# kotaro-kinoshita/yomitoku

Hardware: AMD Instinct MI355X
Metric: pages/sec (DocumentAnalyzer @1600x1200, lite model set) (higher is better)
Workload: dtype f32 held as two scaled fp16 planes per operand on the MFMA pipe: 3 x v_mfma_f32_32x32x16_f16 per product tile (products to 2^-21, below the fp32 accumulation's own rounding), fp32 accumulate, fp32 activations in HBM; attention, LayerNorm, the fused greedy step and every grid-starved launch exact fp3

## Files before the change

### include/ymk.h

```cpp
#ifndef YMK_H
#define YMK_H
#include <stddef.h>
#include <stdint.h>

#ifdef __cplusplus
extern "C" {
#endif

typedef struct ymk_model ymk_model;

int ymk_version(void);
const char* ymk_last_error(void);
int ymk_device_count(void);

ymk_model* ymk_model_create(const char* kind, int device);
void ymk_model_destroy(ymk_model* m);
int ymk_model_set_param(ymk_model* m, const char* key, double value);
int ymk_model_set_tensor(ymk_model* m, const char* name, const float* host_data, int ndim, const int64_t* dims);
int ymk_model_finalize(ymk_model* m);
int ymk_model_reserve(ymk_model* m, int n, int h, int w, void* stream);
int ymk_op_plan_workspace(int64_t n, const int64_t* sizes, const int64_t* release_pos, int64_t* offsets_out, int64_t* peak_out,
                          int64_t* live_bound_out);
int64_t ymk_model_weight_bytes(const ymk_model* m);
int64_t ymk_model_workspace_bytes(const ymk_model* m);
// ... 26 lines not shown
int ymk_crop_desc_size(void);

int ymk_db_postprocess(const float* prob_host, int h, int w, float thresh, float box_thresh, int min_size,
                       int max_candidates, float unclip_ratio, int dest_w, int dest_h, int16_t* quads_out,
                       double* scores_out, int capacity, int* count);

int ymk_table_hole_rects(int h, int w, const int* cell_boxes, int n, int pad, int close_ksize, int min_area, int* rects_out,
                         int capacity, int* count);

int ymk_prof_begin(void);
int ymk_debug_option(const char* key, int value);
int ymk_stat(const char* key, int64_t* value);
int ymk_amax_check_counters(int64_t* out4);
int ymk_prof_end(double* conv_ms, double* conv_flop, int64_t* conv_launches);
int ymk_prof_bytes(double* conv_bytes);
int ymk_prof_launch_table(double* ms, double* flop, double* bytes, double* mfma_products, int64_t capacity, int64_t* count);

int ymk_op_conv2d(const float* x_dev, int n, int h, int w, int c,
                  const float* w_host_oihw, int cout, int cin, int kh, int kw, const float* scale_host,
                  const float* bias_host, const float* res_dev, int stride, int pad, int dil, int act, int tap4,
                  float* y_dev, void* stream);
int ymk_op_conv1x1_astat(const float* x_dev, int m, int c, const float* w_host_oc, int cout, const float* scale_host,
                         const float* bias_host, const float* res_dev, int act, const float* ln_g_host, const float* ln_b_host,
                         float ln_eps, float* y_dev, int reps, float* kernel_ms, void* stream);

int ymk_op_vit_mlp(const float* x_dev, int m, int d, int f, const float* ln_g_host, const float* ln_b_host, float ln_eps,
                   const float* w1_host_fd, const float* b1_host, const float* w2_host_df, const float* b2_host, float* y_dev, int reps,
                   float* kernel_ms, void* stream);

int ymk_op_layernorm(const float* x_dev, int rows, int d, const float* g_dev, const float* b_dev, float eps,
                     float* y_dev, void* stream);
int ymk_op_attention(const float* q_dev, const float* k_dev, const float* v_dev, float* o_dev, int b, int heads, int lq,
                     int lk, int hd, float scale, const unsigned char* mask_qk_dev, const unsigned char* kpm_dev,
                     int use_small, void* stream);
int ymk_op_nar_cross_attention(const float* q_dev, const float* k_dev, const float* v_dev, float* o_dev, int b, int heads, int lq,
                               int lk, int hd, float scale, const int* koff_dev, const int* klen_dev, void* stream);
int ymk_op_maxpool3x3s2(const float* x_dev, int n, int h, int w, int c, float* y_dev, void* stream);
int ymk_op_upsample_bilinear(const float* x_dev, int n, int h, int w, int c, int oh, int ow, const float* add_dev,
                             float* y_dev, void* stream);

int ymk_op_topk_tokens(const float* logits_dev, int b, const int* level_hw, int nc, int k, int* idx_dev, void* stream);
int ymk_op_gather_queries(const float* om_dev, const float* bbox_dev, const float* anchors_dev, const int* idx_dev, int b,
                          const int* level_hw, int k, int d, float* content_dev, float* ref_dev, void* stream);
int ymk_op_refine_boxes(const float* delta_dev, const float* ref_dev, float* out_dev, int64_t n, void* stream);
int ymk_op_mask_rows(const float* in_dev, const float* valid_dev, int b, const int* level_hw, int d, float* out_dev, void* stream);
int ymk_op_deform_sample(const float* offs_dev, const float* attw_dev, const float* ref_dev, const float* value_dev, int ldv, int b,
                         const int* level_hw, int k, float* out_dev, void* stream);
int ymk_op_avgpool2x2_ceil(const float* x_dev, int n, int h, int w, int c, float* y_dev, void* stream);
int ymk_op_upsample_nearest2x(const float* x_dev, int n, int h, int w, int c, float* y_dev, void* stream);

int ymk_op_deconv2x2(const float* x_dev, int n, int h, int w, int cin, const float* w_host, int cout, const float* scale_host,
                     const float* bias_host, int act, float* y_dev, void* stream);
int ymk_op_deconv2x2_to1_sigmoid(const float* x_dev, int n, int h, int w, const float* w_host, float bias, float* y_dev, void* stream);
int ymk_op_dbnet_asf(const float* ax_dev, const float* fuse_dev, int n, int h, int w, const float* w1_host, const float* w2_host,
                     int cmid, const float* sp33_host, float sp11, const float* watt_host, float* out_dev, void* stream);

int ymk_op_parseq_dec_step(int d, int heads, int f, const float* sa_in_w_host, const float* sa_in_b_host, const float* sa_out_w_host,
                           const float* sa_out_b_host, const float* ca_in_w_host, const float* ca_in_b_host,
                           const float* ca_out_w_host, const float* ca_out_b_host, const float* lin1_w_host, const float* lin1_b_host,
                           const float* lin2_w_host, const float* lin2_b_host, const float* const* ln_host, const float* emb_host,
                           int ntok, const float* posq_host, const float* qsa_host, const int* tok_dev, float* skv_dev,
                           const float* memkv_dev, const int* mem_off_dev, const int* mem_len_dev, const int* prev_not_done_dev,
                           const int* gid_dev, const int* gopen_dev, int ng, int step, int b, int l, int ns, float* out_dev,
                           void* stream);
int ymk_op_greedy_step(const float* logits_dev, int64_t ld_b, int c, int step, int num_steps, int* tok_dev, int* raw_dev, int ld_tok,
                       int* state_dev, int eos_id, int rep_on, int period_max, int min_run_p1, int min_repeats, int* not_done_dev,
                       const int* prev_not_done_dev, const int* gid_dev, int* gopen_dev, int ng, int partials, int b, void* stream);
int ymk_op_refine_prep(const int* raw_dev, int ld_tok, int s_len, int bos_id, int eos_id, int* tok2_dev, unsigned char* kpm_dev, int b,
                       const int* gid_dev, const int* gsteps_dev, void* stream);
int ymk_op_rep_cut(float* logits_dev, int64_t ld_b, int c, int s_len, const int* state_dev, int eos_id, int b, void* stream);
int ymk_op_row_argmax(const float* logits_dev, int rows, int c, int* out_dev, void* stream);
int ymk_op_ctx_embed_ln(const int* tok_dev, int ld_tok, int pos0, int npos, const float* emb_dev, const float* posq_dev,
                        const float* g_dev, const float* b_dev, float eps, float* out_dev, int out_rows, int d, int b, void* stream);
int ymk_op_init_decode(int* tok_dev, int ld_tok, int* state_dev, int bos_id, int pad_id, int b, void* stream);
int ymk_op_tile_rows(const float* src_dev, int rows, int d, float* dst_dev, int b, void* stream);
int ymk_op_add_pos_embed(float* x_dev, const float* pos_dev, int b, int gh, int gw, int full_gw, int d, void* stream);

#ifdef __cplusplus
}
#endif
#endif
```

### yomitoku_amd/_lib.py

```python

from __future__ import annotations

import ctypes
import os
from ctypes import POINTER, c_char_p, c_double, c_float, c_int, c_int64, c_void_p

_HERE = os.path.dirname(os.path.abspath(__file__))
LIB_PATH = os.path.join(_HERE, "lib", "libymk_hip.so")

SIGNATURES = {
    "ymk_version": (c_int, []),
    "ymk_last_error": (c_char_p, []),
    "ymk_device_count": (c_int, []),
    "ymk_model_create": (c_void_p, [c_char_p, c_int]),
    "ymk_model_destroy": (None, [c_void_p]),
    "ymk_model_set_param": (c_int, [c_void_p, c_char_p, c_double]),
    "ymk_model_set_tensor": (c_int, [c_void_p, c_char_p, c_void_p, c_int, POINTER(c_int64)]),
    "ymk_model_finalize": (c_int, [c_void_p]),
    "ymk_model_reserve": (c_int, [c_void_p, c_int, c_int, c_int, c_void_p]),
    "ymk_op_plan_workspace": (c_int, [c_int64, POINTER(c_int64), POINTER(c_int64), POINTER(c_int64), POINTER(c_int64), POINTER(c_int64)]),
    "ymk_model_weight_bytes": (c_int64, [c_void_p]),
    "ymk_model_workspace_bytes": (c_int64, [c_void_p]),
    "ymk_dbnet_forward": (c_int, [c_void_p, c_void_p, c_int, c_int, c_int, c_void_p, c_void_p]),
    "ymk_parseq_dims": (c_int, [c_void_p, POINTER(c_int), POINTER(c_int)]),
# ... 31 lines not shown
    "ymk_stat": (c_int, [c_char_p, POINTER(c_int64)]),
    "ymk_op_vit_mlp": (
        c_int,
        [c_void_p, c_int, c_int, c_int, c_void_p, c_void_p, c_float, c_void_p, c_void_p, c_void_p, c_void_p, c_void_p, c_int, POINTER(c_float), c_void_p],
    ),
    "ymk_amax_check_counters": (c_int, [POINTER(c_int64)]),
    "ymk_prof_begin": (c_int, []),
    "ymk_prof_end": (c_int, [POINTER(c_double), POINTER(c_double), POINTER(c_int64)]),
    "ymk_prof_bytes": (c_int, [POINTER(c_double)]),
    "ymk_prof_launch_table": (c_int, [POINTER(c_double), POINTER(c_double), POINTER(c_double), POINTER(c_double), c_int64, POINTER(c_int64)]),
    "ymk_op_conv2d": (
        c_int,
        [c_void_p, c_int, c_int, c_int, c_int, c_void_p, c_int, c_int, c_int, c_int, c_void_p, c_void_p, c_void_p,
         c_int, c_int, c_int, c_int, c_int, c_void_p, c_void_p],
    ),
    "ymk_op_conv1x1_astat": (
        c_int,
        [c_void_p, c_int, c_int, c_void_p, c_int, c_void_p, c_void_p, c_void_p, c_int, c_void_p, c_void_p, c_float, c_void_p, c_int,
         POINTER(c_float), c_void_p],
    ),
    "ymk_op_layernorm": (c_int, [c_void_p, c_int, c_int, c_void_p, c_void_p, c_float, c_void_p, c_void_p]),
    "ymk_op_attention": (
        c_int,
        [c_void_p, c_void_p, c_void_p, c_void_p, c_int, c_int, c_int, c_int, c_int, c_float, c_void_p, c_void_p, c_int,
         c_void_p],
    ),
    "ymk_op_nar_cross_attention": (
        c_int,
        [c_void_p, c_void_p, c_void_p, c_void_p, c_int, c_int, c_int, c_int, c_int, c_float, c_void_p, c_void_p, c_void_p],
    ),
    "ymk_op_maxpool3x3s2": (c_int, [c_void_p, c_int, c_int, c_int, c_int, c_void_p, c_void_p]),
    "ymk_op_upsample_bilinear": (
        c_int,
        [c_void_p, c_int, c_int, c_int, c_int, c_int, c_int, c_void_p, c_void_p, c_void_p],
    ),
    "ymk_op_topk_tokens": (c_int, [c_void_p, c_int, POINTER(c_int), c_int, c_int, c_void_p, c_void_p]),
    "ymk_op_gather_queries": (
        c_int,
        [c_void_p, c_void_p, c_void_p, c_void_p, c_int, POINTER(c_int), c_int, c_int, c_void_p, c_void_p, c_void_p],
    ),
    "ymk_op_refine_boxes": (c_int, [c_void_p, c_void_p, c_void_p, c_int64, c_void_p]),
    "ymk_op_mask_rows": (c_int, [c_void_p, c_void_p, c_int, POINTER(c_int), c_int, c_void_p, c_void_p]),
    "ymk_op_deform_sample": (
        c_int,
        [c_void_p, c_void_p, c_void_p, c_void_p, c_int, c_int, POINTER(c_int), c_int, c_void_p, c_void_p],
    ),
    "ymk_op_avgpool2x2_ceil": (c_int, [c_void_p, c_int, c_int, c_int, c_int, c_void_p, c_void_p]),
    "ymk_op_upsample_nearest2x": (c_int, [c_void_p, c_int, c_int, c_int, c_int, c_void_p, c_void_p]),
    "ymk_op_deconv2x2": (
        c_int,
        [c_void_p, c_int, c_int, c_int, c_int, c_void_p, c_int, c_void_p, c_void_p, c_int, c_void_p, c_void_p],
    ),
    "ymk_op_deconv2x2_to1_sigmoid": (c_int, [c_void_p, c_int, c_int, c_int, c_void_p, c_float, c_void_p, c_void_p]),
    "ymk_op_dbnet_asf": (
        c_int,
        [c_void_p, c_void_p, c_int, c_int, c_int, c_void_p, c_void_p, c_int, c_void_p, c_float, c_void_p, c_void_p, c_void_p],
    ),
    "ymk_op_parseq_dec_step": (
        c_int,
        [c_int, c_int, c_int] + [c_void_p] * 12 + [POINTER(c_void_p), c_void_p, c_int, c_void_p, c_void_p]
        + [c_void_p] * 8 + [c_int, c_int, c_int, c_int, c_int, c_void_p, c_void_p],
    ),
    "ymk_op_greedy_step": (
        c_int,
        [c_void_p, c_int64, c_int, c_int, c_int, c_void_p, c_void_p, c_int, c_void_p, c_int, c_int, c_int, c_int, c_int, c_void_p,
         c_void_p, c_void_p, c_void_p, c_int, c_int, c_int, c_void_p],
    ),
    "ymk_op_refine_prep": (c_int, [c_void_p, c_int, c_int, c_int, c_int, c_void_p, c_void_p, c_int, c_void_p, c_void_p, c_void_p]),
    "ymk_op_rep_cut": (c_int, [c_void_p, c_int64, c_int, c_int, c_void_p, c_int, c_int, c_void_p]),
    "ymk_op_row_argmax": (c_int, [c_void_p, c_int, c_int, c_void_p, c_void_p]),
    "ymk_op_ctx_embed_ln": (
        c_int,
        [c_void_p, c_int, c_int, c_int, c_void_p, c_void_p, c_void_p, c_void_p, c_float, c_void_p, c_int, c_int, c_int, c_void_p],
    ),
    "ymk_op_init_decode": (c_int, [c_void_p, c_int, c_void_p, c_int, c_int, c_int, c_void_p]),
    "ymk_op_tile_rows": (c_int, [c_void_p, c_int, c_int, c_void_p, c_int, c_void_p]),
    "ymk_op_add_pos_embed": (c_int, [c_void_p, c_void_p, c_int, c_int, c_int, c_int, c_int, c_void_p]),
}

_lib = None


class YmkError(RuntimeError):
    pass


def load():
    global _lib
    if _lib is not None:
        return _lib
    if not os.path.exists(LIB_PATH):
        raise YmkError(
            f"{LIB_PATH} not found - build it with `python -c 'import __graft_entry__ as g; g.build()'` "
            "or `make -C yomitoku_amd/csrc` (there is no CPU fallback)"
        )
    lib = ctypes.CDLL(LIB_PATH)
    for name, (res, args) in SIGNATURES.items():
        fn = getattr(lib, name)
        fn.restype = res
        fn.argtypes = args
    _lib = lib
    spec = os.environ.get("YMK_DEBUG_OPTIONS", "")
    if os.environ.get("YMK_CONV_SPLIT"):
        spec += ",conv_split=" + os.environ["YMK_CONV_SPLIT"]
    if os.environ.get("YMK_WORKSPACE_REUSE"):
        spec += ",workspace_reuse=" + os.environ["YMK_WORKSPACE_REUSE"]
# ... 71 lines not shown
```

### yomitoku_amd/csrc/ymk_api.cpp

```cpp
#include "../../include/ymk.h"
#include "ymk_common.h"
#include "ymk_decstep.h"
#include "ymk_det.h"
#include "ymk_seq.h"

namespace ymk {
const std::string& last_error();
void dbnet_forward(Model* m, const float* x, int n, int h, int w, float* prob, hipStream_t s);
void parseq_forward(Model* m, const float* x, int B, int W, float* logits, int* out_len, int* ar_steps, hipStream_t s);
void parseq_forward_groups(Model* m, const float* const* x, const int* b, const int* w, int ng, float* logits, int* out_len,
                           int* ar_steps, hipStream_t s);
void parseq_dims(Model* m, int* num_steps, int* num_classes);
Model* create_parseq();
Model* create_rtdetr();
void rtdetr_forward(Model* m, const float* x, int B, int H, int W, float* logits, float* boxes, hipStream_t s);
void row_maxprob(hipStream_t s, const float* logits, int rows, int C, int* ids, float* probs);
void prof_begin();
void prof_end(double* ms, double* flop, int64_t* launches);
double prof_bytes();
int64_t prof_launch_table(double* ms, double* flop, double* bytes, double* products, int64_t capacity);
bool gemm_takes_astat(int M, int K, const ConvW& w, bool with_res, int ld);
bool conv_debug_option(const std::string& key, int value);
bool parseq_debug_option(const std::string& key, int value);
bool decstep_debug_option(const std::string& key, int value);
bool conv_split_debug_option(const std::string& key, int value);
bool conv_split_stat(const std::string& key, long long* value);
bool parseq_stat(const std::string& key, long long* value);
void amax_check_counters(long long* out4);
}

struct ymk_model {
  ymk::Model* impl = nullptr;
  int device = 0;
};

#include <dlfcn.h>
namespace {
struct Roctx {
  int (*push)(const char*) = nullptr;
  int (*pop)() = nullptr;
  Roctx() {
    const char* on = std::getenv("YMK_ROCTX");
    if (on == nullptr || on[0] == '\0' || on[0] == '0') return;
    for (const char* name : {"librocprofiler-sdk-roctx.so", "libroctx64.so"}) {
      if (void* h = dlopen(name, RTLD_NOW | RTLD_GLOBAL)) {
        push = reinterpret_cast<int (*)(const char*)>(dlsym(h, "roctxRangePushA"));
        pop = reinterpret_cast<int (*)()>(dlsym(h, "roctxRangePop"));
        if (push && pop) return;
        push = nullptr;
        pop = nullptr;
      }
    }
  }
};
struct RoctxRange {
  explicit RoctxRange(const char* name) {
    static Roctx r;
    pop_ = r.pop;
    if (r.push) (void)r.push(name);
    else pop_ = nullptr;
  }
  ~RoctxRange() {
    if (pop_) (void)pop_();
  }
  int (*pop_)() = nullptr;
};
}

#define YMK_API_BEGIN try {
#define YMK_API_END                                 \
  return 0;                                         \
  }                                                 \
  catch (const std::exception& e) {                 \
    ymk::set_error(e.what());                       \
    return 1;                                       \
  }                                                 \
  catch (...) {                                     \
    ymk::set_error("unknown C++ exception");        \
    return 2;                                       \
// ... 104 lines not shown
int ymk_parseq_forward(ymk_model* m, const float* x_dev, int b, int w, float* logits_dev, int* out_len, int* ar_steps,
                       void* stream) {
  YMK_API_BEGIN
  RoctxRange roctx_range("ymk_parseq_forward");
  YMK_CHECK(m && x_dev && logits_dev && out_len && ar_steps, "null argument");
  YMK_HIP(hipSetDevice(m->device));
  ymk::parseq_forward(m->impl, x_dev, b, w, logits_dev, out_len, ar_steps, (hipStream_t)stream);
  YMK_API_END
}

int ymk_parseq_forward_groups(ymk_model* m, const float* const* x_dev, const int* b, const int* w, int n_groups,
                              float* logits_dev, int* out_len, int* ar_steps, void* stream) {
  YMK_API_BEGIN
  RoctxRange roctx_range("ymk_parseq_forward_groups");
  YMK_CHECK(m && x_dev && b && w && logits_dev && out_len && ar_steps, "null argument");
  YMK_HIP(hipSetDevice(m->device));
  ymk::parseq_forward_groups(m->impl, x_dev, b, w, n_groups, logits_dev, out_len, ar_steps, (hipStream_t)stream);
  YMK_API_END
}

int ymk_parseq_token_stats(const float* logits_dev, int rows, int num_classes, int* ids_dev, float* probs_dev,
                           void* stream) {
  YMK_API_BEGIN
  RoctxRange roctx_range("ymk_parseq_token_stats");
  YMK_CHECK(logits_dev && ids_dev && probs_dev, "null argument");
  ymk::row_maxprob((hipStream_t)stream, logits_dev, rows, num_classes, ids_dev, probs_dev);
  YMK_API_END
}

int ymk_rtdetr_forward(ymk_model* m, const float* x_dev, int b, int h, int w, float* logits_dev, float* boxes_dev,
                       void* stream) {
  YMK_API_BEGIN
  RoctxRange roctx_range("ymk_rtdetr_forward");
  YMK_CHECK(m && x_dev && logits_dev && boxes_dev, "null argument");
  YMK_HIP(hipSetDevice(m->device));
  ymk::rtdetr_forward(m->impl, x_dev, b, h, w, logits_dev, boxes_dev, (hipStream_t)stream);
  YMK_API_END
}

int ymk_debug_option(const char* key, int value) {
  YMK_API_BEGIN
  YMK_CHECK(key != nullptr, "null key");
  const std::string k(key);
  YMK_CHECK(ymk::conv_debug_option(k, value) || ymk::parseq_debug_option(k, value) || ymk::decstep_debug_option(k, value) ||
                ymk::conv_split_debug_option(k, value) || ymk::runtime_debug_option(k, value),
            "unknown debug option: " + k);
  YMK_API_END
}

int ymk_stat(const char* key, int64_t* value) {
  YMK_API_BEGIN
  YMK_CHECK(key != nullptr && value != nullptr, "null argument");
  long long v = 0;
  YMK_CHECK(ymk::conv_split_stat(std::string(key), &v) || ymk::runtime_stat(std::string(key), &v) || ymk::parseq_stat(std::string(key), &v), std::string("unknown counter: ") + key);
  *value = v;
  YMK_API_END
}

int ymk_amax_check_counters(int64_t* out4) {
  YMK_API_BEGIN
  YMK_CHECK(out4 != nullptr, "null argument");
  long long v[4];
  ymk::amax_check_counters(v);
  for (int i = 0; i < 4; ++i) out4[i] = v[i];
  YMK_API_END
}

int ymk_prof_begin(void) {
  YMK_API_BEGIN
  ymk::prof_begin();
  YMK_API_END
}

int ymk_prof_end(double* conv_ms, double* conv_flop, int64_t* conv_launches) {
  YMK_API_BEGIN
  YMK_CHECK(conv_ms && conv_flop && conv_launches, "null argument");
  ymk::prof_end(conv_ms, conv_flop, conv_launches);
  YMK_API_END
}

int ymk_prof_bytes(double* conv_bytes) {
  YMK_API_BEGIN
  YMK_CHECK(conv_bytes, "null argument");
  *conv_bytes = ymk::prof_bytes();
  YMK_API_END
}

int ymk_prof_launch_table(double* ms, double* flop, double* bytes, double* mfma_products, int64_t capacity, int64_t* count) {
  YMK_API_BEGIN
  YMK_CHECK(count != nullptr && capacity >= 0 && (capacity == 0 || (ms && flop && bytes && mfma_products)), "null argument");
  *count = ymk::prof_launch_table(ms, flop, bytes, mfma_products, capacity);
  YMK_API_END
}

int ymk_op_plan_workspace(int64_t n, const int64_t* sizes, const int64_t* release_pos, int64_t* offsets_out, int64_t* peak_out,
                          int64_t* live_bound_out) {
  YMK_API_BEGIN
  YMK_CHECK(n >= 0 && (n == 0 || (sizes && offsets_out)), "plan_workspace: bad argument");
  std::vector<size_t> sz((size_t)n), off((size_t)n);
  for (int64_t k = 0; k < n; ++k) {
    YMK_CHECK(sizes[k] >= 0, "plan_workspace: negative size");
    sz[(size_t)k] = (size_t)sizes[k];
  }
  size_t peak = 0, live = 0;
  ymk::plan_workspace((size_t)n, sz.data(), release_pos, off.data(), &peak, &live);
  for (int64_t k = 0; k < n; ++k) offsets_out[k] = (int64_t)off[(size_t)k];
  if (peak_out) *peak_out = (int64_t)peak;
// ... 260 lines not shown

int ymk_op_deform_sample(const float* offs_dev, const float* attw_dev, const float* ref_dev, const float* value_dev, int ldv, int b,
                         const int* level_hw, int k, float* out_dev, void* stream) {
  YMK_API_BEGIN
  using namespace ymk;
  const DetGeom g = det_geom_arg(b, level_hw);
  YMK_CHECK(offs_dev && attw_dev && ref_dev && value_dev && out_dev && k >= 1, "deform_sample: bad argument");
  YMK_CHECK(ldv >= 256 && ldv % 4 == 0, "deform_sample: ldv >= 256, a multiple of 4");
  YMK_CHECK(aligned16(value_dev) && aligned16(ref_dev) && aligned16(out_dev), "deform_sample: value / ref / out must be 16 B aligned");
  deform_sample((hipStream_t)stream, offs_dev, attw_dev, ref_dev, value_dev, ldv, g, k, out_dev);
  YMK_API_END
}

int ymk_op_avgpool2x2_ceil(const float* x_dev, int n, int h, int w, int c, float* y_dev, void* stream) {
  YMK_API_BEGIN
  using namespace ymk;
  YMK_CHECK(x_dev && y_dev && n >= 1 && h >= 1 && w >= 1 && c >= 4 && c % 4 == 0, "avgpool: c must be a positive multiple of 4");
  Tensor in{const_cast<float*>(x_dev), n, h, w, c, c};
  Tensor out{y_dev, n, (h + 1) / 2, (w + 1) / 2, c, c};
  avgpool2x2_ceil((hipStream_t)stream, in, out);
  YMK_API_END
}

int ymk_op_upsample_nearest2x(const float* x_dev, int n, int h, int w, int c, float* y_dev, void* stream) {
  YMK_API_BEGIN
  using namespace ymk;
  YMK_CHECK(x_dev && y_dev && n >= 1 && h >= 1 && w >= 1 && c >= 4 && c % 4 == 0, "nearest2x: c must be a positive multiple of 4");
  Tensor in{const_cast<float*>(x_dev), n, h, w, c, c};
  Tensor out{y_dev, n, 2 * h, 2 * w, c, c};
  upsample_nearest2x((hipStream_t)stream, in, out);
  YMK_API_END
}

int ymk_op_deconv2x2(const float* x_dev, int n, int h, int w, int cin, const float* w_host, int cout, const float* scale_host,
                     const float* bias_host, int act, float* y_dev, void* stream) {
  YMK_API_BEGIN
  using namespace ymk;
  YMK_CHECK(x_dev && w_host && y_dev && n >= 1 && h >= 1 && w >= 1, "deconv2x2: bad argument");
  YMK_CHECK(cin >= 4 && cin % 4 == 0 && cout >= 4 && cout % 4 == 0, "deconv2x2: cin and cout must be positive multiples of 4");
  DevicePool pool;
  const ConvW cw = make_deconv2x2_panel(pool, w_host, cin, cout, scale_host, bias_host);
  Tensor in{const_cast<float*>(x_dev), n, h, w, cin, cin};
  Tensor out{y_dev, n, 2 * h, 2 * w, cout, cout};
  ConvArgs a;
  a.act = act;
  a.epi = EPI_DECONV2X2;
  SplitCtxOwner split_ctx;
  ConvSplitScope scope(-1, split_ctx.get(), 0);
  conv2d((hipStream_t)stream, in, cw, a, out);
  YMK_HIP(hipStreamSynchronize((hipStream_t)stream));
  YMK_API_END
}

int ymk_op_deconv2x2_to1_sigmoid(const float* x_dev, int n, int h, int w, const float* w_host, float bias, float* y_dev,
                                 void* stream) {
  YMK_API_BEGIN
  using namespace ymk;
  YMK_CHECK(x_dev && w_host && y_dev && n >= 1 && h >= 1 && w >= 1, "deconv_to1: bad argument");
  YMK_CHECK(aligned16(x_dev), "deconv_to1: input must be 16 B aligned");
  DevicePool pool;
  const float* wd = pool.upload(w_host, 64 * 4);
  Tensor in{const_cast<float*>(x_dev), n, h, w, 64, 64};
  deconv2x2_to1_sigmoid((hipStream_t)stream, in, wd, bias, y_dev);
  YMK_HIP(hipStreamSynchronize((hipStream_t)stream));
  YMK_API_END
}

int ymk_op_dbnet_asf(const float* ax_dev, const float* fuse_dev, int n, int h, int w, const float* w1_host, const float* w2_host,
                     int cmid, const float* sp33_host, float sp11, const float* watt_host, float* out_dev, void* stream) {
  YMK_API_BEGIN
  using namespace ymk;
  YMK_CHECK(ax_dev && fuse_dev && out_dev && w1_host && w2_host && sp33_host && watt_host && n >= 1 && h >= 1 && w >= 1,
            "asf: bad argument");
  YMK_CHECK(cmid >= 1 && cmid <= 64, "asf: 1 <= cmid <= 64");
  YMK_CHECK(aligned16(ax_dev) && aligned16(fuse_dev) && aligned16(out_dev), "asf: tensors must be 16 B aligned");
  hipStream_t s = (hipStream_t)stream;
  DevicePool pool;
  const float* w1 = pool.upload(w1_host, (size_t)cmid * 64);
  const float* w2 = pool.upload(w2_host, (size_t)64 * cmid);
  const float* sp33 = pool.upload(sp33_host, 9);
  const float* watt = pool.upload(watt_host, 4 * 64);
  float* gap_scr = pool.alloc((size_t)GAP_CHUNKS * n * 64);
  float* gap = pool.alloc((size_t)n * 64);
  float* gate = pool.alloc((size_t)n * 64);
  float* cmean = pool.alloc((size_t)n * h * w);
  Tensor x{const_cast<float*>(ax_dev), n, h, w, 64, 64};
  Tensor fuse{const_cast<float*>(fuse_dev), n, h, w, 256, 256};
  Tensor out{out_dev, n, h, w, 256, 256};
  asf_block(s, x, w1, w2, cmid, sp33, sp11, watt, fuse, gap_scr, gap, gate, cmean, out);
  YMK_HIP(hipStreamSynchronize(s));
  YMK_API_END
}

int ymk_op_parseq_dec_step(int d, int heads, int f, const float* sa_in_w_host, const float* sa_in_b_host, const float* sa_out_w_host,
                           const float* sa_out_b_host, const float* ca_in_w_host, const float* ca_in_b_host,
                           const float* ca_out_w_host, const float* ca_out_b_host, const float* lin1_w_host, const float* lin1_b_host,
                           const float* lin2_w_host, const float* lin2_b_host, const float* const* ln_host, const float* emb_host,
                           int ntok, const float* posq_host, const float* qsa_host, const int* tok_dev, float* skv_dev,
                           const float* memkv_dev, const int* mem_off_dev, const int* mem_len_dev, const int* prev_not_done_dev,
                           const int* gid_dev, const int* gopen_dev, int ng, int step, int b, int l, int ns, float* out_dev,
                           void* stream) {
  YMK_API_BEGIN
  using namespace ymk;
  YMK_CHECK(d >= 4 && heads >= 1 && f >= 4 && l >= 1 && ns >= 1 && parseq_dec_step_supported(d, heads, f, l, ns),
            "fused decoder step: unsupported geometry");
  YMK_CHECK(sa_in_w_host && sa_in_b_host && sa_out_w_host && sa_out_b_host && ca_in_w_host && ca_in_b_host && ca_out_w_host &&
// ... 99 lines not shown
```

### yomitoku_amd/csrc/ymk_common.h

```cpp
#pragma once
#include <hip/hip_runtime.h>
#include <cstdint>
#include <cstdio>
#include <cstring>
#include <map>
#include <string>
#include <vector>
#include <stdexcept>
#include <cmath>

namespace ymk {

void set_error(const std::string& msg);

struct Error : public std::runtime_error {
  explicit Error(const std::string& m) : std::runtime_error(m) {}
};

#define YMK_HIP(expr)                                                                 \
  do {                                                                                \
    hipError_t e__ = (expr);                                                          \
    if (e__ != hipSuccess) {                                                          \
      throw ::ymk::Error(std::string(#expr) + " failed: " + hipGetErrorString(e__) +  \
                         " at " + __FILE__ + ":" + std::to_string(__LINE__));         \
// ... 57 lines not shown
  size_t high_water() const { return high_; }
  size_t capacity() const { return cap_; }
  bool dry_run = false;
  void amax_begin(hipStream_t s, int records);
  unsigned* amax_next();
  bool planned() const { return planned_; }
  bool set_planned(bool on);
  bool resize_pending() const { return resize_pending_; }
  size_t plan_commit(uint64_t key, bool bound = false);
  bool plan_select(uint64_t key, size_t* need);
  void forward_begin();
 private:
  struct Plan {
    std::vector<size_t> size, off;
    std::vector<int64_t> rel;
    std::vector<uint32_t> rel_order;
    size_t peak = 0, bump = 0, live = 0;
  };
  void publish(const Plan& p) const;
  char* base_ = nullptr;
  size_t cap_ = 0, off_ = 0, high_ = 0;
  unsigned* amax_pool_ = nullptr;
  int amax_n_ = 0, amax_used_ = 0;
  hipStream_t stream_ = nullptr;
  bool planned_ = false, resize_pending_ = false;
  std::map<uint64_t, Plan> plans_;
  std::vector<Plan> bounds_;
  const Plan* cur_ = nullptr;
  size_t k_ = 0, r_ = 0;
  std::vector<size_t> t_size_, t_at_;
  std::vector<int64_t> t_rel_;
  std::vector<uint32_t> t_rel_order_;
};
bool runtime_debug_option(const std::string& key, int value);
bool workspace_reuse_default();

__device__ __forceinline__ void amax_fold(unsigned& am, float v) { am = max(am, __float_as_uint(fabsf(v))); }
__device__ __forceinline__ void amax_fold4(unsigned& am, const float4 v) {
  am = max(max(am, __float_as_uint(fabsf(v.x))), max(__float_as_uint(fabsf(v.y)), max(__float_as_uint(fabsf(v.z)), __float_as_uint(fabsf(v.w)))));
}
__device__ __forceinline__ void amax_commit(unsigned* rec, unsigned am, int t) {
#pragma unroll
  for (int o = 32; o > 0; o >>= 1) am = max(am, (unsigned)__shfl_xor((int)am, o));
  if ((t & 63) == 0 && am != 0u)
    atomicMax(rec + ((blockIdx.x * (blockDim.x >> 6) + (t >> 6)) & (AMAX_LINES - 1)) * AMAX_LINE_WORDS, am);
}
__device__ __forceinline__ unsigned amax_read(const unsigned* rec, int lane) {
  unsigned m = rec[(lane & (AMAX_LINES - 1)) * AMAX_LINE_WORDS];
#pragma unroll
  for (int o = 16; o > 0; o >>= 1) m = max(m, (unsigned)__shfl_xor((int)m, o));
  return m;
}

enum Act : int { ACT_NONE = 0, ACT_RELU = 1, ACT_SILU = 2, ACT_SIGMOID = 3, ACT_GELU = 4 };

__device__ __forceinline__ float gelu_f32(float v) {
  const float z = fabsf(v) * 0.70710678118654752440f;
  const float t = __builtin_amdgcn_rcpf(fmaf(0.39032074649205456f, z, 1.f));
  float q = -0.22690855651422961f;
  q = fmaf(q, t, 0.8816638035254636f);
  q = fmaf(q, t, -0.6277749224408846f);
  q = fmaf(q, t, 0.6443424378640197f);
  q = fmaf(q, t, 0.09342759526711675f);
  q = fmaf(q, t, 0.23524963446014596f);
  const float e = __builtin_amdgcn_exp2f(z * z * -1.4426950408889634f);
  const float r = fmaf(-(t * q), e, 1.f);
  const float hv = 0.5f * v;
  return fmaf(hv, copysignf(r, v), hv);
}

struct ConvW {
  float* w = nullptr;
  float* scale = nullptr;
  float* bias = nullptr;
  int cout = 0, cin = 0, kh = 1, kw = 1;
  int kpad = 0, ctiles = 0, mode = 0;
  float pl_a = 0.f, pl_b = 0.f;
};

enum Epi : int { EPI_STORE = 0, EPI_DECONV2X2 = 1, EPI_ROWMAX = 2 };
constexpr int ROWMAX_TILE_N = 64;

struct ConvArgs {
  int stride = 1, pad = 0, dil = 1;
  int stride_w = 0;
  int act = ACT_NONE;
  int epi = EPI_STORE;
  const Tensor* res = nullptr;
  bool res_post = false;
  const int* row_group = nullptr;
  const int* group_open = nullptr;
  const unsigned* amax_in = nullptr;
  unsigned* amax_out = nullptr;
  const float* ln_g = nullptr;
  const float* ln_b = nullptr;
  float ln_eps = 0.f;
  bool out_planes = false;
};

constexpr int SPLIT_F16X2 = 16;
class SplitCtx;
struct SplitCtxOwner {
  SplitCtx* get();
  ~SplitCtxOwner();
 private:
  SplitCtx* p_ = nullptr;
};
constexpr int SPLIT_MODEL_DEFAULT = SPLIT_F16X2;
class ConvSplitScope {
 public:
  explicit ConvSplitScope(int split, SplitCtx* ctx = nullptr, int dflt = -1);
  ~ConvSplitScope();
 private:
  int prev_, prev_dflt_;
  SplitCtx* prev_ctx_;
};

class ConvSplitTileScope {
 public:
  explicit ConvSplitTileScope(int tile);
  ~ConvSplitTileScope();
 private:
  int prev_;
};

int conv_effective_split();
void absmax_record(hipStream_t s, const float* x, size_t n, unsigned* rec);

void conv2d(hipStream_t s, const Tensor& in, const ConvW& w, const ConvArgs& a, const Tensor& out);

bool conv_planes_pair_ok(const Tensor& in, const ConvW& w1, const ConvArgs& a1, const ConvW& w2, const ConvArgs& a2);

void gemm(hipStream_t s, const float* A, int M, int K, int lda, const ConvW& w, int act, const float* res, int res_ld,
          float* out, int out_ld, const int* row_group = nullptr, const int* group_open = nullptr, int epi = EPI_STORE,
          const unsigned* amax_in = nullptr, unsigned* amax_out = nullptr);

bool gemm_ln_fused(hipStream_t s, const float* X, int M, int K, int ldx, const float* ln_g, const float* ln_b, float ln_eps, const ConvW& w,
                   int act, const float* res, int res_ld, float* out, int out_ld, const unsigned* amax_in, unsigned* amax_out = nullptr);

bool vit_mlp_fused(hipStream_t s, float* x, int M, int ld, const float* ln_g, const float* ln_b, float ln_eps, float ln_bound, const ConvW& fc1,
                   const ConvW& fc2);
float layernorm_output_bound(const std::vector<float>& gamma, const std::vector<float>& beta);

void pack_conv_weight(const float* oihw, int cout, int cin, int kh, int kw, bool tap4,
                      std::vector<float>& panel, int& kpad, int& ctiles);

inline int conv_out_dim(int in, int k, int stride, int pad, int dil) {
  return (in + 2 * pad - dil * (k - 1) - 1) / stride + 1;
}

void nchw3_to_nhwc4(hipStream_t s, const float* in, int n, int h, int w, const Tensor& out);
void maxpool3x3s2(hipStream_t s, const Tensor& in, const Tensor& out);
void upsample_bilinear(hipStream_t s, const Tensor& in, const Tensor& out, const Tensor* add);
void upsample_nearest2x(hipStream_t s, const Tensor& in, const Tensor& out);
void avgpool2x2_ceil(hipStream_t s, const Tensor& in, const Tensor& out);
constexpr int GAP_CHUNKS = 256;
void global_avgpool(hipStream_t s, const Tensor& in, float* scratch, float* out_nc);
void add_act(hipStream_t s, const Tensor& a, const Tensor& b, int act, const Tensor& out);
void amax_merge(hipStream_t s, unsigned* dst, const unsigned* src);

void asf_channel_gate(hipStream_t s, const float* gap_nc, const float* w1, const float* w2, int n,
                      int c, int cmid, float* gate_nc);
void asf_channel_mean(hipStream_t s, const Tensor& x, const float* gate_nc, float* mean_nhw);
void asf_apply(hipStream_t s, const Tensor& x, const float* gate_nc, const float* mean_nhw,
               const float* w_sp3x3, float w_sp1x1, const float* w_att ,
               const Tensor& fuse , const Tensor& out);
void asf_block(hipStream_t s, const Tensor& x, const float* w1 , const float* w2 , int cmid,
               const float* w_sp3x3, float w_sp1x1, const float* w_att , const Tensor& fuse, float* gap_scr,
               float* gap, float* gate, float* cmean, const Tensor& out);
void deconv2x2_to1_sigmoid(hipStream_t s, const Tensor& in, const float* w_c4 , float bias,
                           float* out);

struct HostTensor {
  std::vector<int64_t> dims;
  std::vector<float> data;
  size_t numel() const { return data.size(); }
};

class WeightStore {
 public:
  void put(const std::string& name, const float* data, int ndim, const int64_t* dims);
  const HostTensor& get(const std::string& name) const;
  bool has(const std::string& name) const { return t_.count(name) != 0; }
  void clear() { t_.clear(); }
// ... 56 lines not shown
```

### yomitoku_amd/csrc/ymk_conv.hip

```cpp
#include <atomic>
#include <deque>
#include <mutex>

#include "ymk_conv_kernel.h"

namespace ymk {

template <int BM, int BN, int WM, int WN, int MODE, int PF = 1, int OPT = 0>
__global__ __launch_bounds__(64 * WM * WN, ((OPT & 2) ? blocks_per_cu(BM, BN, OPT) : 2 * (BM + BN) * LDK * 4 <= 80 * 1024 ? 2 : 1) * WM * WN / 4) void conv_igemm(ConvK p) {
  static_assert(PF == 1 || PF == 2, "prefetch distance 1 or 2");
  constexpr int LDR = lds_row(OPT);
  static_assert(!(OPT & 2) || (64 * WM * WN / 8) % 16 == 0, "swizzle: staging passes must keep (row >> 1) & 7");
  constexpr int NT = 64 * WM * WN;
  static_assert(NT == 256 || NT == 512 || NT == 1024, "4, 8 or 16 waves per block");
  constexpr int WTM = BM / WM, WTN = BN / WN;
  constexpr int TM = WTM / 32, TN = WTN / 32;
  constexpr int RPP = NT / 8;
  constexpr int APASS = BM / RPP, BPASS = BN / RPP;
  static_assert(BM % RPP == 0 && BN % RPP == 0, "tile rows must divide by the staging pass");
  constexpr int STAGE = (BM + BN) * LDR;
  constexpr int LDC = BN + 4;
  constexpr int EROWS = (2 * STAGE / LDC) / 32 * 32 < BM ? (2 * STAGE / LDC) / 32 * 32 : BM;
  static_assert(EROWS >= WTM && EROWS % WTM == 0, "an epilogue pass must hold whole wave tiles");
  __shared__ __attribute__((aligned(16))) float lds[2 * STAGE];

  const int t = threadIdx.x;
  int tile;
  {
    const int nblk = gridDim.x, bid = blockIdx.x;
    const int xcd = bid & 7, idx = bid >> 3, q = nblk >> 3, r = nblk & 7;
    tile = (xcd < r ? xcd * (q + 1) : r * (q + 1) + (xcd - r) * q) + idx;
  }
  const int tile_m = tile / p.ntiles_n, tile_n = tile - tile_m * p.ntiles_n;
  const int m0 = tile_m * BM, n0 = tile_n * BN;
  if (!tile_needed<BM, NT>(p, m0, t)) return;

  const int colq = t & 7, rowb = t >> 3;
  int pixb[APASS], ih0[APASS], iw0[APASS];
  const bool pointwise = (p.fast & 1) && p.KH == 1 && p.KW == 1 && p.stride == 1 && p.stride_w == 1 && p.pad == 0;
#pragma unroll
  for (int i = 0; i < APASS; ++i) {
    const int m = m0 + rowb + RPP * i;
    if (m < p.M && pointwise) {
      pixb[i] = m;
      ih0[i] = 0;
      iw0[i] = 0;
    } else if (m < p.M) {
      const int ohw = p.OH * p.OW;
      const int n = m / ohw, rem = m - n * ohw;
      const int oh = rem / p.OW, ow = rem - oh * p.OW;
      pixb[i] = n * p.H * p.W;
      ih0[i] = oh * p.stride - p.pad;
      iw0[i] = ow * p.stride_w - p.pad;
    } else {
      pixb[i] = 0;
      ih0[i] = -(1 << 20);
      iw0[i] = 0;
    }
  }
  const float* wrow = p.w + (size_t)(n0 + rowb) * p.Kpad + colq * 4;

// ... 62 lines not shown
      *reinterpret_cast<f32x4*>(Bs + RPP * j * LDR) = rb[set][j];
  };

  const int wv = t >> 6, lane = t & 63;
  const int wm = wv / WN, wn = wv - wm * WN;
  const int li = lane & 31, lh = lane >> 5;

  f32x16 acc[TM][TN];
#pragma unroll
  for (int a = 0; a < TM; ++a)
#pragma unroll
    for (int b = 0; b < TN; ++b)
#pragma unroll
      for (int r = 0; r < 16; ++r) acc[a][b][r] = 0.f;

  const int ktiles = p.Kpad >> 5;

  int a_off[4], b_off[4];
#pragma unroll
  for (int kc = 0; kc < 4; ++kc) {
    a_off[kc] = lds_slot<OPT>(wm * WTM + li, 2 * kc + lh);
    b_off[kc] = BM * LDR + lds_slot<OPT>(wn * WTN + li, 2 * kc + lh);
  }
  auto compute = [&](int buf) {
    const float* Ts = lds + buf * STAGE;
#pragma unroll
    for (int kc = 0; kc < 4; ++kc) {
      f32x4 fa[TM], fb[TN];
#pragma unroll
      for (int a = 0; a < TM; ++a)
        fa[a] = *reinterpret_cast<const f32x4*>(Ts + a_off[kc] + a * 32 * LDR);
#pragma unroll
      for (int b = 0; b < TN; ++b)
        fb[b] = *reinterpret_cast<const f32x4*>(Ts + b_off[kc] + b * 32 * LDR);
#pragma unroll
      for (int a = 0; a < TM; ++a)
#pragma unroll
        for (int b = 0; b < TN; ++b) {
          acc[a][b] = __builtin_amdgcn_mfma_f32_32x32x2f32(fa[a].x, fb[b].x, acc[a][b], 0, 0, 0);
          acc[a][b] = __builtin_amdgcn_mfma_f32_32x32x2f32(fa[a].y, fb[b].y, acc[a][b], 0, 0, 0);
          acc[a][b] = __builtin_amdgcn_mfma_f32_32x32x2f32(fa[a].z, fb[b].z, acc[a][b], 0, 0, 0);
          acc[a][b] = __builtin_amdgcn_mfma_f32_32x32x2f32(fa[a].w, fb[b].w, acc[a][b], 0, 0, 0);
        }
    }
  };

  load_tile(0, 0);
  store_tile(0, 0);
  if (PF == 2 && ktiles > 1) load_tile(1, 1);
  __syncthreads();

  using Epi = EpiRows<EROWS, BN, NT>;
  constexpr bool CAN_PRE = PF == 1 && EROWS == BM && Epi::NR <= 8 && NT <= 512;
  const bool pre_res = CAN_PRE && (p.fast & 2) && p.res != nullptr && p.vec && p.epi == EPI_STORE;
  float4 rpre[CAN_PRE ? Epi::NR : 1];
  if (PF == 1) {
    for (int kt = 0; kt < ktiles; ++kt) {
      const int buf = kt & 1;
      if (kt + 1 < ktiles) load_tile(kt + 1, 0);
      if (CAN_PRE && kt + 1 == ktiles && pre_res) prefetch_residual<EROWS, BN, NT>(p, m0, n0, t, rpre);
      compute(buf);
      if (kt + 1 < ktiles) store_tile(buf ^ 1, 0);
      if (!(OPT & 1) || kt + 1 < ktiles) __syncthreads();
    }
  } else {
    for (int kt = 0; kt < ktiles; kt += 2) {
      if (kt + 2 < ktiles) load_tile(kt + 2, 0);
      compute(0);
      if (kt + 1 < ktiles) store_tile(1, PF - 1);
      __syncthreads();
      if (kt + 1 >= ktiles) break;
      if (kt + 3 < ktiles) load_tile(kt + 3, PF - 1);
      compute(1);
      if (kt + 2 < ktiles) store_tile(0, 0);
      __syncthreads();
    }
  }

  if (OPT & 1) {
    epilogue_direct<TM, TN>(p, acc, m0 + wm * WTM, n0 + wn * WTN, li, lh);
    return;
  }
  float* Cs = lds;
#pragma unroll
  for (int e0 = 0; e0 < BM; e0 += EROWS) {
    if (e0 > 0) __syncthreads();
    if (wm * WTM >= e0 && wm * WTM < e0 + EROWS) {
#pragma unroll
      for (int a = 0; a < TM; ++a)
#pragma unroll
        for (int b = 0; b < TN; ++b)
#pragma unroll
          for (int r = 0; r < 16; ++r) {
            const int row = wm * WTM - e0 + a * 32 + (r & 3) + 8 * (r >> 2) + 4 * lh;
            Cs[row * LDC + wn * WTN + b * 32 + li] = acc[a][b][r];
          }
    }
    __syncthreads();
    if (CAN_PRE && pre_res) epilogue_tile<EROWS, BN, NT, true>(p, Cs, m0 + e0, n0, t, rpre);
    else epilogue_tile<EROWS, BN, NT>(p, Cs, m0 + e0, n0, t);
  }
}

template <int TM, int TN, int NW, int PF>
__global__ __launch_bounds__(64 * NW) void conv_splitk(ConvK p) {
  constexpr int BM = 32 * TM, BN = 32 * TN, NT = 64 * NW;
  constexpr int LDC = BN + 4;
  constexpr int PART = TM * TN * 16 * 64;
  constexpr int RED = (NW / 2) * PART > BM * LDC ? (NW / 2) * PART : BM * LDC;
  __shared__ __attribute__((aligned(16))) float red[RED];

  const int t = threadIdx.x;
  const int lane = t & 63, li = lane & 31, lh = lane >> 5;
  const int wv = __builtin_amdgcn_readfirstlane(t >> 6);
  int tile;
  {
    const int nblk = gridDim.x, bid = blockIdx.x;
    const int xcd = bid & 7, idx = bid >> 3, q = nblk >> 3, r = nblk & 7;
    tile = (xcd < r ? xcd * (q + 1) : r * (q + 1) + (xcd - r) * q) + idx;
  }
  const int tile_m = tile / p.ntiles_n, tile_n = tile - tile_m * p.ntiles_n;
  const int m0 = tile_m * BM, n0 = tile_n * BN;
  if (!tile_needed<BM, NT>(p, m0, t)) return;

  int pixb[TM], ih0[TM], iw0[TM];
  const bool pointwise = (p.fast & 1) && p.KH == 1 && p.KW == 1 && p.stride == 1 && p.stride_w == 1 && p.pad == 0;
#pragma unroll
  for (int a = 0; a < TM; ++a) {
    const int m = m0 + 32 * a + li;
    if (m < p.M && pointwise) {
      pixb[a] = m;
      ih0[a] = 0;
      iw0[a] = 0;
    } else if (m < p.M) {
      const int ohw = p.OH * p.OW;
      const int n = m / ohw, rem = m - n * ohw;
      const int oh = rem / p.OW, ow = rem - oh * p.OW;
      pixb[a] = n * p.H * p.W;
      ih0[a] = oh * p.stride - p.pad;
      iw0[a] = ow * p.stride_w - p.pad;
    } else {
      pixb[a] = 0;
      ih0[a] = -(1 << 20);
      iw0[a] = 0;
    }
  }
  const float* wrow = p.w + (size_t)(n0 + li) * p.Kpad + lh * 4;
  const __amdgpu_buffer_rsrc_t rsrc = __builtin_amdgcn_make_buffer_rsrc(const_cast<float*>(p.in), 0, p.in_bytes, 0x00020000);

  const int ktiles = p.Kpad >> 5;
  const int nt = wv < ktiles ? (ktiles - wv + NW - 1) / NW : 0;
  f32x4 sa[PF][TM][4], sb[PF][TN][4];

  auto load = [&](int s, int j) {
    int kt = wv + NW * j;
    kt = kt < ktiles ? kt : ktiles - 1;
    const int tap = kt / p.ctiles, cc = kt - tap * p.ctiles;
// ... 43 lines not shown

#pragma unroll
  for (int s = 0; s < PF; ++s) load(s, s);
  int j0 = 0;
  for (; j0 + PF <= nt; j0 += PF) {
#pragma unroll
    for (int s = 0; s < PF; ++s) {
      compute(s);
      load(s, j0 + s + PF);
    }
  }
  {
    const int rem = nt - j0;
#pragma unroll
    for (int s = 0; s < PF - 1; ++s)
      if (s < rem) compute(s);
  }

#pragma unroll
  for (int half = NW / 2; half >= 1; half >>= 1) {
    if (wv >= half && wv < 2 * half) {
      float* dst = red + (wv - half) * PART + lane;
#pragma unroll
      for (int a = 0; a < TM; ++a)
#pragma unroll
        for (int b = 0; b < TN; ++b)
#pragma unroll
          for (int r = 0; r < 16; ++r) dst[((a * TN + b) * 16 + r) * 64] = acc[a][b][r];
    }
    __syncthreads();
    if (wv < half) {
      const float* src = red + wv * PART + lane;
#pragma unroll
      for (int a = 0; a < TM; ++a)
#pragma unroll
        for (int b = 0; b < TN; ++b)
#pragma unroll
          for (int r = 0; r < 16; ++r) acc[a][b][r] += src[((a * TN + b) * 16 + r) * 64];
    }
    __syncthreads();
  }
  if (wv == 0) {
#pragma unroll
    for (int a = 0; a < TM; ++a)
#pragma unroll
      for (int b = 0; b < TN; ++b)
#pragma unroll
        for (int r = 0; r < 16; ++r) {
          const int row = a * 32 + (r & 3) + 8 * (r >> 2) + 4 * lh;
          red[row * LDC + b * 32 + li] = acc[a][b][r];
        }
  }
  __syncthreads();
  epilogue_tile<BM, BN, NT>(p, red, m0, n0, t);
}

struct ProfState {
  std::mutex mu;
  bool on = false;
  std::deque<std::pair<hipEvent_t, hipEvent_t>> ev;
  size_t used = 0;
  double flop = 0.0;
  double bytes = 0.0;
  std::vector<std::string> desc;
  std::vector<double> lflop, lbytes, lms, lprod;
};
static ProfState g_prof;

constexpr int SPLITK_MAX_GRID = 384;
static std::atomic<int> g_splitk_force{-1};
static std::atomic<int> g_no_splitk{0};
static std::atomic<int> g_conv_fast{27};
static std::atomic<int> g_conv_variant{0};
static std::atomic<int> g_prof_dump{0};
static std::atomic<int> g_conv_split{-1};
static std::atomic<int> g_gemm_row_limit{0};
static int gemm_row_limit() { return g_gemm_row_limit.load(std::memory_order_relaxed); }
static int splitk_forced() { return g_splitk_force.load(std::memory_order_relaxed); }
static bool no_splitk() { return g_no_splitk.load(std::memory_order_relaxed) != 0; }
static thread_local int t_conv_split = -1;
static thread_local SplitCtx* t_split_ctx = nullptr;
static thread_local int t_split_default = 0;
ConvSplitScope::ConvSplitScope(int split, SplitCtx* ctx, int dflt) : prev_(t_conv_split), prev_dflt_(t_split_default), prev_ctx_(t_split_ctx) {
  t_conv_split = split;
  if (ctx) t_split_ctx = ctx;
  if (dflt >= 0) t_split_default = dflt;
}
ConvSplitScope::~ConvSplitScope() {
  t_conv_split = prev_;
  t_split_default = prev_dflt_;
  t_split_ctx = prev_ctx_;
}

int conv_effective_split() {
  int split = t_conv_split;
  if (split < 0) split = g_conv_split.load(std::memory_order_relaxed);
  if (split < 0) split = t_split_default;
  return split;
}

bool conv_debug_option(const std::string& key, int value) {
  if (key == "splitk_force") g_splitk_force = value;
  else if (key == "no_splitk") g_no_splitk = value;
  else if (key == "conv_variant") g_conv_variant = value;
  else if (key == "conv_fast") g_conv_fast = value;
  else if (key == "prof_dump") g_prof_dump = value;
  else if (key == "conv_split") g_conv_split = value;
  else if (key == "gemm_row_limit") g_gemm_row_limit = value;
  else return false;
  return true;
}

void prof_begin() {
  std::lock_guard<std::mutex> lock(g_prof.mu);
  g_prof.on = true;
  g_prof.used = 0;
  g_prof.flop = 0.0;
  g_prof.bytes = 0.0;
}
double prof_bytes() {
  std::lock_guard<std::mutex> lock(g_prof.mu);
  return g_prof.bytes;
}
void prof_end(double* ms, double* flop, int64_t* launches) {
  std::lock_guard<std::mutex> lock(g_prof.mu);
  double total = 0.0;
  for (size_t i = 0; i < g_prof.used; ++i) {
    YMK_HIP(hipEventSynchronize(g_prof.ev[i].second));
    float t = 0.f;
    YMK_HIP(hipEventElapsedTime(&t, g_prof.ev[i].first, g_prof.ev[i].second));
    total += t;
    g_prof.lms[i] = t;
    if (g_prof_dump.load(std::memory_order_relaxed))
      fprintf(stderr, "[ymk-prof] %3zu %s  %8.1f us  %6.1f TFLOP/s  %7.1f MB\n", i, g_prof.desc[i].c_str(), t * 1e3,
              g_prof.lflop[i] / (t * 1e-3) / 1e12, g_prof.lbytes[i] / 1e6);
  }
  *ms = total;
  *flop = g_prof.flop;
  *launches = (int64_t)g_prof.used;
  g_prof.on = false;
}
int64_t prof_launch_table(double* ms, double* flop, double* bytes, double* products, int64_t capacity) {
  std::lock_guard<std::mutex> lock(g_prof.mu);
  const int64_t n = g_prof.on ? 0 : (int64_t)g_prof.used;
  for (int64_t i = 0; i < n && i < capacity; ++i) {
    ms[i] = g_prof.lms[i];
    flop[i] = g_prof.lflop[i];
    bytes[i] = g_prof.lbytes[i];
    products[i] = g_prof.lprod[i];
  }
  return n;
}

std::pair<hipEvent_t, hipEvent_t>* conv_prof_open(hipStream_t s, const ConvK& k, int BM, int BN, int grid, int ksplit) {
  std::pair<hipEvent_t, hipEvent_t>* e = nullptr;
  if (g_prof.on) {
    std::lock_guard<std::mutex> lock(g_prof.mu);
    if (g_prof.used == g_prof.ev.size()) {
      std::pair<hipEvent_t, hipEvent_t> n;
      YMK_HIP(hipEventCreate(&n.first));
      YMK_HIP(hipEventCreate(&n.second));
      g_prof.ev.push_back(n);
    }
    e = &g_prof.ev[g_prof.used++];
    const int creal = k.mode == 0 ? k.C : 3;
    const double fl = 2.0 * (double)k.M * (double)k.Cout * (double)(k.KH * k.KW * creal);
    g_prof.flop += fl;
    const double images = (double)k.M / ((double)k.OH * k.OW);
    const double outs = (double)k.M * k.Cout;
    const double by = 4.0 * (images * k.H * k.W * creal + (double)k.Cout * k.KH * k.KW * creal + outs * (k.res ? 2.0 : 1.0));
    g_prof.bytes += by;
    char buf[176];
    snprintf(buf, sizeof buf, "M=%7d Cin=%4d Cout=%4d k=%dx%d s=%d d=%d res=%d tile=%dx%d ksplit=%d grid=%d", k.M, k.C, k.Cout,
             k.KH, k.KW, k.stride, k.dil, k.res ? 1 : 0, BM, BN, ksplit, grid);
    if (g_prof.desc.size() < g_prof.used) {
      g_prof.desc.resize(g_prof.used);
      g_prof.lflop.resize(g_prof.used);
      g_prof.lbytes.resize(g_prof.used);
      g_prof.lms.resize(g_prof.used);
      g_prof.lprod.resize(g_prof.used);
    }
    g_prof.desc[g_prof.used - 1] = buf;
    g_prof.lflop[g_prof.used - 1] = fl;
    g_prof.lbytes[g_prof.used - 1] = by;
    g_prof.lms[g_prof.used - 1] = 0.0;
    g_prof.lprod[g_prof.used - 1] = ksplit >= 160 ? 3.0 : (ksplit == 30 ? 6.0 : (ksplit == 20 ? 3.0 : 0.0));
    YMK_HIP(hipEventRecord(e->first, s));
  }
  return e;
}

std::pair<hipEvent_t, hipEvent_t>* conv_prof_open_raw(hipStream_t s, const char* desc, double flops, double bytes, double products) {
  if (!g_prof.on) return nullptr;
  std::lock_guard<std::mutex> lock(g_prof.mu);
  if (g_prof.used == g_prof.ev.size()) {
    std::pair<hipEvent_t, hipEvent_t> n;
    YMK_HIP(hipEventCreate(&n.first));
    YMK_HIP(hipEventCreate(&n.second));
    g_prof.ev.push_back(n);
  }
  auto* e = &g_prof.ev[g_prof.used++];
  g_prof.flop += flops;
  g_prof.bytes += bytes;
  if (g_prof.desc.size() < g_prof.used) {
    g_prof.desc.resize(g_prof.used);
    g_prof.lflop.resize(g_prof.used);
    g_prof.lbytes.resize(g_prof.used);
    g_prof.lms.resize(g_prof.used);
    g_prof.lprod.resize(g_prof.used);
  }
  g_prof.desc[g_prof.used - 1] = desc;
  g_prof.lflop[g_prof.used - 1] = flops;
  g_prof.lbytes[g_prof.used - 1] = bytes;
  g_prof.lms[g_prof.used - 1] = 0.0;
  g_prof.lprod[g_prof.used - 1] = products;
  YMK_HIP(hipEventRecord(e->first, s));
  return e;
}

template <int TM, int TN, int NW, int PF>
static void launch_splitk(hipStream_t s, ConvK& k) {
  const int mt = (k.M + 32 * TM - 1) / (32 * TM), nt = (k.Cout + 32 * TN - 1) / (32 * TN);
  k.ntiles_n = nt;
  auto* e = conv_prof_open(s, k, 32 * TM, 32 * TN, mt * nt, NW);
  hipLaunchKernelGGL((conv_splitk<TM, TN, NW, PF>), dim3(mt * nt), dim3(64 * NW), 0, s, k);
  if (e) YMK_HIP(hipEventRecord(e->second, s));
}

static bool try_splitk(hipStream_t s, ConvK& k) {
  struct Cand {
    int tm, tn, nw;
    void (*fn)(hipStream_t, ConvK&);
  };
  static const Cand cands[] = {
      {2, 2, 4, launch_splitk<2, 2, 4, 2>}, {2, 1, 4, launch_splitk<2, 1, 4, 3>}, {2, 1, 8, launch_splitk<2, 1, 8, 3>},
      {1, 1, 4, launch_splitk<1, 1, 4, 4>}, {1, 1, 8, launch_splitk<1, 1, 8, 4>},
  };
  if (k.in_bytes >= SPLITK_OOB_ROW) return false;
  const int ktiles = k.Kpad >> 5;
  const Cand* best = nullptr;
  double best_cost = 0.0;
  for (const Cand& c : cands) {
    const long blocks = (long)((k.M + 32 * c.tm - 1) / (32 * c.tm)) * ((k.Cout + 32 * c.tn - 1) / (32 * c.tn));
    const long waves = blocks * c.nw;
    const double per_wave = (double)((ktiles + c.nw - 1) / c.nw) * c.tm * c.tn * 1024.0 + 3000.0 + (c.nw == 8 ? 1800.0 : 1200.0);
    const double cost = (double)((waves + 1023) / 1024) * per_wave;
    if (!best || cost < best_cost * 0.97) {
      best = &c;
      best_cost = cost;
    }
  }
  const int forced = splitk_forced();
  if (forced >= 0) best = &cands[forced % (int)(sizeof(cands) / sizeof(cands[0]))];
  best->fn(s, k);
  return true;
}

template <int BM, int BN, int WM, int WN, int MODE = 0, int PF = 1>
static void launch(hipStream_t s, ConvK& k) {
  const int mt = (k.M + BM - 1) / BM, nt = (k.Cout + BN - 1) / BN;
  k.ntiles_n = nt;
  if (MODE == 0 && (mt * nt < SPLITK_MAX_GRID || splitk_forced() >= 0) && !no_splitk() && try_splitk(s, k)) return;
  constexpr bool HAS_OPT = MODE == 0 && PF == 1;
  constexpr bool HAS_SWZ = HAS_OPT && BM == 128 && BN == 64 && WM * WN == 8;
  const bool direct = HAS_OPT && k.epi == EPI_STORE && ((k.fast & 4) || ((k.fast & 16) && !k.vec));
  const bool swz = HAS_SWZ && (k.fast & 8);
  auto* e = conv_prof_open(s, k, BM, BN, mt * nt, 1);
  const dim3 grid(mt * nt), block(64 * WM * WN);
  if constexpr (HAS_SWZ) {
    if (swz && direct) hipLaunchKernelGGL((conv_igemm<BM, BN, WM, WN, MODE, PF, 3>), grid, block, 0, s, k);
    else if (swz) hipLaunchKernelGGL((conv_igemm<BM, BN, WM, WN, MODE, PF, 2>), grid, block, 0, s, k);
  }
  if constexpr (HAS_OPT) {
    if (direct && !swz) hipLaunchKernelGGL((conv_igemm<BM, BN, WM, WN, MODE, PF, 1>), grid, block, 0, s, k);
  }
  if (!direct && !swz) hipLaunchKernelGGL((conv_igemm<BM, BN, WM, WN, MODE, PF>), grid, block, 0, s, k);
  if (e) YMK_HIP(hipEventRecord(e->second, s));
}

static void launch_wide(hipStream_t s, ConvK& k) {
  switch (g_conv_variant.load(std::memory_order_relaxed)) {
    case 1: launch<128, 128, 2, 2>(s, k); break;
    case 2: launch<128, 128, 4, 4>(s, k); break;
    case 4: launch<128, 128, 4, 2>(s, k); break;
    case 5: launch<128, 128, 4, 2, 0, 2>(s, k); break;
    case 8: launch<128, 64, 4, 2>(s, k); break;
    default:
      if (k.Kpad <= 512) launch<128, 128, 4, 4>(s, k);
      else launch<128, 128, 4, 2>(s, k);
      break;
  }
}
static void launch_n64(hipStream_t s, ConvK& k) {
  switch (g_conv_variant.load(std::memory_order_relaxed)) {
    case 3: launch<128, 64, 2, 2>(s, k); break;
    case 6: launch<128, 64, 4, 2, 0, 2>(s, k); break;
    default: launch<128, 64, 4, 2>(s, k); break;
  }
}

static bool conv2d_impl(hipStream_t s, const Tensor& in, const ConvW& w, const ConvArgs& a, const Tensor& out) {
  ConvK k{};
  k.ln_g = a.ln_g;
  k.ln_b = a.ln_b;
  k.ln_eps = a.ln_eps;
  k.in_planes = in.planes ? 1 : 0;
  k.out_planes = a.out_planes ? 1 : 0;
  k.pl_a = w.pl_a;
  k.pl_b = w.pl_b;
  if (a.out_planes)
    YMK_CHECK(a.epi == EPI_STORE && a.res == nullptr && out.ld == w.cout && w.cout % 32 == 0 && out.amax != nullptr,
              "conv: fp16 planes are written by plain stores into a whole tensor of 32-channel slices that has a record");
  if (in.planes) YMK_CHECK(in.ld == in.c && in.c % 32 == 0 && in.amax != nullptr, "conv: malformed tensor of fp16 planes");
  k.in = in.p;
  k.w = w.w;
  k.scale = w.scale;
  k.bias = w.bias;
  k.res = a.res ? a.res->p : nullptr;
  k.res_ld = a.res ? a.res->ld : 0;
  k.res_post = a.res_post ? 1 : 0;
  k.out = out.p;
  k.H = in.h;
  k.W = in.w;
  k.C = in.c;
  k.in_ld = in.ld;
  k.KH = w.kh;
  k.KW = w.kw;
  k.stride = a.stride;
  k.stride_w = a.stride_w > 0 ? a.stride_w : a.stride;
  k.pad = a.pad;
  k.dil = a.dil;
  k.OH = conv_out_dim(in.h, w.kh, a.stride, a.pad, a.dil);
  k.OW = conv_out_dim(in.w, w.kw, k.stride_w, a.pad, a.dil);
  k.Cout = w.cout;
  k.out_ld = out.ld;
  k.Kpad = w.kpad;
  k.ctiles = w.ctiles;
  k.mode = w.mode;
  k.M = in.n * k.OH * k.OW;
  k.act = a.act;
  k.epi = a.epi;
  k.row_group = a.row_group;
  k.group_open = a.group_open;
  k.amax = in.amax ? in.amax : a.amax_in;
  k.amax_out = a.epi == EPI_ROWMAX ? nullptr : (out.amax ? out.amax : a.amax_out);
  YMK_CHECK((a.row_group == nullptr) == (a.group_open == nullptr), "conv: row_group and group_open come together");
  YMK_CHECK(w.w != nullptr, "conv weight not packed");
  if (w.mode == 0) {
    YMK_CHECK(in.c == w.cin, "conv: input channels " + std::to_string(in.c) + " != weight cin " + std::to_string(w.cin));
    YMK_CHECK(in.c % 4 == 0 && in.ld % 4 == 0, "conv: channels/ld must be multiples of 4");
  } else {
    YMK_CHECK(in.c == 4 && in.ld == 4, "conv tap4 mode wants a 4-channel packed input");
  }
  YMK_CHECK(((uintptr_t)in.p & 15) == 0, "conv: input not 16B aligned");
  if (a.epi == EPI_ROWMAX) {
    YMK_CHECK(a.res == nullptr && a.act == ACT_NONE && w.mode == 0, "row-max epilogue: plain linear layers only");
    YMK_CHECK(out.ld == 2 * ((w.cout + ROWMAX_TILE_N - 1) / ROWMAX_TILE_N), "row-max epilogue: out must be [M][2 * ceil(Cout / 64)]");
  } else if (a.epi == EPI_STORE) {
    YMK_CHECK(out.n == in.n && out.h == k.OH && out.w == k.OW && out.c == w.cout, "conv: bad output shape");
    if (a.res && a.res->ld != 0)
      YMK_CHECK(a.res->n == out.n && a.res->h == out.h && a.res->w == out.w && a.res->c == out.c, "conv: bad residual shape");
  } else {
    YMK_CHECK(w.kh == 1 && w.kw == 1 && a.stride == 1 && a.pad == 0, "deconv epilogue wants a 1x1 panel");
    YMK_CHECK(out.n == in.n && out.h == 2 * in.h && out.w == 2 * in.w && out.c * 4 == w.cout, "deconv: bad output shape");
  }
  if (k.M == 0) return true;
  {
    const size_t ib = ((in.pixels() - 1) * (size_t)in.ld + in.c) * sizeof(float);
    if (a.ln_g != nullptr && ib >= (size_t)OOB_OFFSET) return false;
    YMK_CHECK(ib < (size_t)OOB_OFFSET, "conv input view must stay below 4 GiB (split the batch)");
    k.in_bytes = (unsigned)ib;
  }
  {
    auto al16 = [](const void* q) { return ((uintptr_t)q & 15) == 0; };
    const int cq = a.epi == EPI_DECONV2X2 ? w.cout / 4 : w.cout;
    k.vec = (cq % 4 == 0) && (out.ld % 4 == 0) && al16(out.p) && (!w.scale || al16(w.scale)) &&
            (!w.bias || al16(w.bias)) && (!a.res || (a.res->ld % 4 == 0 && al16(a.res->p)));
    if (a.epi == EPI_DECONV2X2) YMK_CHECK(k.vec, "deconv epilogue needs 16 B aligned channels");
  }
  k.fast = g_conv_fast.load(std::memory_order_relaxed);

  {
    int split = t_conv_split;
    if (split < 0) split = g_conv_split.load(std::memory_order_relaxed);
    if (split < 0) split = t_split_default;
    if (split != 0 && t_split_ctx != nullptr && conv2d_split(s, k, w, split, t_split_ctx)) return true;
    if (a.ln_g != nullptr) return false;
    YMK_CHECK(!in.planes && !a.out_planes, "conv: fp16 planes outside the fp16-split path (conv_planes_pair_ok decides before the launch)");
  }
  if (a.epi == EPI_ROWMAX) {
    k.vec = 0;
    const int mt = (k.M + 63) / 64, nt = (k.Cout + ROWMAX_TILE_N - 1) / ROWMAX_TILE_N;
    k.ntiles_n = nt;
    auto* e = conv_prof_open(s, k, 64, 64, mt * nt, 1);
    hipLaunchKernelGGL((conv_igemm<64, 64, 2, 2, 0, 1>), dim3(mt * nt), dim3(256), 0, s, k);
    if (e) YMK_HIP(hipEventRecord(e->second, s));
    YMK_HIP(hipGetLastError());
    return true;
  }
  const long blocks128 = (long)((k.M + 127) / 128) * ((w.cout + 127) / 128);
  if (w.mode == 0 && g_conv_variant.load(std::memory_order_relaxed) == 7) {
    launch<64, 64, 2, 2>(s, k);
  } else if (w.mode == 1) {
    if (w.cout <= 32) launch<128, 32, 4, 1, 1>(s, k);
    else launch<128, 64, 2, 2, 1>(s, k);
  } else if (w.cout <= 32) {
    launch<128, 32, 4, 1>(s, k);
  } else if (w.cout <= 64) {
    if ((k.M + 127) / 128 >= 256) launch_n64(s, k);
    else launch<64, 64, 2, 2>(s, k);
  } else if (blocks128 >= 384) {
    const int waste = (128 - w.cout % 128) % 128;
    const bool short_k = (k.fast & 8) && k.Kpad <= 512 && g_conv_variant.load(std::memory_order_relaxed) == 0;
    if ((waste >= 48 && waste * 5 >= w.cout) || short_k) launch_n64(s, k);
    else launch_wide(s, k);
  } else {
    const long blocks64 = (long)((k.M + 127) / 128) * ((w.cout + 63) / 64);
    const int pad_rows = (k.M + 127) / 128 * 128 - k.M;
    if (blocks64 >= 256 && !(k.M <= 1024 && pad_rows * 8 >= k.M)) launch_n64(s, k);
    else launch<64, 64, 2, 2>(s, k);
  }
  YMK_HIP(hipGetLastError());
  return true;
}

int conv_split_route_with_planes(long M, int cout, int kpad, int taps, bool* auto_tile);

bool conv_planes_pair_ok(const Tensor& in, const ConvW& w1, const ConvArgs& a1, const ConvW& w2, const ConvArgs& a2) {
  if (conv_effective_split() != SPLIT_F16X2 || t_split_ctx == nullptr) return false;
  if (w1.mode != 0 || w2.mode != 0 || a1.epi != EPI_STORE || a2.epi != EPI_STORE || a1.res != nullptr) return false;
  if (a1.row_group != nullptr || a2.row_group != nullptr || a1.ln_g != nullptr) return false;
  if (a1.act != ACT_NONE && a1.act != ACT_RELU && a1.act != ACT_SILU && a1.act != ACT_GELU) return false;
  if (w1.cout % 32 != 0 || w2.cin != w1.cout || w2.kh * w2.kw <= 1 || in.planes) return false;
  const int sw1 = a1.stride_w > 0 ? a1.stride_w : a1.stride, sw2 = a2.stride_w > 0 ? a2.stride_w : a2.stride;
  const int h1 = conv_out_dim(in.h, w1.kh, a1.stride, a1.pad, a1.dil), v1 = conv_out_dim(in.w, w1.kw, sw1, a1.pad, a1.dil);
  const int h2 = conv_out_dim(h1, w2.kh, a2.stride, a2.pad, a2.dil), v2 = conv_out_dim(v1, w2.kw, sw2, a2.pad, a2.dil);
  if (h1 <= 0 || v1 <= 0 || h2 <= 0 || v2 <= 0) return false;
  if ((size_t)in.n * h1 * v1 * w1.cout * sizeof(float) >= (size_t)OOB_OFFSET) return false;
  bool auto1 = false, auto2 = false;
  const int r1 = conv_split_route_with_planes((long)in.n * h1 * v1, w1.cout, w1.kpad, w1.kh * w1.kw, &auto1);
  const int r2 = conv_split_route_with_planes((long)in.n * h2 * v2, w2.cout, w2.kpad, w2.kh * w2.kw, &auto2);
  return auto1 && auto2 && (r1 == 2 || r1 == 3) && r2 == 2;
}

void conv2d(hipStream_t s, const Tensor& in, const ConvW& w, const ConvArgs& a, const Tensor& out) {
  YMK_CHECK(a.ln_g == nullptr, "conv2d: a fused LayerNorm goes through gemm_ln_fused");
  (void)conv2d_impl(s, in, w, a, out);
}

bool gemm_ln_fused(hipStream_t s, const float* X, int M, int K, int ldx, const float* ln_g, const float* ln_b, float ln_eps, const ConvW& w,
                   int act, const float* res, int res_ld, float* out, int out_ld, const unsigned* amax_in, unsigned* amax_out) {
  YMK_CHECK(K == w.cin && ln_g != nullptr && ln_b != nullptr, "gemm_ln_fused: K must equal the weight's in-features; gamma and beta are required");
  if (w.kh != 1 || w.kw != 1 || w.mode != 0 || amax_in == nullptr) return false;
  Tensor in{const_cast<float*>(X), 1, 1, M, K, ldx};
  Tensor o{out, 1, 1, M, w.cout, out_ld};
  Tensor r{const_cast<float*>(res), 1, 1, M, w.cout, res_ld};
  ConvArgs a;
  a.act = act;
  a.res = res ? &r : nullptr;
  a.amax_in = amax_in;
  a.amax_out = amax_out;
  a.ln_g = ln_g;
  a.ln_b = ln_b;
  a.ln_eps = ln_eps;
  return conv2d_impl(s, in, w, a, o);
}

bool vit_mlp_split_launch(hipStream_t s, SplitCtx* ctx, float* x, int M, int ld, const float* ln_g, const float* ln_b, float ln_eps,
                          float ln_bound, const ConvW& fc1, const ConvW& fc2);

bool vit_mlp_fused(hipStream_t s, float* x, int M, int ld, const float* ln_g, const float* ln_b, float ln_eps, float ln_bound, const ConvW& fc1,
                   const ConvW& fc2) {
  if (conv_effective_split() != SPLIT_F16X2 || t_split_ctx == nullptr) return false;
  return vit_mlp_split_launch(s, t_split_ctx, x, M, ld, ln_g, ln_b, ln_eps, ln_bound, fc1, fc2);
}

void gemm(hipStream_t s, const float* A, int M, int K, int lda, const ConvW& w, int act, const float* res, int res_ld,
          float* out, int out_ld, const int* row_group, const int* group_open, int epi, const unsigned* amax_in, unsigned* amax_out) {
  YMK_CHECK(K == w.cin, "gemm: K " + std::to_string(K) + " != weight in-features " + std::to_string(w.cin));
// ... 46 lines not shown
```

### yomitoku_amd/csrc/ymk_conv_astat.hip

```cpp
#include <atomic>
#include <string>

#include "ymk_conv_kernel.h"

namespace ymk {

typedef _Float16 as_hf16x2_t __attribute__((ext_vector_type(2)));
typedef _Float16 as_hf16x8_t __attribute__((ext_vector_type(8)));
typedef float as_hf32x2_t __attribute__((ext_vector_type(2)));
typedef __attribute__((address_space(3))) void as_lds_void;

__device__ __forceinline__ float2 astat_scales(unsigned amax_bits) {
  int e = (int)(amax_bits >> 23);
  e = e < 27 ? 27 : (e > 227 ? 227 : e);
  float2 r;
  r.x = __uint_as_float((unsigned)(268 - e) << 23);
  r.y = __uint_as_float((unsigned)(e - 14) << 23);
  return r;
}

__device__ __forceinline__ void astat_split8(const f32x4 u, const f32x4 v, float sa, as_hf16x8_t& hi, as_hf16x8_t& lo) {
  as_hf32x2_t x[4] = {{u.x, u.y}, {u.z, u.w}, {v.x, v.y}, {v.z, v.w}};
  as_hf16x2_t h[4], l[4];
#pragma unroll
// ... 252 lines not shown
        }
#pragma unroll
        for (int b = 0; b < TN; ++b) acc[b] = __builtin_amdgcn_mfma_f32_32x32x16_f16(al[kt][s], bh[b], acc[b], 0, 0, 0);
#pragma unroll
        for (int b = 0; b < TN; ++b) acc[b] = __builtin_amdgcn_mfma_f32_32x32x16_f16(ah[kt][s], bl[b], acc[b], 0, 0, 0);
#pragma unroll
        for (int b = 0; b < TN; ++b) acc[b] = __builtin_amdgcn_mfma_f32_32x32x16_f16(ah[kt][s], bh[b], acc[b], 0, 0, 0);
        if (s == 0 && issued < total) {
          issue(inb, ikt, stp);
          advance();
          ++issued;
        }
      }
      st = st == NST - 1 ? 0 : st + 1;
      stp = stp == NST - 1 ? 0 : stp + 1;
    }
    if constexpr (RM) {
      static_assert(!RM || TN == 4, "row-max epilogue: 128-column blocks");
      astat_rowmax(p, acc, inv_sa, m0 + 32 * wv, nb * BN, li, lh);
    } else {
      switch (p.act) {
        case ACT_RELU: astat_store<ACT_RELU, TN, RG>(p, acc, inv_sa, m0 + 32 * wv, nb * BN, li, lh, rsrc_o, rsrc_r, am); break;
        case ACT_GELU: astat_store<ACT_GELU, TN, RG>(p, acc, inv_sa, m0 + 32 * wv, nb * BN, li, lh, rsrc_o, rsrc_r, am); break;
        case ACT_SILU: astat_store<ACT_SILU, TN, RG>(p, acc, inv_sa, m0 + 32 * wv, nb * BN, li, lh, rsrc_o, rsrc_r, am); break;
        case ACT_SIGMOID: astat_store<ACT_SIGMOID, TN, RG>(p, acc, inv_sa, m0 + 32 * wv, nb * BN, li, lh, rsrc_o, rsrc_r, am); break;
        default: astat_store<ACT_NONE, TN, RG>(p, acc, inv_sa, m0 + 32 * wv, nb * BN, li, lh, rsrc_o, rsrc_r, am); break;
      }
    }
#pragma unroll
    for (int b = 0; b < TN; ++b)
#pragma unroll
      for (int r = 0; r < 16; ++r) acc[b][r] = 0.f;
  }
  if (p.amax_out) amax_commit(p.amax_out, am, t);
}


static std::atomic<int> g_astat_rowmax_dealt{0};
void astat_rowmax_dealt(int on) { g_astat_rowmax_dealt = on; }

template <int BN, int KT, bool LN, bool RM = false>
static void launch_astat(hipStream_t s, ConvK& k, const void* planes, size_t w_bytes, int groups) {
  hipLaunchKernelGGL((conv_f16_astat<BN, KT, LN, RM>), dim3((k.M + 127) / 128, groups), dim3(256), 0, s, k, reinterpret_cast<const uint4*>(planes), (unsigned)w_bytes);
}

static bool astat_narrow(const ConvK& k) { return k.epi == EPI_ROWMAX ? false : k.Kpad > 192 || k.Cout <= 64 || (k.res != nullptr && k.Kpad > 128) || k.ln_g != nullptr; }

int conv2d_f16_astat_columns(const ConvK& k) { return astat_narrow(k) ? 64 : 128; }

bool conv2d_f16_astat_can(const ConvK& k, size_t w_bytes) {
  if (k.KH != 1 || k.KW != 1 || k.stride != 1 || k.stride_w != 1 || k.pad != 0) return false;
  if (k.epi == EPI_ROWMAX) {
    if (k.Kpad > 192 || k.res != nullptr || k.ln_g != nullptr || k.act != ACT_NONE || k.Cout <= 64) return false;
  } else if (k.epi != EPI_STORE || k.row_group != nullptr) {
    return false;
  }
  if (k.Kpad % 32 != 0 || k.Kpad < 32 || k.Kpad > 256 || k.C % 4 != 0 || k.M <= 0) return false;
  if ((size_t)k.M * (size_t)k.out_ld * 4 >= (size_t)OOB_OFFSET || (size_t)k.M * (size_t)k.res_ld * 4 >= (size_t)OOB_OFFSET) return false;
  if (w_bytes >= (size_t)OOB_OFFSET) return false;
  if (k.ln_g != nullptr && (k.C != k.Kpad || k.ln_b == nullptr || (k.Kpad != 128 && k.Kpad != 192))) return false;
  return true;
}

bool gemm_takes_astat(int M, int K, const ConvW& w, bool with_res, int ld) {
  ConvK k{};
  k.KH = k.KW = k.stride = k.stride_w = 1;
  k.epi = EPI_STORE;
  k.Kpad = w.kpad;
  k.C = K;
  k.M = M;
  k.out_ld = ld;
  k.res_ld = with_res ? ld : 0;
  return w.kh == 1 && w.kw == 1 && w.mode == 0 && conv2d_f16_astat_can(k, (size_t)((w.cout + 255) / 256 * 256) * w.kpad * 4);
}

bool conv2d_f16_astat(hipStream_t s, ConvK& k, const void* planes, size_t w_bytes) {
  if (!conv2d_f16_astat_can(k, w_bytes)) return false;
  const bool narrow = astat_narrow(k);
  const int bn = narrow ? 64 : 128;
  k.ntiles_n = (k.Cout + bn - 1) / bn;
  const int mblocks = (k.M + 127) / 128;
  int groups = 1;
  while (mblocks * groups < 512 && groups * 2 <= k.ntiles_n) groups *= 2;
  if (k.epi == EPI_ROWMAX && !g_astat_rowmax_dealt.load(std::memory_order_relaxed)) groups = k.ntiles_n;
  const int kt = k.Kpad / 32;
  if (k.epi == EPI_ROWMAX) {
    switch (kt) {
      case 1: launch_astat<128, 1, false, true>(s, k, planes, w_bytes, groups); break;
      case 2: launch_astat<128, 2, false, true>(s, k, planes, w_bytes, groups); break;
      case 3: launch_astat<128, 3, false, true>(s, k, planes, w_bytes, groups); break;
      case 4: launch_astat<128, 4, false, true>(s, k, planes, w_bytes, groups); break;
      case 5: launch_astat<128, 5, false, true>(s, k, planes, w_bytes, groups); break;
      default: launch_astat<128, 6, false, true>(s, k, planes, w_bytes, groups); break;
    }
  } else if (k.ln_g != nullptr) {
    switch (kt) {
      case 4: launch_astat<64, 4, true>(s, k, planes, w_bytes, groups); break;
      case 6: launch_astat<64, 6, true>(s, k, planes, w_bytes, groups); break;
      default: return false;
    }
  } else if (narrow) {
    switch (kt) {
      case 1: launch_astat<64, 1, false>(s, k, planes, w_bytes, groups); break;
      case 2: launch_astat<64, 2, false>(s, k, planes, w_bytes, groups); break;
      case 3: launch_astat<64, 3, false>(s, k, planes, w_bytes, groups); break;
      case 4: launch_astat<64, 4, false>(s, k, planes, w_bytes, groups); break;
      case 5: launch_astat<64, 5, false>(s, k, planes, w_bytes, groups); break;
// ... 19 lines not shown
```

### yomitoku_amd/csrc/ymk_conv_kernel.h

```cpp
#pragma once
#include <utility>

#include "ymk_common.h"

namespace ymk {

typedef float f32x16 __attribute__((ext_vector_type(16)));

struct ConvK {
  const float* in;
  const float* w;
  const float* scale;
  const float* bias;
  const float* res;
  float* out;
  int H, W, C, in_ld;
  int OH, OW, Cout, out_ld, res_ld, res_post;
  int KH, KW, stride, stride_w, pad, dil;
  int Kpad, ctiles, mode;
  int M;
  int act, epi;
  int ntiles_n;
  unsigned in_bytes;
  int vec;
  const int* row_group;
  const int* group_open;
  int fast;
  const unsigned* amax;
  unsigned* amax_out;
  const float* ln_g;
  const float* ln_b;
  float ln_eps;
  int in_planes, out_planes;
  float pl_a, pl_b;
};

template <int BM, int NT>
__device__ __forceinline__ bool tile_needed(const ConvK& p, int m0, int t) {
  if (!p.row_group) return true;
  int live = 0;
  for (int r = t; r < BM; r += NT) {
    const int m = m0 + r;
    if (m < p.M && p.group_open[p.row_group[m]] != 0) live = 1;
  }
  return __syncthreads_or(live) != 0;
}

__device__ __forceinline__ float apply_act(float v, int act) {
  switch (act) {
    case ACT_RELU: return fmaxf(v, 0.f);
    case ACT_SILU: return v / (1.f + expf(-v));
    case ACT_SIGMOID: return 1.f / (1.f + expf(-v));
    case ACT_GELU: return gelu_f32(v);
    default: return v;
  }
}

__device__ __forceinline__ float2 f16_plane_scales(unsigned amax_bits) {
  int e = (int)(amax_bits >> 23);
  e = e < 27 ? 27 : (e > 227 ? 227 : e);
  float2 r;
  r.x = __uint_as_float((unsigned)(268 - e) << 23);
  r.y = __uint_as_float((unsigned)(e - 14) << 23);
  return r;
}

constexpr int LDK = 36;

constexpr int lds_row(int opt) { return (opt & 2) ? 32 : LDK; }
constexpr int blocks_per_cu(int bm, int bn, int opt) {
  const int bytes = 2 * (bm + bn) * lds_row(opt) * 4;
  return 3 * bytes <= 160 * 1024 ? 3 : 2 * bytes <= 160 * 1024 ? 2 : 1;
}
template <int OPT>
__device__ __forceinline__ int lds_slot(int row, int slot) {
  if (OPT & 2) return (row >> 1) * 64 + ((((row & 1) << 3) | slot) ^ ((row >> 1) & 7)) * 4;
  return row * LDK + slot * 4;
}

typedef unsigned int u32x4 __attribute__((ext_vector_type(4)));
typedef float f32x4 __attribute__((ext_vector_type(4)));
constexpr unsigned OOB_OFFSET = 0xFFFFFFF0u;
constexpr unsigned SPLITK_OOB_ROW = 0xC0000000u;

template <int BM, int BN, int NT>
struct EpiRows {
  static constexpr int TPR = BN / 4, RPP = NT / TPR, NR = (BM + RPP - 1) / RPP;
};

template <int BM, int BN, int NT>
__device__ __forceinline__ void prefetch_residual(const ConvK& p, int m0, int n0, int t, float4* rr) {
  using E = EpiRows<BM, BN, NT>;
  const int c4 = t % E::TPR, r0 = t / E::TPR;
  const int co = n0 + c4 * 4;
#pragma unroll
  for (int i = 0; i < E::NR; ++i) {
    const int m = m0 + r0 + E::RPP * i;
    rr[i] = (co < p.Cout && m < p.M && r0 + E::RPP * i < BM) ? *reinterpret_cast<const float4*>(p.res + (size_t)m * p.res_ld + co)
                                                         : make_float4(0.f, 0.f, 0.f, 0.f);
  }
}

template <int BM, int BN, int NT, bool PRE = false, int UNROLL = 4, bool PL = false>
__device__ __forceinline__ void epilogue_tile(const ConvK& p, const float* Cs, int m0, int n0, int t, const float4* pre = nullptr) {
  constexpr int LDC = BN + 4;
  if constexpr (PL) {
    typedef _Float16 ep_h2 __attribute__((ext_vector_type(2)));
    typedef float ep_f2 __attribute__((ext_vector_type(2)));
    constexpr int TPR = BN / 4, RPP = NT / TPR;
    const int c4 = t % TPR, r0 = t / TPR;
    const int co = n0 + c4 * 4;
    const unsigned bound_bits = __float_as_uint(fmaf(__uint_as_float(amax_read(p.amax, t)), p.pl_a, p.pl_b));
    const float so = f16_plane_scales(bound_bits).x;
    if (co < p.Cout) {
      const float4 sc = p.scale ? *reinterpret_cast<const float4*>(p.scale + co) : make_float4(1.f, 1.f, 1.f, 1.f);
      const float4 bi = p.bias ? *reinterpret_cast<const float4*>(p.bias + co) : make_float4(0.f, 0.f, 0.f, 0.f);
      char* const obase = reinterpret_cast<char*>(p.out) + (size_t)(co >> 5) * 128 + (size_t)(co & 31) * 2;
#pragma unroll 4
      for (int i = 0; i < EpiRows<BM, BN, NT>::NR; ++i) {
        const int row = r0 + RPP * i;
        const int m = m0 + row;
        if (row >= BM || m >= p.M) break;
        float4 v = *reinterpret_cast<const float4*>(Cs + row * LDC + c4 * 4);
        v.x = apply_act(v.x * sc.x + bi.x, p.act);
        v.y = apply_act(v.y * sc.y + bi.y, p.act);
        v.z = apply_act(v.z * sc.z + bi.z, p.act);
        v.w = apply_act(v.w * sc.w + bi.w, p.act);
        ep_f2 a = {v.x * so, v.y * so}, b = {v.z * so, v.w * so};
        const ep_h2 ha = __builtin_convertvector(a, ep_h2), hb = __builtin_convertvector(b, ep_h2);
        a -= __builtin_convertvector(ha, ep_f2);
        b -= __builtin_convertvector(hb, ep_f2);
        const ep_h2 la = __builtin_convertvector(a, ep_h2), lb = __builtin_convertvector(b, ep_h2);
        char* o = obase + (size_t)m * p.out_ld * 4;
        *reinterpret_cast<uint2*>(o) = make_uint2(__builtin_bit_cast(unsigned, ha), __builtin_bit_cast(unsigned, hb));
        *reinterpret_cast<uint2*>(o + 64) = make_uint2(__builtin_bit_cast(unsigned, la), __builtin_bit_cast(unsigned, lb));
      }
    }
    if (p.amax_out) amax_commit(p.amax_out, bound_bits, t);
    return;
  }
  const float4 zero4 = make_float4(0.f, 0.f, 0.f, 0.f);
  constexpr int TPR = BN / 4;
  constexpr int RPP = NT / TPR;
  const int c4 = t % TPR, r0 = t / TPR;
  const int co = n0 + c4 * 4;
  if (p.epi == EPI_ROWMAX) {
    constexpr int G = (BN < ROWMAX_TILE_N ? BN : ROWMAX_TILE_N) / 4;
    const int ntn = (p.Cout + ROWMAX_TILE_N - 1) / ROWMAX_TILE_N, tn = co / ROWMAX_TILE_N;
    for (int row = r0; row < BM; row += RPP) {
      float best = -INFINITY;
      int bi = 0x7fffffff;
#pragma unroll
      for (int e = 0; e < 4; ++e) {
        const int c = co + e;
        if (c < p.Cout) {
          const float v = Cs[row * LDC + c4 * 4 + e] * (p.scale ? p.scale[c] : 1.f) + (p.bias ? p.bias[c] : 0.f);
          if (v > best) {
            best = v;
            bi = c;
          }
        }
      }
#pragma unroll
      for (int o = G / 2; o > 0; o >>= 1) {
        const float ov = __shfl_xor(best, o);
        const int oi = __shfl_xor(bi, o);
        if (ov > best || (ov == best && oi < bi)) {
          best = ov;
          bi = oi;
        }
      }
      const int m = m0 + row;
      if ((c4 & (G - 1)) == 0 && m < p.M && co < p.Cout) {
        float2 pr;
        pr.x = best;
        pr.y = __int_as_float(bi);
        *reinterpret_cast<float2*>(p.out + ((size_t)m * ntn + tn) * 2) = pr;
      }
    }
    return;
  }
  unsigned am = 0u;
  const bool live = co < p.Cout;
  const int ohw = p.OH * p.OW;
  if (live && p.vec) {
    float4 sc = make_float4(1.f, 1.f, 1.f, 1.f), bi = zero4;
    if (p.scale) sc = *reinterpret_cast<const float4*>(p.scale + co);
    if (p.bias) bi = *reinterpret_cast<const float4*>(p.bias + co);
    int cq = co, ab = 0;
    if (p.epi == EPI_DECONV2X2) {
      const int cq_n = p.Cout >> 2;
      ab = co / cq_n;
      cq = co - ab * cq_n;
    }
#pragma unroll(PRE ? EpiRows<BM, BN, NT>::NR : UNROLL)
    for (int i = 0; i < EpiRows<BM, BN, NT>::NR; ++i) {
      const int row = r0 + RPP * i;
      const int m = m0 + row;
      if (row >= BM || m >= p.M) break;
      float4 v = *reinterpret_cast<const float4*>(Cs + row * LDC + c4 * 4);
      v.x = v.x * sc.x + bi.x;
      v.y = v.y * sc.y + bi.y;
      v.z = v.z * sc.z + bi.z;
      v.w = v.w * sc.w + bi.w;
      size_t o;
      float4 rr = zero4;
      if (p.epi == EPI_STORE) {
        if (p.res) {
          rr = PRE ? pre[i] : *reinterpret_cast<const float4*>(p.res + (size_t)m * p.res_ld + co);
          if (!p.res_post) {
            v.x += rr.x; v.y += rr.y; v.z += rr.z; v.w += rr.w;
          }
        }
        o = (size_t)m * p.out_ld + co;
      } else {
        const int n = m / ohw, rem = m - n * ohw;
        const int oh = rem / p.OW, ow = rem - oh * p.OW;
        const size_t opix = ((size_t)n * (2 * p.OH) + 2 * oh + (ab >> 1)) * (2 * p.OW) + 2 * ow + (ab & 1);
        o = opix * p.out_ld + cq;
      }
      v.x = apply_act(v.x, p.act);
      v.y = apply_act(v.y, p.act);
      v.z = apply_act(v.z, p.act);
      v.w = apply_act(v.w, p.act);
      if (p.res_post) {
        v.x += rr.x; v.y += rr.y; v.z += rr.z; v.w += rr.w;
      }
      *reinterpret_cast<float4*>(p.out + o) = v;
      amax_fold4(am, v);
      if (PRE) __builtin_amdgcn_sched_barrier(0);
    }
  } else if (live) {
    for (int row = r0; row < BM; row += RPP) {
      const int m = m0 + row;
      if (m >= p.M) break;
      for (int e = 0; e < 4 && co + e < p.Cout; ++e) {
        float v = Cs[row * LDC + c4 * 4 + e];
        v = v * (p.scale ? p.scale[co + e] : 1.f) + (p.bias ? p.bias[co + e] : 0.f);
        const float rr = p.res ? p.res[(size_t)m * p.res_ld + co + e] : 0.f;
        if (!p.res_post) v += rr;
        v = apply_act(v, p.act);
        if (p.res_post) v += rr;
        p.out[(size_t)m * p.out_ld + co + e] = v;
        amax_fold(am, v);
      }
    }
  }
  if (p.amax_out) amax_commit(p.amax_out, am, t);
}

template <int ACT, int TM, int TN>
__device__ __forceinline__ void epilogue_direct_act(const ConvK& p, const f32x16 (&acc)[TM][TN], int mw, int nw, int li, int lh) {
  unsigned am = 0u;
#pragma unroll
  for (int b = 0; b < TN; ++b) {
    const int co = nw + 32 * b + li;
    const bool cok = co < p.Cout;
    const float sc = (p.scale && cok) ? p.scale[co] : 1.f;
    const float bi = (p.bias && cok) ? p.bias[co] : 0.f;
#pragma unroll
    for (int a = 0; a < TM; ++a) {
      const int mb = mw + 32 * a + 4 * lh;
      const float* rp = p.res ? p.res + (size_t)mb * p.res_ld + co : nullptr;
      float* op = p.out + (size_t)mb * p.out_ld + co;
      float rr[16];
#pragma unroll
      for (int r = 0; r < 16; ++r) {
        const int dr = (r & 3) + 8 * (r >> 2);
        rr[r] = (rp && cok && mb + dr < p.M) ? rp[(size_t)dr * p.res_ld] : 0.f;
      }
#pragma unroll
      for (int r = 0; r < 16; ++r) {
        const int dr = (r & 3) + 8 * (r >> 2);
        float v = acc[a][b][r] * sc + bi;
        if (rp && !p.res_post) v += rr[r];
        v = apply_act(v, ACT);
        if (p.res_post) v += rr[r];
        if (cok && mb + dr < p.M) {
          op[(size_t)dr * p.out_ld] = v;
          amax_fold(am, v);
        }
      }
    }
  }
// ... 23 lines not shown
```

### yomitoku_amd/csrc/ymk_conv_split.hip

```cpp
#include <atomic>
#include <string>
#include <type_traits>
#include <unordered_map>

#include "ymk_conv_kernel.h"

namespace ymk {

typedef __bf16 bf16x2_t __attribute__((ext_vector_type(2)));
typedef __bf16 bf16x8_t __attribute__((ext_vector_type(8)));
typedef _Float16 f16x2_t __attribute__((ext_vector_type(2)));
typedef _Float16 f16x8_t __attribute__((ext_vector_type(8)));
typedef float f32x2_t __attribute__((ext_vector_type(2)));

template <int FMT> struct Half;
template <> struct Half<0> { typedef bf16x2_t v2; typedef bf16x8_t v8; };
template <> struct Half<1> { typedef f16x2_t v2; typedef f16x8_t v8; };

template <int FMT>
__device__ __forceinline__ f32x16 mfma16(const typename Half<FMT>::v8 a, const typename Half<FMT>::v8 b, const f32x16 c) {
  if constexpr (FMT == 0) return __builtin_amdgcn_mfma_f32_32x32x16_bf16(a, b, c, 0, 0, 0);
  else return __builtin_amdgcn_mfma_f32_32x32x16_f16(a, b, c, 0, 0, 0);
}

template <int FMT, int NS>
__device__ __forceinline__ void split4(const f32x4 v, float sa, uint2* planes) {
  typedef typename Half<FMT>::v2 h2;
  f32x2_t a = {v.x, v.y}, b = {v.z, v.w};
  if (FMT == 1) {
    a *= sa;
    b *= sa;
  }
#pragma unroll
  for (int pl = 0; pl < NS; ++pl) {
    const h2 pa = __builtin_convertvector(a, h2), pb = __builtin_convertvector(b, h2);
    planes[pl].x = __builtin_bit_cast(unsigned, pa);
    planes[pl].y = __builtin_bit_cast(unsigned, pb);
    if (pl + 1 < NS) {
      a -= __builtin_convertvector(pa, f32x2_t);
      b -= __builtin_convertvector(pb, f32x2_t);
    }
  }
}

__device__ __forceinline__ float2 f16_scales(unsigned amax_bits) { return f16_plane_scales(amax_bits); }

template <int BM, int BN, int WM, int WN, int NS, int KS>
constexpr int bf16_waves_per_simd() {
  constexpr int lds = 2 * (BM + BN) * (KS * NS * 64 + 16);
  constexpr int blocks = 2 * lds <= 160 * 1024 ? 2 : 1;
  return blocks * 64 * WM * WN / 256;
}

template <int BM, int BN, int WM, int WN, int NS, int KS, int PF, int FMT, bool OPL = false>
__global__ __launch_bounds__(64 * WM * WN, (bf16_waves_per_simd<BM, BN, WM, WN, NS, KS>())) void conv_igemm_split(ConvK p, const uint4* __restrict__ wsplit) {
  typedef typename Half<FMT>::v8 h8;
  static_assert(PF >= 1 && PF <= 3, "prefetch: 1 = one stage ahead, 2 = two ahead, 3 = two ahead with the LDS stores threaded through the MFMAs");
  constexpr int NSET = PF == 1 ? 1 : 2;
  constexpr int NT = 64 * WM * WN;
  constexpr int WTM = BM / WM, WTN = BN / WN;
  constexpr int TM = WTM / 32, TN = WTN / 32;
  constexpr int TILEB = NS * 64;
  constexpr int ROWB = KS * TILEB + 16;
  constexpr int STAGE_B = (BM + BN) * ROWB;
  constexpr int RPP = NT / 8;
  constexpr int APASS = BM / RPP;
  static_assert(BM % RPP == 0, "tile rows must divide by the staging pass");
  constexpr int PPR = NS * 4;
  constexpr int BPASS = (BN * PPR + NT - 1) / NT;
  constexpr int LDC = BN + 4;
  constexpr int ECAP = 2 * STAGE_B / 4 / LDC;
  constexpr int EROWS = ECAP >= BM ? BM : (ECAP >= BM / 2 ? BM / 2 : BM / 4);
  static_assert(EROWS >= WTM && EROWS % WTM == 0 && EROWS <= ECAP, "an epilogue pass must hold whole wave tiles");
  __shared__ __attribute__((aligned(16))) char lds[2 * STAGE_B];

  const int t = threadIdx.x;
  float sa = 1.f, inv_sa = 1.f;
  if (FMT == 1) {
    const float2 sc = f16_scales((unsigned)__builtin_amdgcn_readfirstlane((int)amax_read(p.amax, t)));
    sa = sc.x;
    inv_sa = sc.y;
  }
  int tile;
  {
    const int nblk = gridDim.x, bid = blockIdx.x;
    const int xcd = bid & 7, idx = bid >> 3, q = nblk >> 3, r = nblk & 7;
    tile = (xcd < r ? xcd * (q + 1) : r * (q + 1) + (xcd - r) * q) + idx;
  }
  const int tile_m = tile / p.ntiles_n, tile_n = tile - tile_m * p.ntiles_n;
  const int m0 = tile_m * BM, n0 = tile_n * BN;
  if (!tile_needed<BM, NT>(p, m0, t)) return;

  const int colq = t & 7, rowb = t >> 3;
  int pixb[APASS], ih0[APASS], iw0[APASS];
  const bool pointwise = (p.fast & 1) && p.KH == 1 && p.KW == 1 && p.stride == 1 && p.stride_w == 1 && p.pad == 0;
#pragma unroll
  for (int i = 0; i < APASS; ++i) {
    const int m = m0 + rowb + RPP * i;
    if (m < p.M && pointwise) {
      pixb[i] = m;
      ih0[i] = 0;
      iw0[i] = 0;
    } else if (m < p.M) {
      const int ohw = p.OH * p.OW;
      const int n = m / ohw, rem = m - n * ohw;
      const int oh = rem / p.OW, ow = rem - oh * p.OW;
      pixb[i] = n * p.H * p.W;
// ... 189 lines not shown
  store_stage(0, 0);
  if (PF >= 2 && nstages > 1) load_stage(1, 1);
  __syncthreads();
  if (PF == 3) {
    for (int st = 0; st < nstages; st += 2) {
      if (st + 2 < nstages) load_stage(st + 2, 0);
      if (st + 1 < nstages) compute_store(0, 1, NSET - 1, std::true_type{});
      else compute_store(0, 1, NSET - 1, std::false_type{});
      __syncthreads();
      if (st + 1 >= nstages) break;
      if (st + 3 < nstages) load_stage(st + 3, NSET - 1);
      if (st + 2 < nstages) compute_store(1, 0, 0, std::true_type{});
      else compute_store(1, 0, 0, std::false_type{});
      __syncthreads();
    }
  } else if (PF == 1) {
    for (int st = 0; st < nstages; ++st) {
      const int buf = st & 1;
      if (st + 1 < nstages) load_stage(st + 1, 0);
      compute(buf);
      if (st + 1 < nstages) store_stage(buf ^ 1, 0);
      __syncthreads();
    }
  } else {
    for (int st = 0; st < nstages; st += 2) {
      if (st + 2 < nstages) load_stage(st + 2, 0);
      compute(0);
      if (st + 1 < nstages) store_stage(1, NSET - 1);
      __syncthreads();
      if (st + 1 >= nstages) break;
      if (st + 3 < nstages) load_stage(st + 3, NSET - 1);
      compute(1);
      if (st + 2 < nstages) store_stage(0, 0);
      __syncthreads();
    }
  }

  float* Cs = reinterpret_cast<float*>(lds);
#pragma unroll
  for (int e0 = 0; e0 < BM; e0 += EROWS) {
    if (e0 > 0) __syncthreads();
    if (wm * WTM >= e0 && wm * WTM < e0 + EROWS) {
#pragma unroll
      for (int a = 0; a < TM; ++a)
#pragma unroll
        for (int b = 0; b < TN; ++b)
#pragma unroll
          for (int r = 0; r < 16; ++r) {
            const int row = wm * WTM - e0 + a * 32 + (r & 3) + 8 * (r >> 2) + 4 * lh;
            Cs[row * LDC + wn * WTN + b * 32 + li] = FMT == 1 ? acc[a][b][r] * inv_sa : acc[a][b][r];
          }
    }
    __syncthreads();
    epilogue_tile<EROWS, BN, NT, false, 4, OPL>(p, Cs, m0 + e0, n0, t);
  }
}

template <int NS>
__global__ void k_split_panel(const float* __restrict__ w, unsigned short* __restrict__ out, size_t n_elems, int kpad) {
  const size_t i = (size_t)blockIdx.x * blockDim.x + threadIdx.x;
  if (i >= n_elems) return;
  const size_t row = i / kpad;
  const int k = (int)(i - row * kpad), kt = k >> 5, kk = k & 31;
  float r = w[i];
#pragma unroll
  for (int pl = 0; pl < NS; ++pl) {
    const __bf16 h = (__bf16)r;
    out[((row * (kpad >> 5) + kt) * NS + pl) * 32 + kk] = __builtin_bit_cast(unsigned short, h);
    r -= (float)h;
  }
}

__global__ void k_split_panel_f16(const float* __restrict__ w, unsigned short* __restrict__ out, int kpad, const float* __restrict__ scale,
                                  int cout, float* __restrict__ scale_out, int taps, int ctiles, int perm) {
  __shared__ unsigned red[4];
  const int row = blockIdx.x, t = threadIdx.x;
  const float* wr = w + (size_t)row * kpad;
  unsigned m = 0;
  for (int k = t; k < kpad; k += 256) m = max(m, __float_as_uint(fabsf(wr[k])));
#pragma unroll
  for (int o = 32; o > 0; o >>= 1) m = max(m, (unsigned)__shfl_xor((int)m, o));
  if ((t & 63) == 0) red[t >> 6] = m;
  __syncthreads();
  m = max(max(red[0], red[1]), max(red[2], red[3]));
  const float2 sc = f16_scales(m);
  for (int k = t; k < kpad; k += 256) {
    const int kt_src = k >> 5;
    int kk = k & 31;
    const int tap = kt_src / ctiles, cc = kt_src - tap * ctiles;
    const int kt = cc * taps + tap;
    if (perm) {
      const int rem = kk & 15;
      kk = (kk & 16) | (((rem >> 2) & 1) << 3) | ((rem >> 3) << 2) | (rem & 3);
    }
    float r = wr[k] * sc.x;
    const _Float16 h = (_Float16)r;
    r -= (float)h;
    const _Float16 l = (_Float16)r;
    unsigned short* o = out + (((size_t)row * (kpad >> 5) + kt) * 2) * 32 + kk;
    o[0] = __builtin_bit_cast(unsigned short, h);
    o[32] = __builtin_bit_cast(unsigned short, l);
  }
  if (t == 0 && row < cout) scale_out[row] = (scale ? scale[row] : 1.f) * sc.y;
}

__global__ __launch_bounds__(256) void k_absmax(const float* __restrict__ in, size_t items, int c4, int ld, unsigned* __restrict__ slot,
                                                unsigned* __restrict__ next) {
// ... 165 lines not shown
  SplitCtx* ctx = split_ctx.get();
  int code;
  {
    ConvSplitScope scope(conv_split(), ctx, SPLIT_MODEL_DEFAULT);
    code = conv_effective_split();
  }
  ctx->prebuild(nullptr, pool.convs(), pool.perm_convs(), code);
  const int enc = (int)param("conv_split_encoder", -1);
  if (enc > 0 && enc != code) ctx->prebuild(nullptr, pool.convs(), pool.perm_convs(), enc);
  YMK_HIP(hipStreamSynchronize(nullptr));
}

static void amax_verify(hipStream_t s, const ConvK& k, SplitCtx* ctx) {
  if (!g_amax_counters) {
    YMK_HIP(hipMalloc((void**)&g_amax_counters, 4 * sizeof(unsigned long long)));
    YMK_HIP(hipMemset(g_amax_counters, 0, 4 * sizeof(unsigned long long)));
  }
  const unsigned* truth = ctx->absmax(s, k);
  hipLaunchKernelGGL(k_amax_verify, dim3(1), dim3(64), 0, s, k.amax, truth, g_amax_counters);
  if (g_amax_check.load(std::memory_order_relaxed) >= 2) {
    unsigned got[AMAX_REC_WORDS], want[AMAX_REC_WORDS];
    YMK_HIP(hipStreamSynchronize(s));
    YMK_HIP(hipMemcpy(got, k.amax, sizeof(got), hipMemcpyDeviceToHost));
    YMK_HIP(hipMemcpy(want, truth, sizeof(want), hipMemcpyDeviceToHost));
    unsigned g = 0, w = 0;
    for (int i = 0; i < AMAX_LINES; ++i) {
      g = std::max(g, got[i * AMAX_LINE_WORDS]);
      w = std::max(w, want[i * AMAX_LINE_WORDS]);
    }
    if (g < w) {
      float gf, wf;
      std::memcpy(&gf, &g, 4);
      std::memcpy(&wf, &w, 4);
      std::fprintf(stderr, "amax_check: record BELOW the truth: %g < %g  M=%d C=%d ld=%d Cout=%d k=%dx%d stride=%d H=%d W=%d act=%d res=%d rec=%p in=%p\n", gf, wf,
                   k.M, k.C, k.in_ld, k.Cout, k.KH, k.KW, k.stride, k.H, k.W, k.act, k.res ? 1 : 0, (const void*)k.amax, (const void*)k.in);
    }
  }
}

template <int FMT, int BM, int BN, int WM, int WN, int NS, int KS = 1, int PF = 1, bool OPL = false>
static void launch_split(hipStream_t s, ConvK& k, const void* wsplit, SplitCtx* ctx = nullptr) {
  if (KS > 1 && (k.Kpad >> 5) % KS != 0) {
    launch_split<FMT, BM, BN, WM, WN, NS, 1, PF, OPL>(s, k, wsplit, ctx);
    return;
  }
  const int mt = (k.M + BM - 1) / BM, nt = (k.Cout + BN - 1) / BN;
  k.ntiles_n = nt;
  auto* e = conv_prof_open(s, k, BM, BN, mt * nt, (FMT ? 160 : 10 * NS));
  if (FMT == 1 && k.amax == nullptr) {
    k.amax = ctx->absmax(s, k);
  } else if (FMT == 1 && g_amax_check.load(std::memory_order_relaxed)) {
    amax_verify(s, k, ctx);
  }
  hipLaunchKernelGGL((conv_igemm_split<BM, BN, WM, WN, NS, KS, PF, FMT, OPL>), dim3(mt * nt), dim3(64 * WM * WN), 0, s, k,
                     reinterpret_cast<const uint4*>(wsplit));
  if (e) YMK_HIP(hipEventRecord(e->second, s));
}

static std::atomic<int> g_split_tile{0};
static thread_local int t_split_tile = 0;
static int split_tile_now() { return t_split_tile != 0 ? t_split_tile : g_split_tile.load(std::memory_order_relaxed); }
ConvSplitTileScope::ConvSplitTileScope(int tile) : prev_(t_split_tile) { t_split_tile = tile; }
ConvSplitTileScope::~ConvSplitTileScope() { t_split_tile = prev_; }
static std::atomic<int> g_astat{1};
static std::atomic<int> g_act_planes{1};
static std::atomic<int> g_rowmax_tile{0};
static std::atomic<long long> g_n_astat{0}, g_n_ln_fused{0}, g_n_planes_read{0}, g_n_planes_written{0}, g_n_rowmax_wide{0};
long long vit_mlp_fused_launches();
bool conv_split_stat(const std::string& key, long long* value) {
  if (key == "astat_launches") *value = g_n_astat.load();
  else if (key == "ln_fused_launches") *value = g_n_ln_fused.load();
  else if (key == "planes_read_launches") *value = g_n_planes_read.load();
  else if (key == "planes_written_launches") *value = g_n_planes_written.load();
  else if (key == "rowmax_wide_launches") *value = g_n_rowmax_wide.load();
  else if (key == "mlp_fused_launches") *value = vit_mlp_fused_launches();
  else return false;
  return true;
}
void astat_rowmax_dealt(int on);
bool conv_split_debug_option(const std::string& key, int value) {
  if (key == "conv_split_tile") g_split_tile = value;
  else if (key == "amax_check") g_amax_check = value;
  else if (key == "astat") g_astat = value;
  else if (key == "act_planes") g_act_planes = value;
  else if (key == "rowmax_tile") {
    g_rowmax_tile = value;
    astat_rowmax_dealt(value == 4);
  }
  else return false;
  return true;
}

template <int NS>
static void dispatch_bf16(hipStream_t s, ConvK& k, const void* ws, int tile, bool narrow) {
  if (narrow) {
    launch_split<0, 128, 64, 4, 2, NS>(s, k, ws);
    return;
  }
  switch (tile) {
    case 2: launch_split<0, 256, 128, 4, 4, NS>(s, k, ws); break;
    case 4: launch_split<0, 128, 128, 4, 2, NS>(s, k, ws); break;
    case 5: launch_split<0, 128, 128, 4, 4, NS, NS == 2 ? 2 : 1, 1>(s, k, ws); break;
    case 6: launch_split<0, 128, 128, 4, 4, NS, NS == 2 ? 2 : 1, 2>(s, k, ws); break;
    case 7: launch_split<0, 128, 128, 4, 2, NS, NS == 2 ? 2 : 1, 2>(s, k, ws); break;
    case 8: launch_split<0, 256, 128, 4, 4, NS, 1, 2>(s, k, ws); break;
    case 9: launch_split<0, 128, 128, 4, 2, NS, 1, 2>(s, k, ws); break;
    case 10: launch_split<0, 128, 128, 4, 4, NS, 1, 2>(s, k, ws); break;
    case 12: launch_split<0, 128, 128, 4, 4, NS, 1, 3>(s, k, ws); break;
    case 13: launch_split<0, 256, 128, 4, 4, NS, 1, 3>(s, k, ws); break;
    case 14: launch_split<0, 128, 128, 4, 2, NS, 1, 3>(s, k, ws); break;
    case 11:
      if (NS == 2 && k.Cout >= 256) launch_split<0, 256, 256, 4, 4, 2>(s, k, ws);
      else launch_split<0, 128, 128, 4, 4, NS>(s, k, ws);
      break;
    default: launch_split<0, 128, 128, 4, 4, NS>(s, k, ws); break;
  }
}

static void dispatch_f16(hipStream_t s, ConvK& k, const void* ws, int tile, bool narrow, SplitCtx* ctx) {
  if (k.out_planes) {
    if (narrow) launch_split<1, 128, 64, 4, 2, 2, 1, 1, true>(s, k, ws, ctx);
    else launch_split<1, 128, 128, 4, 4, 2, 1, 1, true>(s, k, ws, ctx);
    return;
  }
  if (narrow) {
    launch_split<1, 128, 64, 4, 2, 2>(s, k, ws, ctx);
    return;
  }
  switch (tile) {
    case 2: launch_split<1, 256, 128, 4, 4, 2>(s, k, ws, ctx); break;
    case 4: launch_split<1, 128, 128, 4, 2, 2>(s, k, ws, ctx); break;
    case 11:
      if (k.Cout >= 256) launch_split<1, 256, 256, 4, 4, 2>(s, k, ws, ctx);
      else launch_split<1, 128, 128, 4, 4, 2>(s, k, ws, ctx);
      break;
    default: launch_split<1, 128, 128, 4, 4, 2>(s, k, ws, ctx); break;
  }
}

bool conv2d_f16_dma(hipStream_t s, ConvK& k, const void* wsplit, size_t w_bytes, bool narrow, int rows);

enum SplitRoute : int { ROUTE_NONE = 0, ROUTE_ASTAT = 1, ROUTE_DMA = 2, ROUTE_STAGED = 3 };
struct RouteQuery {
  long M;
  int cout, kpad, taps;
  bool rowmax, row_group, astat_can, ln, planes_io;
};
static SplitRoute route_f16(const RouteQuery& q, int& tile, bool& narrow) {
  const long mt128 = (q.M + 127) / 128;
  const long blocks128 = mt128 * ((q.cout + 127) / 128), blocks64 = mt128 * ((q.cout + 63) / 64);
  tile = split_tile_now();
  const bool auto_tile = tile == 0;
  const bool astat_forced = tile == 30;
  bool few = false;
  if (blocks128 < 256 && !astat_forced) {
    if (blocks64 < 256) return ROUTE_NONE;
    few = true;
  }
  if (tile == 0) tile = 3;
  const int rowmax_tile = q.rowmax && auto_tile && !few ? g_rowmax_tile.load(std::memory_order_relaxed) : 0;
  if (rowmax_tile == 2) tile = 4;
  if (rowmax_tile == 3) tile = 2;
  narrow = q.cout <= 64 || tile == 1 || (q.rowmax && (rowmax_tile < 1 || rowmax_tile > 3)) || few;
  if ((!q.rowmax || ((rowmax_tile == 0 || rowmax_tile == 4) && auto_tile)) && q.astat_can && !q.planes_io &&
      (astat_forced || q.ln || (auto_tile && g_astat.load(std::memory_order_relaxed) != 0 && q.cout > 64 && !few && q.kpad <= 192)))
    return ROUTE_ASTAT;
  if (q.ln) return ROUTE_NONE;
  if (tile == 30) {
    if (blocks128 < 256) return ROUTE_NONE;
    tile = 3;
  }
  const bool dma_shape = q.taps > 1 || (q.kpad >= 1024 && q.cout <= 512) || q.cout <= 64;
  const bool dma_fills = blocks128 >= 256 || (q.cout <= 64 && mt128 >= 256);
  if (!q.rowmax && !q.row_group && (tile == 20 || tile == 21 || (auto_tile && dma_shape && dma_fills))) return ROUTE_DMA;
  if (tile == 20 || tile == 21) tile = 3;
  return ROUTE_STAGED;
}

int conv_split_route_with_planes(long M, int cout, int kpad, int taps, bool* auto_tile) {
  int tile = 0;
  bool narrow = false;
  *auto_tile = split_tile_now() == 0 && g_act_planes.load(std::memory_order_relaxed) != 0;
  return (int)route_f16(RouteQuery{M, cout, kpad, taps, false, false, false, false, true}, tile, narrow);
}

bool conv2d_split(hipStream_t s, ConvK& k, const ConvW& w, int code, SplitCtx* ctx) {
  if (w.mode != 0 || ctx == nullptr || (code != 2 && code != 3 && code != SPLIT_F16X2)) return false;
  const bool planes_io = k.in_planes != 0 || k.out_planes != 0;
  if ((k.ln_g != nullptr || planes_io) && code != SPLIT_F16X2) return false;
  const bool rowmax = k.epi == EPI_ROWMAX;
  const size_t w_bytes_f16 = (size_t)((w.cout + 255) / 256 * 256) * w.kpad * 2 * 2;
  int tile = 0;
  bool narrow = false;
  SplitRoute route = ROUTE_STAGED;
  if (code == SPLIT_F16X2) {
    route = route_f16(RouteQuery{k.M, w.cout, k.Kpad, k.KH * k.KW, rowmax, k.row_group != nullptr, conv2d_f16_astat_can(k, w_bytes_f16),
                                 k.ln_g != nullptr, planes_io}, tile, narrow);
  } else {
    const long mt128 = (k.M + 127) / 128;
    const long blocks128 = mt128 * ((w.cout + 127) / 128), blocks64 = mt128 * ((w.cout + 63) / 64);
    tile = split_tile_now();
    if (tile == 0) tile = code == 3 ? 2 : 3;
    if (tile == 20 || tile == 21 || tile == 30) tile = 3;
    if (blocks128 < 256 && blocks64 < 256) return false;
    narrow = w.cout <= 64 || tile == 1 || rowmax || blocks128 < 256;
  }
  if (route == ROUTE_NONE) return false;
  YMK_CHECK(!k.in_planes || (route == ROUTE_DMA && tile != 20), "a tensor stored as fp16 planes reached a kernel that cannot read it");
  YMK_CHECK(!k.out_planes || (route == ROUTE_DMA && tile != 20) || (route == ROUTE_STAGED && (narrow || tile == 3)),
            "fp16 planes asked of a kernel that cannot write them");
  const SplitCtx::Panels& pn = ctx->panels(s, w, code);
  if (k.in_planes) ++g_n_planes_read;
  if (k.out_planes) ++g_n_planes_written;
  if (route == ROUTE_ASTAT) {
    k.scale = pn.scale;
    const int bn = conv2d_f16_astat_columns(k);
    auto* e = conv_prof_open(s, k, 128, bn, ((k.M + 127) / 128) * ((k.Cout + bn - 1) / bn), 162);
    if (k.amax == nullptr) k.amax = ctx->absmax(s, k);
    else if (g_amax_check.load(std::memory_order_relaxed) && k.ln_g == nullptr) amax_verify(s, k, ctx);
    const bool taken = conv2d_f16_astat(s, k, pn.planes, w_bytes_f16);
    if (e) YMK_HIP(hipEventRecord(e->second, s));
    YMK_HIP(hipGetLastError());
    YMK_CHECK(taken, "conv_f16_astat refused a launch it had accepted");
    ++g_n_astat;
    if (rowmax) ++g_n_rowmax_wide;
    if (k.ln_g != nullptr) ++g_n_ln_fused;
    return true;
  }
  if (route == ROUTE_DMA) {
    k.scale = pn.scale;
    const bool nar = w.cout <= 64;
    const int rows = tile == 20 ? 256 : 128;
    k.ntiles_n = (k.Cout + (nar ? 64 : 128) - 1) / (nar ? 64 : 128);
    auto* e = conv_prof_open(s, k, rows, nar ? 64 : 128, ((k.M + rows - 1) / rows) * k.ntiles_n, 161);
    YMK_CHECK(!k.in_planes || k.amax != nullptr, "a tensor of fp16 planes without the record that holds its scale");
    if (k.amax == nullptr) k.amax = ctx->absmax(s, k);
    else if (g_amax_check.load(std::memory_order_relaxed) && !k.in_planes) amax_verify(s, k, ctx);
    const bool taken = conv2d_f16_dma(s, k, pn.planes, w_bytes_f16, nar, rows);
    if (e) YMK_HIP(hipEventRecord(e->second, s));
    YMK_HIP(hipGetLastError());
    YMK_CHECK(taken, "conv_f16_dma refused a launch");
    return true;
  }
  if (code == SPLIT_F16X2) {
    k.scale = pn.scale;
    if (rowmax && !narrow) ++g_n_rowmax_wide;
    dispatch_f16(s, k, pn.planes, tile, narrow, ctx);
  } else if (code == 2) {
    dispatch_bf16<2>(s, k, pn.planes, tile, narrow);
  } else {
    dispatch_bf16<3>(s, k, pn.planes, tile, narrow);
  }
  YMK_HIP(hipGetLastError());
  return true;
}

struct MlpK {
  const float* x;
  float* out;
  int M, ld;
  const float *ln_g, *ln_b;
  float ln_eps, ln_bound;
  const uint4* w1;
  unsigned w1_bytes;
  const float *s1, *b1;
  const uint4* w2;
  unsigned w2_bytes;
  const float *s2, *b2;
  float g_bound;
};
bool vit_mlp_f16_launch(hipStream_t s, const MlpK& k, int D, int F);
std::pair<hipEvent_t, hipEvent_t>* conv_prof_open_raw(hipStream_t s, const char* desc, double flops, double bytes, double products);

static std::atomic<long long> g_n_mlp_fused{0};
long long vit_mlp_fused_launches() { return g_n_mlp_fused.load(); }

bool vit_mlp_split_launch(hipStream_t s, SplitCtx* ctx, float* x, int M, int ld, const float* ln_g, const float* ln_b, float ln_eps,
                          float ln_bound, const ConvW& fc1, const ConvW& fc2) {
  const int D = fc1.cin, F = fc1.cout;
  if (ctx == nullptr || fc1.mode != 0 || fc2.mode != 0 || fc1.kh * fc1.kw != 1 || fc2.kh * fc2.kw != 1) return false;
  if (fc2.cin != F || fc2.cout != D || fc1.kpad != D || fc2.kpad != F || fc1.scale != nullptr || fc2.scale != nullptr) return false;
  if (fc1.bias == nullptr || fc2.bias == nullptr || D != 192 || F != 768) return false;
  if ((M + 127) / 128 < 256) return false;
  const SplitCtx::Panels& p1 = ctx->panels(s, fc1, SPLIT_F16X2);
  const SplitCtx::Panels& p2 = ctx->panels(s, fc2, SPLIT_F16X2_PERM);
  MlpK k{};
  k.x = x;
  k.out = x;
  k.M = M;
  k.ld = ld;
  k.ln_g = ln_g;
  k.ln_b = ln_b;
  k.ln_eps = ln_eps;
  k.ln_bound = ln_bound;
  k.w1 = reinterpret_cast<const uint4*>(p1.planes);
  k.w1_bytes = (unsigned)((size_t)((F + 255) / 256 * 256) * fc1.kpad * 4);
  k.s1 = p1.scale;
  k.b1 = fc1.bias;
  k.w2 = reinterpret_cast<const uint4*>(p2.planes);
// ... 16 lines not shown
```

### yomitoku_amd/csrc/ymk_dbnet.cpp

```cpp
#include "ymk_common.h"

namespace ymk {

namespace {

struct Bottleneck {
  ConvW c1, c2, c3, down;
  bool has_down = false;
  int stride = 1, dil = 1;
};

class DBNetModel : public Model {
 public:
  const char* kind() const override { return "dbnet"; }

  void finalize() override {
    const std::string bb = "backbone.body.";
    stem_ = make_conv(pool, ws, bb + "conv1", bb + "bn1", true);
    const int nblocks[4] = {3, 4, 6, 3};
    for (int L = 0; L < 4; ++L) {
      layers_[L].clear();
      for (int i = 0; i < nblocks[L]; ++i) {
        const std::string p = bb + "layer" + std::to_string(L + 1) + "." + std::to_string(i) + ".";
        Bottleneck b;
// ... 11 lines not shown
    for (int L = 0; L < 4; ++L) {
      in_proj_[L] = make_conv(pool, ws, d + "input_proj.layer" + std::to_string(L + 1), "");
      out_proj_[L] = make_conv(pool, ws, d + "out_proj.layer" + std::to_string(L + 1) + (L == 0 ? "" : ".0"), "");
    }
    asf_conv_ = make_conv(pool, ws, d + "concat_attention.conv", "");
    const std::string ea = d + "concat_attention.enhanced_attention.";
    {
      const HostTensor& w1 = ws.get(ea + "channel_wise.1.weight");
      const HostTensor& w2 = ws.get(ea + "channel_wise.3.weight");
      asf_c_ = (int)w1.dims[1];
      asf_cmid_ = (int)w1.dims[0];
      YMK_CHECK(asf_c_ == 64 && (int)w2.dims[0] == 64, "ASF expects 64 inner channels");
      asf_w1_ = pool.upload(w1.data);
      asf_w2_ = pool.upload(w2.data);
      asf_sp33_ = pool.upload(ws.get(ea + "spatial_wise.0.weight").data);
      asf_sp11_ = ws.get(ea + "spatial_wise.2.weight").data[0];
      const HostTensor& wa = ws.get(ea + "attention_wise.0.weight");
      YMK_CHECK((int)wa.dims[0] == 4, "ASF expects 4 scales");
      asf_watt_ = pool.upload(wa.data);
    }
    bin_conv_ = make_conv(pool, ws, d + "binarize.0", d + "binarize.1");
    {
      const HostTensor& w = ws.get(d + "binarize.3.weight");
      const HostTensor& b = ws.get(d + "binarize.3.bias");
      const int ci = (int)w.dims[0], co = (int)w.dims[1];
      YMK_CHECK(w.dims[2] == 2 && w.dims[3] == 2, "binarize.3 must be a 2x2 transposed conv");
      const HostTensor& g = ws.get(d + "binarize.4.weight");
      const HostTensor& be = ws.get(d + "binarize.4.bias");
      const HostTensor& m = ws.get(d + "binarize.4.running_mean");
      const HostTensor& v = ws.get(d + "binarize.4.running_var");
      std::vector<float> sc(co), bi(co);
      for (int o = 0; o < co; ++o) {
        const float s = g.data[o] / std::sqrt(v.data[o] + 1e-5f);
        sc[o] = s;
        bi[o] = be.data[o] + (b.data[o] - m.data[o]) * s;
      }
      deconv1_ = make_deconv2x2_panel(pool, w.data.data(), ci, co, sc.data(), bi.data());
    }
    {
      const HostTensor& w = ws.get(d + "binarize.6.weight");
      YMK_CHECK(w.dims[0] == 64 && w.dims[1] == 1, "binarize.6 must be 64->1");
      deconv2_w_ = pool.upload(w.data);
      deconv2_b_ = ws.get(d + "binarize.6.bias").data[0];
    }
    ws.clear();
    finalized = true;
  }

  void forward(const float* x_nchw, int n, int h, int w, float* prob, hipStream_t s) {
    YMK_CHECK(finalized, "model not finalized");
    ForwardScope forward_scope;
    ConvSplitScope split_scope(conv_split(), split_ctx.get(), SPLIT_MODEL_DEFAULT);
    YMK_CHECK(n > 0 && h % 32 == 0 && w % 32 == 0 && h >= 32 && w >= 32, "dbnet input must be a multiple of 32");
    const uint64_t key = shape_key(n, h, w);
    if (sync_workspace_mode()) shape_key_ = 0;
    if (key != shape_key_) {
      size_t need = 0;
      if (!arena.plan_select(key, &need)) {
        arena.dry_run = true;
        arena.reset();
        run(x_nchw, n, h, w, prob, s);
        arena.dry_run = false;
        need = arena.plan_commit(key);
        arena.reset();
      }
      if (need > arena.capacity()) {
        forward_sync(s);
        arena.reserve(need);
      }
      shape_key_ = key;
    }
    arena.forward_begin();
    run(x_nchw, n, h, w, prob, s);
  }

  void reserve(int n, int h, int w, hipStream_t s) override {
    YMK_CHECK(finalized, "model not finalized");
    YMK_CHECK(n > 0 && h % 32 == 0 && w % 32 == 0 && h >= 32 && w >= 32, "dbnet reserve: sizes must be multiples of 32");
    sync_workspace_mode();
    size_t need = 0;
    for (int turn = 0; turn < 2; ++turn) {
      arena.dry_run = true;
      arena.reset();
      run(nullptr, n, turn ? w : h, turn ? h : w, nullptr, s);
      arena.dry_run = false;
      need = std::max(need, arena.plan_commit(shape_key(n, turn ? w : h, turn ? h : w), true));
      arena.reset();
    }
    if (need > arena.capacity() || arena.resize_pending()) {
      YMK_HIP(hipStreamSynchronize(s));
      arena.reserve(need);
    }
    shape_key_ = 0;
  }

 private:
  static uint64_t shape_key(int n, int h, int w) { return ((uint64_t)n << 40) | ((uint64_t)h << 20) | (uint64_t)w; }

  Tensor conv(hipStream_t s, const Tensor& in, const ConvW& w, int stride, int pad, int dil, int act,
              const Tensor* res = nullptr, const Tensor* into = nullptr, unsigned* rec = nullptr, bool out_planes = false) {
    Tensor out;
    if (into) {
      out = *into;
    } else {
      out = arena.tensor(in.n, conv_out_dim(in.h, w.kh, stride, pad, dil), conv_out_dim(in.w, w.kw, stride, pad, dil),
                         w.cout);
      out.amax = arena.amax_next();
    }
    if (rec) out.amax = rec;
    out.planes = out_planes && out.amax != nullptr;
    if (arena.dry_run) return out;
    ConvArgs a;
    a.stride = stride;
    a.pad = pad;
    a.dil = dil;
    a.act = act;
    a.res = res;
    a.out_planes = out.planes;
    conv2d(s, in, w, a, out);
    return out;
  }

  Tensor bottleneck(hipStream_t s, const Tensor& x, const Bottleneck& b) {
    ConvArgs a1, a2;
    a1.act = a2.act = ACT_RELU;
    a2.stride = b.stride;
    a2.pad = a2.dil = b.dil;
    const bool planes = conv_planes_pair_ok(x, b.c1, a1, b.c2, a2);
    Tensor t1 = conv(s, x, b.c1, 1, 0, 1, ACT_RELU, nullptr, nullptr, nullptr, planes);
    Tensor t2 = conv(s, t1, b.c2, b.stride, b.dil, b.dil, ACT_RELU);
    arena.release(t1);
    Tensor idn = x;
    if (b.has_down) idn = conv(s, x, b.down, b.stride, 0, 1, ACT_NONE);
    Tensor out = conv(s, t2, b.c3, 1, 0, 1, ACT_RELU, &idn);
    arena.release(t2);
    if (b.has_down) arena.release(idn);
    return out;
  }

  void run(const float* x_nchw, int n, int h, int w, float* prob, hipStream_t s) {
    const bool dry = arena.dry_run;
    arena.amax_begin(s, 96);
    Tensor x4 = arena.tensor(n, h, w, 4);
    if (!dry) nchw3_to_nhwc4(s, x_nchw, n, h, w, x4);
    Tensor c1 = conv(s, x4, stem_, 2, 3, 1, ACT_RELU);
    arena.release(x4);
    Tensor p = arena.tensor(n, (c1.h + 2 - 3) / 2 + 1, (c1.w + 2 - 3) / 2 + 1, c1.c);
    p.amax = c1.amax;
    if (!dry) maxpool3x3s2(s, c1, p);
    arena.release(c1);
    Tensor feat[4];
    Tensor cur = p;
    for (int L = 0; L < 4; ++L) {
      for (const Bottleneck& b : layers_[L]) {
        Tensor next = bottleneck(s, cur, b);
        if (L == 0 || cur.p != feat[L - 1].p) arena.release(cur);
        cur = next;
      }
      feat[L] = cur;
    }
    Tensor p4 = conv(s, feat[3], in_proj_[3], 1, 0, 1, ACT_NONE);
    arena.release(feat[3]);
    Tensor p3;
    if (feat[2].h == p4.h && feat[2].w == p4.w) {
      p3 = conv(s, feat[2], in_proj_[2], 1, 0, 1, ACT_NONE, &p4);
    } else {
      Tensor up = arena.tensor(n, feat[2].h, feat[2].w, p4.c);
      if (!dry) upsample_bilinear(s, p4, up, nullptr);
      p3 = conv(s, feat[2], in_proj_[2], 1, 0, 1, ACT_NONE, &up);
      arena.release(up);
    }
    arena.release(feat[2]);
    Tensor up3 = arena.tensor(n, feat[1].h, feat[1].w, p3.c);
    if (!dry) upsample_bilinear(s, p3, up3, nullptr);
    Tensor p2 = conv(s, feat[1], in_proj_[1], 1, 0, 1, ACT_NONE, &up3);
    arena.release(up3);
    arena.release(feat[1]);
    Tensor up2 = arena.tensor(n, feat[0].h, feat[0].w, p2.c);
    if (!dry) upsample_bilinear(s, p2, up2, nullptr);
    Tensor p1 = conv(s, feat[0], in_proj_[0], 1, 0, 1, ACT_NONE, &up2);
    arena.release(up2);
    arena.release(feat[0]);

    const int fh = p1.h, fw = p1.w;
    Tensor fuse = arena.tensor(n, fh, fw, 256);
    fuse.amax = arena.amax_next();
    {
      Tensor o4 = conv(s, p4, out_proj_[3], 1, 1, 1, ACT_NONE, nullptr, nullptr, fuse.amax);
      Tensor o3 = conv(s, p3, out_proj_[2], 1, 1, 1, ACT_NONE, nullptr, nullptr, fuse.amax);
      Tensor o2 = conv(s, p2, out_proj_[1], 1, 1, 1, ACT_NONE, nullptr, nullptr, fuse.amax);
      arena.release(p4);
      arena.release(p3);
      arena.release(p2);
      Tensor s0 = fuse.slice_c(0, 64), s1 = fuse.slice_c(64, 64), s2 = fuse.slice_c(128, 64), s3 = fuse.slice_c(192, 64);
      if (!dry) {
        YMK_CHECK(o4.h * 4 == fh && o3.h * 4 == fh && o2.h * 2 == fh, "decoder pyramid shape");
        upsample_bilinear(s, o4, s0, nullptr);
        upsample_bilinear(s, o3, s1, nullptr);
        upsample_bilinear(s, o2, s2, nullptr);
      }
      arena.release(o4);
      arena.release(o3);
      arena.release(o2);
      conv(s, p1, out_proj_[0], 1, 1, 1, ACT_NONE, nullptr, &s3);
      arena.release(p1);
    }
    Tensor ax = conv(s, fuse, asf_conv_, 1, 1, 1, ACT_NONE);
    float* gap_scr = arena.alloc_f((size_t)GAP_CHUNKS * n * 64);
    float* gap = arena.alloc_f((size_t)n * 64);
    float* gate = arena.alloc_f((size_t)n * 64);
    float* cmean = arena.alloc_f((size_t)n * fh * fw);
    Tensor fused = arena.tensor(n, fh, fw, 256);
    fused.amax = fuse.amax;
    if (!dry) asf_block(s, ax, asf_w1_, asf_w2_, asf_cmid_, asf_sp33_, asf_sp11_, asf_watt_, fuse, gap_scr, gap, gate, cmean, fused);
    arena.release(fuse);
    arena.release(ax);
    arena.release(gap_scr);
    arena.release(gap);
    arena.release(gate);
    arena.release(cmean);
    Tensor b0 = conv(s, fused, bin_conv_, 1, 1, 1, ACT_RELU);
    arena.release(fused);
    Tensor b1 = arena.tensor(n, 2 * fh, 2 * fw, 64);
    if (!dry) {
      ConvArgs a;
      a.act = ACT_RELU;
      a.epi = EPI_DECONV2X2;
      conv2d(s, b0, deconv1_, a, b1);
      YMK_CHECK(4 * fh == h && 4 * fw == w, "binarize output shape");
      deconv2x2_to1_sigmoid(s, b1, deconv2_w_, deconv2_b_, prob);
    }
  }

  ConvW stem_;
  std::vector<Bottleneck> layers_[4];
  ConvW in_proj_[4], out_proj_[4];
  ConvW asf_conv_, bin_conv_, deconv1_;
  float *asf_w1_ = nullptr, *asf_w2_ = nullptr, *asf_sp33_ = nullptr, *asf_watt_ = nullptr;
  float asf_sp11_ = 0.f;
  int asf_c_ = 64, asf_cmid_ = 16;
  float* deconv2_w_ = nullptr;
  float deconv2_b_ = 0.f;
  uint64_t shape_key_ = 0;
};

}

Model* create_dbnet() { return new DBNetModel(); }

void dbnet_forward(Model* m, const float* x, int n, int h, int w, float* prob, hipStream_t s) {
  auto* d = dynamic_cast<DBNetModel*>(m);
  YMK_CHECK(d != nullptr, "model is not a dbnet");
  d->forward(x, n, h, w, prob, s);
}

}
```

### yomitoku_amd/csrc/ymk_elem.hip

```cpp
#include "ymk_common.h"

namespace ymk {

static inline int grid_for(size_t work, int block = 256, int cap = 256 * 16) {
  size_t g = (work + block - 1) / block;
  if (g > (size_t)cap) g = cap;
  if (g == 0) g = 1;
  return (int)g;
}

__global__ void k_nchw3_to_nhwc4(const float* __restrict__ in, float4* __restrict__ out, size_t hw, size_t total) {
  for (size_t i = (size_t)blockIdx.x * blockDim.x + threadIdx.x; i < total; i += (size_t)gridDim.x * blockDim.x) {
    const size_t n = i / hw, r = i - n * hw;
    const float* b = in + n * 3 * hw + r;
    out[i] = make_float4(b[0], b[hw], b[2 * hw], 0.f);
  }
}
void nchw3_to_nhwc4(hipStream_t s, const float* in, int n, int h, int w, const Tensor& out) {
  YMK_CHECK(out.c == 4 && out.ld == 4, "nchw3_to_nhwc4 wants packed 4-channel output");
  const size_t hw = (size_t)h * w, total = hw * n;
  hipLaunchKernelGGL(k_nchw3_to_nhwc4, dim3(grid_for(total)), dim3(256), 0, s, in, (float4*)out.p, hw, total);
  YMK_HIP(hipGetLastError());
}

// ... 28 lines not shown
  YMK_CHECK(out.h == (in.h + 2 - 3) / 2 + 1 && out.w == (in.w + 2 - 3) / 2 + 1, "maxpool: shape");
  const size_t total = out.pixels() * (in.c / 4);
  hipLaunchKernelGGL(k_maxpool3x3s2, dim3(grid_for(total)), dim3(256), 0, s, in.p, out.p, in.h, in.w, in.c / 4, in.ld,
                     out.h, out.w, out.ld, total);
  YMK_HIP(hipGetLastError());
}

__global__ void k_avgpool2(const float* __restrict__ in, float* __restrict__ out, int H, int W, int C4, int in_ld,
                           int OH, int OW, int out_ld, size_t total) {
  for (size_t i = (size_t)blockIdx.x * blockDim.x + threadIdx.x; i < total; i += (size_t)gridDim.x * blockDim.x) {
    const int c4 = (int)(i % C4);
    size_t pix = i / C4;
    const int ow = (int)(pix % OW);
    pix /= OW;
    const int oh = (int)(pix % OH);
    const int n = (int)(pix / OH);
    float4 a = make_float4(0, 0, 0, 0);
    int cnt = 0;
    for (int dy = 0; dy < 2; ++dy) {
      const int ih = oh * 2 + dy;
      if (ih >= H) continue;
      for (int dx = 0; dx < 2; ++dx) {
        const int iw = ow * 2 + dx;
        if (iw >= W) continue;
        const float4 v = *reinterpret_cast<const float4*>(in + ((size_t)(n * H + ih) * W + iw) * in_ld + c4 * 4);
        a.x += v.x; a.y += v.y; a.z += v.z; a.w += v.w;
        ++cnt;
      }
    }
    const float d = (float)cnt;
    a.x /= d; a.y /= d; a.z /= d; a.w /= d;
    *reinterpret_cast<float4*>(out + ((size_t)(n * OH + oh) * OW + ow) * out_ld + c4 * 4) = a;
  }
}
void avgpool2x2_ceil(hipStream_t s, const Tensor& in, const Tensor& out) {
  YMK_CHECK(in.c % 4 == 0 && out.c == in.c, "avgpool: channels");
  YMK_CHECK(out.h == (in.h + 1) / 2 && out.w == (in.w + 1) / 2, "avgpool: shape");
  const size_t total = out.pixels() * (in.c / 4);
  hipLaunchKernelGGL(k_avgpool2, dim3(grid_for(total)), dim3(256), 0, s, in.p, out.p, in.h, in.w, in.c / 4, in.ld, out.h,
                     out.w, out.ld, total);
  YMK_HIP(hipGetLastError());
}

__global__ void k_bilinear(const float* __restrict__ in, const float* __restrict__ add, float* __restrict__ out, int H,
                           int W, int C4, int in_ld, int OH, int OW, int out_ld, int add_ld, float sh, float sw,
                           size_t total) {
  for (size_t i = (size_t)blockIdx.x * blockDim.x + threadIdx.x; i < total; i += (size_t)gridDim.x * blockDim.x) {
    const int c4 = (int)(i % C4);
    size_t pix = i / C4;
    const int ow = (int)(pix % OW);
    pix /= OW;
    const int oh = (int)(pix % OH);
    const int n = (int)(pix / OH);
    float fy = ((float)oh + 0.5f) * sh - 0.5f;
    float fx = ((float)ow + 0.5f) * sw - 0.5f;
    fy = fy < 0.f ? 0.f : fy;
    fx = fx < 0.f ? 0.f : fx;
    const int y0 = (int)fy, x0 = (int)fx;
    const int y1 = y0 + (y0 < H - 1 ? 1 : 0), x1 = x0 + (x0 < W - 1 ? 1 : 0);
    const float ly = fy - (float)y0, lx = fx - (float)x0;
    const float hy = 1.f - ly, hx = 1.f - lx;
    const float* b = in + (size_t)n * H * W * in_ld + c4 * 4;
    const float4 v00 = *reinterpret_cast<const float4*>(b + ((size_t)y0 * W + x0) * in_ld);
    const float4 v01 = *reinterpret_cast<const float4*>(b + ((size_t)y0 * W + x1) * in_ld);
    const float4 v10 = *reinterpret_cast<const float4*>(b + ((size_t)y1 * W + x0) * in_ld);
    const float4 v11 = *reinterpret_cast<const float4*>(b + ((size_t)y1 * W + x1) * in_ld);
    float4 r;
    r.x = hy * (hx * v00.x + lx * v01.x) + ly * (hx * v10.x + lx * v11.x);
    r.y = hy * (hx * v00.y + lx * v01.y) + ly * (hx * v10.y + lx * v11.y);
    r.z = hy * (hx * v00.z + lx * v01.z) + ly * (hx * v10.z + lx * v11.z);
    r.w = hy * (hx * v00.w + lx * v01.w) + ly * (hx * v10.w + lx * v11.w);
    const size_t opix = (size_t)(n * OH + oh) * OW + ow;
    if (add) {
      const float4 t = *reinterpret_cast<const float4*>(add + opix * add_ld + c4 * 4);
      r.x += t.x; r.y += t.y; r.z += t.z; r.w += t.w;
    }
    *reinterpret_cast<float4*>(out + opix * out_ld + c4 * 4) = r;
  }
}
void upsample_bilinear(hipStream_t s, const Tensor& in, const Tensor& out, const Tensor* add) {
  YMK_CHECK(in.c % 4 == 0 && out.c == in.c && in.n == out.n, "bilinear: channels");
  YMK_CHECK(out.ld % 4 == 0 && in.ld % 4 == 0, "bilinear: ld");
  const size_t total = out.pixels() * (in.c / 4);
  const float sh = (float)in.h / (float)out.h, sw = (float)in.w / (float)out.w;
  hipLaunchKernelGGL(k_bilinear, dim3(grid_for(total)), dim3(256), 0, s, in.p, add ? add->p : nullptr, out.p, in.h,
                     in.w, in.c / 4, in.ld, out.h, out.w, out.ld, add ? add->ld : 0, sh, sw, total);
  YMK_HIP(hipGetLastError());
}

__global__ void k_nearest2(const float* __restrict__ in, float* __restrict__ out, int H, int W, int C4, int in_ld,
                           int out_ld, size_t total) {
  const int OH = 2 * H, OW = 2 * W;
  for (size_t i = (size_t)blockIdx.x * blockDim.x + threadIdx.x; i < total; i += (size_t)gridDim.x * blockDim.x) {
    const int c4 = (int)(i % C4);
    size_t pix = i / C4;
    const int ow = (int)(pix % OW);
    pix /= OW;
    const int oh = (int)(pix % OH);
    const int n = (int)(pix / OH);
    const float4 v = *reinterpret_cast<const float4*>(in + ((size_t)(n * H + (oh >> 1)) * W + (ow >> 1)) * in_ld + c4 * 4);
    *reinterpret_cast<float4*>(out + ((size_t)(n * OH + oh) * OW + ow) * out_ld + c4 * 4) = v;
  }
}
void upsample_nearest2x(hipStream_t s, const Tensor& in, const Tensor& out) {
  YMK_CHECK(in.c % 4 == 0 && out.c == in.c && out.h == 2 * in.h && out.w == 2 * in.w, "nearest2x: shape");
  const size_t total = out.pixels() * (in.c / 4);
  hipLaunchKernelGGL(k_nearest2, dim3(grid_for(total)), dim3(256), 0, s, in.p, out.p, in.h, in.w, in.c / 4, in.ld, out.ld,
                     total);
  YMK_HIP(hipGetLastError());
}

__global__ void k_add_act(const float* __restrict__ a, const float* __restrict__ b, float* __restrict__ out, int C4,
                          int a_ld, int b_ld, int out_ld, int act, size_t total) {
  for (size_t i = (size_t)blockIdx.x * blockDim.x + threadIdx.x; i < total; i += (size_t)gridDim.x * blockDim.x) {
    const int c4 = (int)(i % C4);
    const size_t pix = i / C4;
    float4 x = *reinterpret_cast<const float4*>(a + pix * a_ld + c4 * 4);
    const float4 y = *reinterpret_cast<const float4*>(b + pix * b_ld + c4 * 4);
    x.x += y.x; x.y += y.y; x.z += y.z; x.w += y.w;
    if (act == ACT_RELU) {
      x.x = fmaxf(x.x, 0.f); x.y = fmaxf(x.y, 0.f); x.z = fmaxf(x.z, 0.f); x.w = fmaxf(x.w, 0.f);
    }
    *reinterpret_cast<float4*>(out + pix * out_ld + c4 * 4) = x;
  }
// ... 212 lines not shown
```

Measured before the change: 127.0.

## Fuse FPN bilinear upsample into lateral conv and deconv-to-1 into deconv epilogue

The DBNet FPN lateral 1x1 convs now read the coarser level directly and blend the 2x bilinear upsample in the conv epilogue, so the upsampled intermediate is never materialised. The binarize head's second deconv (64->1 plus sigmoid) is folded into the first deconv's epilogue, which removes the 64-channel 2x-resolution intermediate and its separate kernel. Both are meant to cut HBM traffic and launches at high resolution. The cost is new epilogue template variants (XE) that disable residual prefetch and the DMA route, force a tile width for the to1 path, and add extra arithmetic in the epilogue.

```diff
diff --git a/include/ymk.h b/include/ymk.h
--- a/include/ymk.h
+++ b/include/ymk.h
@@ -102,6 +102,10 @@
 int ymk_op_deconv2x2(const float* x_dev, int n, int h, int w, int cin, const float* w_host, int cout, const float* scale_host,
                      const float* bias_host, int act, float* y_dev, void* stream);
 int ymk_op_deconv2x2_to1_sigmoid(const float* x_dev, int n, int h, int w, const float* w_host, float bias, float* y_dev, void* stream);
+int ymk_op_deconv2x2_to1_fused(const float* x_dev, int n, int h, int w, int cin, const float* w1_host, const float* scale_host,
+                               const float* bias_host, const float* w2_host, float bias2, int fused, float* y_dev, void* stream);
+int ymk_op_conv1x1_res_up2(const float* x_dev, int n, int h, int w, int cin, const float* w_host_oc, int cout, const float* bias_host,
+                           const float* top_dev, int fused, float* y_dev, int* fused_out, void* stream);
 int ymk_op_dbnet_asf(const float* ax_dev, const float* fuse_dev, int n, int h, int w, const float* w1_host, const float* w2_host,
                      int cmid, const float* sp33_host, float sp11, const float* watt_host, float* out_dev, void* stream);
 
diff --git a/yomitoku_amd/_lib.py b/yomitoku_amd/_lib.py
--- a/yomitoku_amd/_lib.py
+++ b/yomitoku_amd/_lib.py
@@ -107,6 +107,14 @@
         [c_void_p, c_int, c_int, c_int, c_int, c_void_p, c_int, c_void_p, c_void_p, c_int, c_void_p, c_void_p],
     ),
     "ymk_op_deconv2x2_to1_sigmoid": (c_int, [c_void_p, c_int, c_int, c_int, c_void_p, c_float, c_void_p, c_void_p]),
+    "ymk_op_deconv2x2_to1_fused": (
+        c_int,
+        [c_void_p, c_int, c_int, c_int, c_int, c_void_p, c_void_p, c_void_p, c_void_p, c_float, c_int, c_void_p, c_void_p],
+    ),
+    "ymk_op_conv1x1_res_up2": (
+        c_int,
+        [c_void_p, c_int, c_int, c_int, c_int, c_void_p, c_int, c_void_p, c_void_p, c_int, c_void_p, c_void_p, c_void_p],
+    ),
     "ymk_op_dbnet_asf": (
         c_int,
         [c_void_p, c_void_p, c_int, c_int, c_int, c_void_p, c_void_p, c_int, c_void_p, c_float, c_void_p, c_void_p, c_void_p],
diff --git a/yomitoku_amd/csrc/ymk_api.cpp b/yomitoku_amd/csrc/ymk_api.cpp
--- a/yomitoku_amd/csrc/ymk_api.cpp
+++ b/yomitoku_amd/csrc/ymk_api.cpp
@@ -25,6 +25,7 @@
 bool decstep_debug_option(const std::string& key, int value);
 bool conv_split_debug_option(const std::string& key, int value);
 bool conv_split_stat(const std::string& key, long long* value);
+bool conv_stat(const std::string& key, long long* value);
 bool parseq_stat(const std::string& key, long long* value);
 void amax_check_counters(long long* out4);
 }
@@ -235,7 +236,7 @@
   YMK_API_BEGIN
   YMK_CHECK(key != nullptr && value != nullptr, "null argument");
   long long v = 0;
-  YMK_CHECK(ymk::conv_split_stat(std::string(key), &v) || ymk::runtime_stat(std::string(key), &v) || ymk::parseq_stat(std::string(key), &v), std::string("unknown counter: ") + key);
+  YMK_CHECK(ymk::conv_split_stat(std::string(key), &v) || ymk::conv_stat(std::string(key), &v) || ymk::runtime_stat(std::string(key), &v) || ymk::parseq_stat(std::string(key), &v), std::string("unknown counter: ") + key);
   *value = v;
   YMK_API_END
 }
@@ -602,6 +603,67 @@
   YMK_API_END
 }
 
+int ymk_op_conv1x1_res_up2(const float* x_dev, int n, int h, int w, int cin, const float* w_host_oc, int cout, const float* bias_host,
+                           const float* top_dev, int fused, float* y_dev, int* fused_out, void* stream) {
+  YMK_API_BEGIN
+  using namespace ymk;
+  YMK_CHECK(x_dev && w_host_oc && top_dev && y_dev && n >= 1 && h >= 2 && w >= 2 && h % 2 == 0 && w % 2 == 0, "conv1x1_res_up2: bad argument");
+  YMK_CHECK(cin >= 4 && cin % 4 == 0 && cout >= 4 && cout % 4 == 0, "conv1x1_res_up2: cin and cout must be positive multiples of 4");
+  DevicePool pool;
+  const ConvW cw = make_linear_raw(pool, w_host_oc, bias_host, cout, cin);
+  Tensor in{const_cast<float*>(x_dev), n, h, w, cin, cin};
+  Tensor out{y_dev, n, h, w, cout, cout};
+  Tensor top{const_cast<float*>(top_dev), n, h / 2, w / 2, cout, cout};
+  SplitCtxOwner split_ctx;
+  ConvSplitScope scope(-1, split_ctx.get(), 0);
+  ConvArgs a;
+  const bool fuse = fused != 0 && conv_res_up2_ok(in, cw, a, top);
+  if (fused_out) *fused_out = fuse ? 1 : 0;
+  Tensor up = out;
+  if (fuse) {
+    a.res = &top;
+    a.res_up2 = true;
+  } else {
+    if (fused != 0) note_res_up2_fallback();
+    up.p = pool.alloc((size_t)n * h * w * cout);
+    upsample_bilinear((hipStream_t)stream, top, up, nullptr);
+    a.res = &up;
+  }
+  conv2d((hipStream_t)stream, in, cw, a, out);
+  YMK_HIP(hipStreamSynchronize((hipStream_t)stream));
+  YMK_API_END
+}
+
+int ymk_op_deconv2x2_to1_fused(const float* x_dev, int n, int h, int w, int cin, const float* w1_host, const float* scale_host,
+                               const float* bias_host, const float* w2_host, float bias2, int fused, float* y_dev, void* stream) {
+  YMK_API_BEGIN
+  using namespace ymk;
+  YMK_CHECK(x_dev && w1_host && w2_host && y_dev && n >= 1 && h >= 1 && w >= 1 && cin >= 4 && cin % 4 == 0, "deconv2x2_to1_fused: bad argument");
+  DevicePool pool;
+  const ConvW cw = make_deconv2x2_panel(pool, w1_host, cin, 64, scale_host, bias_host);
+  const float* w2 = pool.upload(w2_host, 64 * 4);
+  Tensor in{const_cast<float*>(x_dev), n, h, w, cin, cin};
+  SplitCtxOwner split_ctx;
+  ConvSplitScope scope(-1, split_ctx.get(), 0);
+  ConvArgs a;
+  a.act = ACT_RELU;
+  if (fused != 0) {
+    a.epi = EPI_DECONV2X2_TO1;
+    a.to1_w = w2;
+    a.to1_b = bias2;
+    const Tensor pr{y_dev, n, 4 * h, 4 * w, 1, 1};
+    conv2d((hipStream_t)stream, in, cw, a, pr);
+  } else {
+    Tensor mid{pool.alloc((size_t)n * 4 * h * w * 64), n, 2 * h, 2 * w, 64, 64};
+    a.epi = EPI_DECONV2X2;
+    conv2d((hipStream_t)stream, in, cw, a, mid);
+    deconv2x2_to1_sigmoid((hipStream_t)stream, mid, w2, bias2, y_dev);
+    note_deconv_to1_unfused();
+  }
+  YMK_HIP(hipStreamSynchronize((hipStream_t)stream));
+  YMK_API_END
+}
+
 int ymk_op_deconv2x2_to1_sigmoid(const float* x_dev, int n, int h, int w, const float* w_host, float bias, float* y_dev,
                                  void* stream) {
   YMK_API_BEGIN
diff --git a/yomitoku_amd/csrc/ymk_common.h b/yomitoku_amd/csrc/ymk_common.h
--- a/yomitoku_amd/csrc/ymk_common.h
+++ b/yomitoku_amd/csrc/ymk_common.h
@@ -133,6 +133,29 @@
   return m;
 }
 
+__device__ __forceinline__ void bilinear_src(int o, float scale, int size, int& i0, int& i1, float& l) {
+  float f = ((float)o + 0.5f) * scale - 0.5f;
+  f = f < 0.f ? 0.f : f;
+  i0 = (int)f;
+  i1 = i0 + (i0 < size - 1 ? 1 : 0);
+  l = f - (float)i0;
+}
+__device__ __forceinline__ float bilinear_blend(float hy, float ly, float hx, float lx, float a, float b, float c, float d) {
+#pragma clang fp contract(off)
+  const float top = __builtin_fmaf(hx, a, lx * b);
+  const float bot = __builtin_fmaf(hx, c, lx * d);
+  return __builtin_fmaf(ly, bot, hy * top);
+}
+__device__ __forceinline__ float4 bilinear_blend4(float ly, float lx, const float4 v00, const float4 v01, const float4 v10, const float4 v11) {
+  const float hy = 1.f - ly, hx = 1.f - lx;
+  float4 r;
+  r.x = bilinear_blend(hy, ly, hx, lx, v00.x, v01.x, v10.x, v11.x);
+  r.y = bilinear_blend(hy, ly, hx, lx, v00.y, v01.y, v10.y, v11.y);
+  r.z = bilinear_blend(hy, ly, hx, lx, v00.z, v01.z, v10.z, v11.z);
+  r.w = bilinear_blend(hy, ly, hx, lx, v00.w, v01.w, v10.w, v11.w);
+  return r;
+}
+
 enum Act : int { ACT_NONE = 0, ACT_RELU = 1, ACT_SILU = 2, ACT_SIGMOID = 3, ACT_GELU = 4 };
 
 __device__ __forceinline__ float gelu_f32(float v) {
@@ -159,7 +182,7 @@
   float pl_a = 0.f, pl_b = 0.f;
 };
 
-enum Epi : int { EPI_STORE = 0, EPI_DECONV2X2 = 1, EPI_ROWMAX = 2 };
+enum Epi : int { EPI_STORE = 0, EPI_DECONV2X2 = 1, EPI_ROWMAX = 2, EPI_DECONV2X2_TO1 = 3 };
 constexpr int ROWMAX_TILE_N = 64;
 
 struct ConvArgs {
@@ -169,6 +192,9 @@
   int epi = EPI_STORE;
   const Tensor* res = nullptr;
   bool res_post = false;
+  bool res_up2 = false;
+  const float* to1_w = nullptr;
+  float to1_b = 0.f;
   const int* row_group = nullptr;
   const int* group_open = nullptr;
   const unsigned* amax_in = nullptr;
@@ -211,6 +237,12 @@
 void conv2d(hipStream_t s, const Tensor& in, const ConvW& w, const ConvArgs& a, const Tensor& out);
 
 bool conv_planes_pair_ok(const Tensor& in, const ConvW& w1, const ConvArgs& a1, const ConvW& w2, const ConvArgs& a2);
+
+bool conv_res_up2_ok(const Tensor& in, const ConvW& w, const ConvArgs& a, const Tensor& res);
+void note_res_up2_fallback();
+bool dbnet_fuse_up2();
+bool dbnet_fuse_to1();
+void note_deconv_to1_unfused();
 
 void gemm(hipStream_t s, const float* A, int M, int K, int lda, const ConvW& w, int act, const float* res, int res_ld,
           float* out, int out_ld, const int* row_group = nullptr, const int* group_open = nullptr, int epi = EPI_STORE,
diff --git a/yomitoku_amd/csrc/ymk_conv.hip b/yomitoku_amd/csrc/ymk_conv.hip
--- a/yomitoku_amd/csrc/ymk_conv.hip
+++ b/yomitoku_amd/csrc/ymk_conv.hip
@@ -6,7 +6,7 @@
 
 namespace ymk {
 
-template <int BM, int BN, int WM, int WN, int MODE, int PF = 1, int OPT = 0>
+template <int BM, int BN, int WM, int WN, int MODE, int PF = 1, int OPT = 0, bool XE = false>
 __global__ __launch_bounds__(64 * WM * WN, ((OPT & 2) ? blocks_per_cu(BM, BN, OPT) : 2 * (BM + BN) * LDK * 4 <= 80 * 1024 ? 2 : 1) * WM * WN / 4) void conv_igemm(ConvK p) {
   static_assert(PF == 1 || PF == 2, "prefetch distance 1 or 2");
   constexpr int LDR = lds_row(OPT);
@@ -175,7 +175,7 @@
 
   using Epi = EpiRows<EROWS, BN, NT>;
   constexpr bool CAN_PRE = PF == 1 && EROWS == BM && Epi::NR <= 8 && NT <= 512;
-  const bool pre_res = CAN_PRE && (p.fast & 2) && p.res != nullptr && p.vec && p.epi == EPI_STORE;
+  const bool pre_res = CAN_PRE && !XE && (p.fast & 2) && p.res != nullptr && p.vec && p.epi == EPI_STORE;
   float4 rpre[CAN_PRE ? Epi::NR : 1];
   if (PF == 1) {
     for (int kt = 0; kt < ktiles; ++kt) {
@@ -221,11 +221,11 @@
     }
     __syncthreads();
     if (CAN_PRE && pre_res) epilogue_tile<EROWS, BN, NT, true>(p, Cs, m0 + e0, n0, t, rpre);
-    else epilogue_tile<EROWS, BN, NT>(p, Cs, m0 + e0, n0, t);
-  }
-}
-
-template <int TM, int TN, int NW, int PF>
+    else epilogue_tile<EROWS, BN, NT, false, 4, false, XE>(p, Cs, m0 + e0, n0, t);
+  }
+}
+
+template <int TM, int TN, int NW, int PF, bool XE = false>
 __global__ __launch_bounds__(64 * NW) void conv_splitk(ConvK p) {
   constexpr int BM = 32 * TM, BN = 32 * TN, NT = 64 * NW;
   constexpr int LDC = BN + 4;
@@ -375,7 +375,7 @@
         }
   }
   __syncthreads();
-  epilogue_tile<BM, BN, NT>(p, red, m0, n0, t);
+  epilogue_tile<BM, BN, NT, false, 4, false, XE>(p, red, m0, n0, t);
 }
 
 struct ProfState {
@@ -397,6 +397,9 @@
 static std::atomic<int> g_conv_variant{0};
 static std::atomic<int> g_prof_dump{0};
 static std::atomic<int> g_conv_split{-1};
+static std::atomic<int> g_dbnet_fuse_up2{1};
+static std::atomic<int> g_dbnet_fuse_to1{1};
+static std::atomic<long long> g_n_res_up2{0}, g_n_res_up2_fallback{0}, g_n_deconv_to1_fused{0}, g_n_deconv_to1_unfused{0};
 static std::atomic<int> g_gemm_row_limit{0};
 static int gemm_row_limit() { return g_gemm_row_limit.load(std::memory_order_relaxed); }
 static int splitk_forced() { return g_splitk_force.load(std::memory_order_relaxed); }
@@ -430,6 +433,20 @@
   else if (key == "prof_dump") g_prof_dump = value;
   else if (key == "conv_split") g_conv_split = value;
   else if (key == "gemm_row_limit") g_gemm_row_limit = value;
+  else if (key == "dbnet_fuse_up2") g_dbnet_fuse_up2 = value;
+  else if (key == "dbnet_fuse_to1") g_dbnet_fuse_to1 = value;
+  else return false;
+  return true;
+}
+bool dbnet_fuse_up2() { return g_dbnet_fuse_up2.load(std::memory_order_relaxed) != 0; }
+bool dbnet_fuse_to1() { return g_dbnet_fuse_to1.load(std::memory_order_relaxed) != 0; }
+void note_deconv_to1_unfused() { ++g_n_deconv_to1_unfused; }
+void note_res_up2_fallback() { ++g_n_res_up2_fallback; }
+bool conv_stat(const std::string& key, long long* value) {
+  if (key == "res_up2_launches") *value = g_n_res_up2.load();
+  else if (key == "res_up2_fallbacks") *value = g_n_res_up2_fallback.load();
+  else if (key == "deconv_to1_fused_launches") *value = g_n_deconv_to1_fused.load();
+  else if (key == "deconv_to1_unfused_launches") *value = g_n_deconv_to1_unfused.load();
   else return false;
   return true;
 }
@@ -491,7 +508,8 @@
     g_prof.flop += fl;
     const double images = (double)k.M / ((double)k.OH * k.OW);
     const double outs = (double)k.M * k.Cout;
-    const double by = 4.0 * (images * k.H * k.W * creal + (double)k.Cout * k.KH * k.KW * creal + outs * (k.res ? 2.0 : 1.0));
+    const double by = 4.0 * (images * k.H * k.W * creal + (double)k.Cout * k.KH * k.KW * creal +
+                             (k.epi == EPI_DECONV2X2_TO1 ? 16.0 * k.M : outs * (k.res ? (k.res_up2 ? 1.25 : 2.0) : 1.0)));
     g_prof.bytes += by;
     char buf[176];
     snprintf(buf, sizeof buf, "M=%7d Cin=%4d Cout=%4d k=%dx%d s=%d d=%d res=%d tile=%dx%d ksplit=%d grid=%d", k.M, k.C, k.Cout,
@@ -541,12 +559,15 @@
   return e;
 }
 
+static bool conv_xe(const ConvK& k) { return k.res_up2 != 0 || k.epi == EPI_DECONV2X2_TO1; }
+
 template <int TM, int TN, int NW, int PF>
 static void launch_splitk(hipStream_t s, ConvK& k) {
   const int mt = (k.M + 32 * TM - 1) / (32 * TM), nt = (k.Cout + 32 * TN - 1) / (32 * TN);
   k.ntiles_n = nt;
   auto* e = conv_prof_open(s, k, 32 * TM, 32 * TN, mt * nt, NW);
-  hipLaunchKernelGGL((conv_splitk<TM, TN, NW, PF>), dim3(mt * nt), dim3(64 * NW), 0, s, k);
+  if (conv_xe(k)) hipLaunchKernelGGL((conv_splitk<TM, TN, NW, PF, true>), dim3(mt * nt), dim3(64 * NW), 0, s, k);
+  else hipLaunchKernelGGL((conv_splitk<TM, TN, NW, PF>), dim3(mt * nt), dim3(64 * NW), 0, s, k);
   if (e) YMK_HIP(hipEventRecord(e->second, s));
 }
 
@@ -564,6 +585,7 @@
   const Cand* best = nullptr;
   double best_cost = 0.0;
   for (const Cand& c : cands) {
+    if (k.epi == EPI_DECONV2X2_TO1 && c.tn != 2) continue;
     const long blocks = (long)((k.M + 32 * c.tm - 1) / (32 * c.tm)) * ((k.Cout + 32 * c.tn - 1) / (32 * c.tn));
     const long waves = blocks * c.nw;
     const double per_wave = (double)((ktiles + c.nw - 1) / c.nw) * c.tm * c.tn * 1024.0 + 3000.0 + (c.nw == 8 ? 1800.0 : 1200.0);
@@ -574,7 +596,7 @@
     }
   }
   const int forced = splitk_forced();
-  if (forced >= 0) best = &cands[forced % (int)(sizeof(cands) / sizeof(cands[0]))];
+  if (forced >= 0 && k.epi != EPI_DECONV2X2_TO1) best = &cands[forced % (int)(sizeof(cands) / sizeof(cands[0]))];
   best->fn(s, k);
   return true;
 }
@@ -590,6 +612,14 @@
   const bool swz = HAS_SWZ && (k.fast & 8);
   auto* e = conv_prof_open(s, k, BM, BN, mt * nt, 1);
   const dim3 grid(mt * nt), block(64 * WM * WN);
+  if (conv_xe(k)) {
+    if constexpr (HAS_SWZ) {
+      if (swz) hipLaunchKernelGGL((conv_igemm<BM, BN, WM, WN, MODE, PF, 2, true>), grid, block, 0, s, k);
+    }
+    if (!swz) hipLaunchKernelGGL((conv_igemm<BM, BN, WM, WN, MODE, PF, 0, true>), grid, block, 0, s, k);
+    if (e) YMK_HIP(hipEventRecord(e->second, s));
+    return;
+  }
   if constexpr (HAS_SWZ) {
     if (swz && direct) hipLaunchKernelGGL((conv_igemm<BM, BN, WM, WN, MODE, PF, 3>), grid, block, 0, s, k);
     else if (swz) hipLaunchKernelGGL((conv_igemm<BM, BN, WM, WN, MODE, PF, 2>), grid, block, 0, s, k);
@@ -642,6 +672,9 @@
   k.res = a.res ? a.res->p : nullptr;
   k.res_ld = a.res ? a.res->ld : 0;
   k.res_post = a.res_post ? 1 : 0;
+  k.res_up2 = a.res_up2 ? 1 : 0;
+  k.to1_w = a.to1_w;
+  k.to1_b = a.to1_b;
   k.out = out.p;
   k.H = in.h;
   k.W = in.w;
@@ -666,7 +699,7 @@
   k.row_group = a.row_group;
   k.group_open = a.group_open;
   k.amax = in.amax ? in.amax : a.amax_in;
-  k.amax_out = a.epi == EPI_ROWMAX ? nullptr : (out.amax ? out.amax : a.amax_out);
+  k.amax_out = a.epi == EPI_ROWMAX || a.epi == EPI_DECONV2X2_TO1 ? nullptr : (out.amax ? out.amax : a.amax_out);
   YMK_CHECK((a.row_group == nullptr) == (a.group_open == nullptr), "conv: row_group and group_open come together");
   YMK_CHECK(w.w != nullptr, "conv weight not packed");
   if (w.mode == 0) {
@@ -681,8 +714,16 @@
     YMK_CHECK(out.ld == 2 * ((w.cout + ROWMAX_TILE_N - 1) / ROWMAX_TILE_N), "row-max epilogue: out must be [M][2 * ceil(Cout / 64)]");
   } else if (a.epi == EPI_STORE) {
     YMK_CHECK(out.n == in.n && out.h == k.OH && out.w == k.OW && out.c == w.cout, "conv: bad output shape");
-    if (a.res && a.res->ld != 0)
+    if (a.res_up2)
+      YMK_CHECK(a.res && !a.res_post && a.res->ld >= out.c && a.res->n == out.n && 2 * a.res->h == out.h && 2 * a.res->w == out.w &&
+                    a.res->c == out.c && a.row_group == nullptr,
+                "conv: res_up2 wants a residual [n][oh / 2][ow / 2][cout] added before the activation");
+    else if (a.res && a.res->ld != 0)
       YMK_CHECK(a.res->n == out.n && a.res->h == out.h && a.res->w == out.w && a.res->c == out.c, "conv: bad residual shape");
+  } else if (a.epi == EPI_DECONV2X2_TO1) {
+    YMK_CHECK(w.kh == 1 && w.kw == 1 && a.stride == 1 && a.pad == 0 && w.cout == 256, "deconv-to-1 epilogue wants a 1x1 panel of 4 x 64 columns");
+    YMK_CHECK(out.n == in.n && out.h == 4 * in.h && out.w == 4 * in.w && out.c == 1 && out.ld == 1, "deconv-to-1: out is the plane [n][4h][4w]");
+    YMK_CHECK(a.to1_w != nullptr && a.res == nullptr && a.row_group == nullptr, "deconv-to-1: weights of the final layer, no residual");
   } else {
     YMK_CHECK(w.kh == 1 && w.kw == 1 && a.stride == 1 && a.pad == 0, "deconv epilogue wants a 1x1 panel");
     YMK_CHECK(out.n == in.n && out.h == 2 * in.h && out.w == 2 * in.w && out.c * 4 == w.cout, "deconv: bad output shape");
@@ -700,6 +741,15 @@
     k.vec = (cq % 4 == 0) && (out.ld % 4 == 0) && al16(out.p) && (!w.scale || al16(w.scale)) &&
             (!w.bias || al16(w.bias)) && (!a.res || (a.res->ld % 4 == 0 && al16(a.res->p)));
     if (a.epi == EPI_DECONV2X2) YMK_CHECK(k.vec, "deconv epilogue needs 16 B aligned channels");
+    if (a.epi == EPI_DECONV2X2_TO1) {
+      k.vec = ((uintptr_t)out.p & 7) == 0 && (!w.scale || al16(w.scale)) && (!w.bias || al16(w.bias)) && al16(a.to1_w);
+      YMK_CHECK(k.vec, "deconv-to-1 epilogue needs an 8 B aligned plane and 16 B aligned weights");
+      ++g_n_deconv_to1_fused;
+    }
+    if (a.res_up2) {
+      YMK_CHECK(k.vec, "res_up2 needs 16 B aligned channel groups");
+      ++g_n_res_up2;
+    }
   }
   k.fast = g_conv_fast.load(std::memory_order_relaxed);
 
@@ -748,6 +798,20 @@
 }
 
 int conv_split_route_with_planes(long M, int cout, int kpad, int taps, bool* auto_tile);
+int conv_split_route_plain(long M, int cout, int kpad, int taps, bool pointwise);
+
+bool conv_res_up2_ok(const Tensor& in, const ConvW& w, const ConvArgs& a, const Tensor& res) {
+  const int sw = a.stride_w > 0 ? a.stride_w : a.stride;
+  const int oh = conv_out_dim(in.h, w.kh, a.stride, a.pad, a.dil), ow = conv_out_dim(in.w, w.kw, sw, a.pad, a.dil);
+  bool ok = a.epi == EPI_STORE && !a.res_post && a.row_group == nullptr && a.ln_g == nullptr && !a.out_planes && w.cout % 4 == 0 &&
+            res.ld % 4 == 0 && res.c == w.cout && res.n == in.n && 2 * res.h == oh && 2 * res.w == ow;
+  if (ok && conv_effective_split() == SPLIT_F16X2 && t_split_ctx != nullptr && w.mode == 0) {
+    const bool pointwise = w.kh == 1 && w.kw == 1 && a.stride == 1 && sw == 1 && a.pad == 0;
+    const int route = conv_split_route_plain((long)in.n * oh * ow, w.cout, w.kpad, w.kh * w.kw, pointwise);
+    if (route == 1 || route == 2) ok = false;
+  }
+  return ok;
+}
 
 bool conv_planes_pair_ok(const Tensor& in, const ConvW& w1, const ConvArgs& a1, const ConvW& w2, const ConvArgs& a2) {
   if (conv_effective_split() != SPLIT_F16X2 || t_split_ctx == nullptr) return false;
diff --git a/yomitoku_amd/csrc/ymk_conv_astat.hip b/yomitoku_amd/csrc/ymk_conv_astat.hip
--- a/yomitoku_amd/csrc/ymk_conv_astat.hip
+++ b/yomitoku_amd/csrc/ymk_conv_astat.hip
@@ -328,7 +328,7 @@
   if (k.KH != 1 || k.KW != 1 || k.stride != 1 || k.stride_w != 1 || k.pad != 0) return false;
   if (k.epi == EPI_ROWMAX) {
     if (k.Kpad > 192 || k.res != nullptr || k.ln_g != nullptr || k.act != ACT_NONE || k.Cout <= 64) return false;
-  } else if (k.epi != EPI_STORE || k.row_group != nullptr) {
+  } else if (k.epi != EPI_STORE || k.row_group != nullptr || k.res_up2) {
     return false;
   }
   if (k.Kpad % 32 != 0 || k.Kpad < 32 || k.Kpad > 256 || k.C % 4 != 0 || k.M <= 0) return false;
diff --git a/yomitoku_amd/csrc/ymk_conv_kernel.h b/yomitoku_amd/csrc/ymk_conv_kernel.h
--- a/yomitoku_amd/csrc/ymk_conv_kernel.h
+++ b/yomitoku_amd/csrc/ymk_conv_kernel.h
@@ -33,6 +33,9 @@
   float ln_eps;
   int in_planes, out_planes;
   float pl_a, pl_b;
+  int res_up2;
+  const float* to1_w;
+  float to1_b;
 };
 
 template <int BM, int NT>
@@ -101,7 +104,7 @@
   }
 }
 
-template <int BM, int BN, int NT, bool PRE = false, int UNROLL = 4, bool PL = false>
+template <int BM, int BN, int NT, bool PRE = false, int UNROLL = 4, bool PL = false, bool XE = false>
 __device__ __forceinline__ void epilogue_tile(const ConvK& p, const float* Cs, int m0, int n0, int t, const float4* pre = nullptr) {
   constexpr int LDC = BN + 4;
   if constexpr (PL) {
@@ -188,11 +191,88 @@
     if (p.scale) sc = *reinterpret_cast<const float4*>(p.scale + co);
     if (p.bias) bi = *reinterpret_cast<const float4*>(p.bias + co);
     int cq = co, ab = 0;
-    if (p.epi == EPI_DECONV2X2) {
+    if (p.epi == EPI_DECONV2X2 || (XE && p.epi == EPI_DECONV2X2_TO1)) {
       const int cq_n = p.Cout >> 2;
       ab = co / cq_n;
       cq = co - ab * cq_n;
     }
+    if (XE && p.epi == EPI_DECONV2X2_TO1) {
+      if constexpr (XE && BN % 64 == 0) {
+        const float4* wc = reinterpret_cast<const float4*>(p.to1_w + cq * 4);
+#pragma unroll 1
+        for (int i = 0; i < EpiRows<BM, BN, NT>::NR; ++i) {
+          const int row = r0 + RPP * i;
+          const int m = m0 + row;
+          if (row >= BM || m >= p.M) break;
+          float4 v = *reinterpret_cast<const float4*>(Cs + row * LDC + c4 * 4);
+          v.x = apply_act(v.x * sc.x + bi.x, p.act);
+          v.y = apply_act(v.y * sc.y + bi.y, p.act);
+          v.z = apply_act(v.z * sc.z + bi.z, p.act);
+          v.w = apply_act(v.w * sc.w + bi.w, p.act);
+          float4 wj = wc[0];
+          float a0 = v.x * wj.x, a1 = v.x * wj.y, a2 = v.x * wj.z, a3 = v.x * wj.w;
+          wj = wc[1];
+          a0 += v.y * wj.x; a1 += v.y * wj.y; a2 += v.y * wj.z; a3 += v.y * wj.w;
+          wj = wc[2];
+          a0 += v.z * wj.x; a1 += v.z * wj.y; a2 += v.z * wj.z; a3 += v.z * wj.w;
+          wj = wc[3];
+          a0 += v.w * wj.x; a1 += v.w * wj.y; a2 += v.w * wj.z; a3 += v.w * wj.w;
+#pragma unroll
+          for (int o = 8; o > 0; o >>= 1) {
+            a0 += __shfl_xor(a0, o, 64);
+            a1 += __shfl_xor(a1, o, 64);
+            a2 += __shfl_xor(a2, o, 64);
+            a3 += __shfl_xor(a3, o, 64);
+          }
+          if ((c4 & 15) == 0) {
+            const int n = m / ohw, rem = m - n * ohw;
+            const int oh = rem / p.OW, ow = rem - oh * p.OW;
+            float* o = p.out + ((size_t)n * (4 * p.OH) + 4 * oh + 2 * (ab >> 1)) * (size_t)(4 * p.OW) + 4 * ow + 2 * (ab & 1);
+            float2 top, bot;
+            top.x = 1.f / (1.f + expf(-(a0 + p.to1_b)));
+            top.y = 1.f / (1.f + expf(-(a1 + p.to1_b)));
+            bot.x = 1.f / (1.f + expf(-(a2 + p.to1_b)));
+            bot.y = 1.f / (1.f + expf(-(a3 + p.to1_b)));
+            *reinterpret_cast<float2*>(o) = top;
+            *reinterpret_cast<float2*>(o + 4 * p.OW) = bot;
+          }
+        }
+      }
+      return;
+    }
+    if (XE && p.res_up2) {
+      const int rh = p.OH >> 1, rw = p.OW >> 1;
+#pragma unroll 1
+      for (int i = 0; i < EpiRows<BM, BN, NT>::NR; ++i) {
+        const int row = r0 + RPP * i;
+        const int m = m0 + row;
+        if (row >= BM || m >= p.M) break;
+        const int n = m / ohw, rem = m - n * ohw;
+        const int oh = rem / p.OW, ow = rem - oh * p.OW;
+        int y0, y1, x0, x1;
+        float ly, lx;
+        bilinear_src(oh, 0.5f, rh, y0, y1, ly);
+        bilinear_src(ow, 0.5f, rw, x0, x1, lx);
+        const float* b = p.res + (size_t)n * rh * rw * p.res_ld + co;
+        const float4 v00 = *reinterpret_cast<const float4*>(b + ((size_t)y0 * rw + x0) * p.res_ld);
+        const float4 v01 = *reinterpret_cast<const float4*>(b + ((size_t)y0 * rw + x1) * p.res_ld);
+        const float4 v10 = *reinterpret_cast<const float4*>(b + ((size_t)y1 * rw + x0) * p.res_ld);
+        const float4 v11 = *reinterpret_cast<const float4*>(b + ((size_t)y1 * rw + x1) * p.res_ld);
+        const float4 rr = bilinear_blend4(ly, lx, v00, v01, v10, v11);
+        float4 v = *reinterpret_cast<const float4*>(Cs + row * LDC + c4 * 4);
+        v.x = v.x * sc.x + bi.x;
+        v.y = v.y * sc.y + bi.y;
+        v.z = v.z * sc.z + bi.z;
+        v.w = v.w * sc.w + bi.w;
+        v.x += rr.x; v.y += rr.y; v.z += rr.z; v.w += rr.w;
+        v.x = apply_act(v.x, p.act);
+        v.y = apply_act(v.y, p.act);
+        v.z = apply_act(v.z, p.act);
+        v.w = apply_act(v.w, p.act);
+        *reinterpret_cast<float4*>(p.out + (size_t)m * p.out_ld + co) = v;
+        amax_fold4(am, v);
+      }
+    } else {
 #pragma unroll(PRE ? EpiRows<BM, BN, NT>::NR : UNROLL)
     for (int i = 0; i < EpiRows<BM, BN, NT>::NR; ++i) {
       const int row = r0 + RPP * i;
@@ -230,6 +310,7 @@
       amax_fold4(am, v);
       if (PRE) __builtin_amdgcn_sched_barrier(0);
     }
+    }
   } else if (live) {
     for (int row = r0; row < BM; row += RPP) {
       const int m = m0 + row;
diff --git a/yomitoku_amd/csrc/ymk_conv_split.hip b/yomitoku_amd/csrc/ymk_conv_split.hip
--- a/yomitoku_amd/csrc/ymk_conv_split.hip
+++ b/yomitoku_amd/csrc/ymk_conv_split.hip
@@ -52,7 +52,7 @@
   return blocks * 64 * WM * WN / 256;
 }
 
-template <int BM, int BN, int WM, int WN, int NS, int KS, int PF, int FMT, bool OPL = false>
+template <int BM, int BN, int WM, int WN, int NS, int KS, int PF, int FMT, bool OPL = false, bool XE = false>
 __global__ __launch_bounds__(64 * WM * WN, (bf16_waves_per_simd<BM, BN, WM, WN, NS, KS>())) void conv_igemm_split(ConvK p, const uint4* __restrict__ wsplit) {
   typedef typename Half<FMT>::v8 h8;
   static_assert(PF >= 1 && PF <= 3, "prefetch: 1 = one stage ahead, 2 = two ahead, 3 = two ahead with the LDS stores threaded through the MFMAs");
@@ -348,7 +348,7 @@
           }
     }
     __syncthreads();
-    epilogue_tile<EROWS, BN, NT, false, 4, OPL>(p, Cs, m0 + e0, n0, t);
+    epilogue_tile<EROWS, BN, NT, false, 4, OPL, XE>(p, Cs, m0 + e0, n0, t);
   }
 }
 
@@ -620,6 +620,14 @@
   } else if (FMT == 1 && g_amax_check.load(std::memory_order_relaxed)) {
     amax_verify(s, k, ctx);
   }
+  if constexpr (!OPL) {
+    if (k.res_up2 != 0 || k.epi == EPI_DECONV2X2_TO1) {
+      hipLaunchKernelGGL((conv_igemm_split<BM, BN, WM, WN, NS, KS, PF, FMT, false, true>), dim3(mt * nt), dim3(64 * WM * WN), 0, s, k,
+                         reinterpret_cast<const uint4*>(wsplit));
+      if (e) YMK_HIP(hipEventRecord(e->second, s));
+      return;
+    }
+  }
   hipLaunchKernelGGL((conv_igemm_split<BM, BN, WM, WN, NS, KS, PF, FMT, OPL>), dim3(mt * nt), dim3(64 * WM * WN), 0, s, k,
                      reinterpret_cast<const uint4*>(wsplit));
   if (e) YMK_HIP(hipEventRecord(e->second, s));
@@ -634,6 +642,7 @@
 static std::atomic<int> g_act_planes{1};
 static std::atomic<int> g_rowmax_tile{0};
 static std::atomic<long long> g_n_astat{0}, g_n_ln_fused{0}, g_n_planes_read{0}, g_n_planes_written{0}, g_n_rowmax_wide{0};
+static std::atomic<long long> g_n_res_up2_staged{0};
 long long vit_mlp_fused_launches();
 bool conv_split_stat(const std::string& key, long long* value) {
   if (key == "astat_launches") *value = g_n_astat.load();
@@ -642,6 +651,7 @@
   else if (key == "planes_written_launches") *value = g_n_planes_written.load();
   else if (key == "rowmax_wide_launches") *value = g_n_rowmax_wide.load();
   else if (key == "mlp_fused_launches") *value = vit_mlp_fused_launches();
+  else if (key == "res_up2_staged_launches") *value = g_n_res_up2_staged.load();
   else return false;
   return true;
 }
@@ -743,6 +753,12 @@
   if (!q.rowmax && !q.row_group && (tile == 20 || tile == 21 || (auto_tile && dma_shape && dma_fills))) return ROUTE_DMA;
   if (tile == 20 || tile == 21) tile = 3;
   return ROUTE_STAGED;
+}
+
+int conv_split_route_plain(long M, int cout, int kpad, int taps, bool pointwise) {
+  int tile = 0;
+  bool narrow = false;
+  return (int)route_f16(RouteQuery{M, cout, kpad, taps, false, false, pointwise && kpad <= 256, false, false}, tile, narrow);
 }
 
 int conv_split_route_with_planes(long M, int cout, int kpad, int taps, bool* auto_tile) {
@@ -774,6 +790,10 @@
     narrow = w.cout <= 64 || tile == 1 || rowmax || blocks128 < 256;
   }
   if (route == ROUTE_NONE) return false;
+  if (route == ROUTE_DMA && (k.res_up2 != 0 || k.epi == EPI_DECONV2X2_TO1)) {
+    route = ROUTE_STAGED;
+    if (tile == 20 || tile == 21) tile = 3;
+  }
   YMK_CHECK(!k.in_planes || (route == ROUTE_DMA && tile != 20), "a tensor stored as fp16 planes reached a kernel that cannot read it");
   YMK_CHECK(!k.out_planes || (route == ROUTE_DMA && tile != 20) || (route == ROUTE_STAGED && (narrow || tile == 3)),
             "fp16 planes asked of a kernel that cannot write them");
@@ -813,6 +833,7 @@
   if (code == SPLIT_F16X2) {
     k.scale = pn.scale;
     if (rowmax && !narrow) ++g_n_rowmax_wide;
+    if (k.res_up2) ++g_n_res_up2_staged;
     dispatch_f16(s, k, pn.planes, tile, narrow, ctx);
   } else if (code == 2) {
     dispatch_bf16<2>(s, k, pn.planes, tile, narrow);
diff --git a/yomitoku_amd/csrc/ymk_dbnet.cpp b/yomitoku_amd/csrc/ymk_dbnet.cpp
--- a/yomitoku_amd/csrc/ymk_dbnet.cpp
+++ b/yomitoku_amd/csrc/ymk_dbnet.cpp
@@ -87,7 +87,8 @@
     ForwardScope forward_scope;
     ConvSplitScope split_scope(conv_split(), split_ctx.get(), SPLIT_MODEL_DEFAULT);
     YMK_CHECK(n > 0 && h % 32 == 0 && w % 32 == 0 && h >= 32 && w >= 32, "dbnet input must be a multiple of 32");
-    const uint64_t key = shape_key(n, h, w);
+    fuse_ = decide_fusion(n, h, w);
+    const uint64_t key = shape_key(n, h, w, fuse_);
     if (sync_workspace_mode()) shape_key_ = 0;
     if (key != shape_key_) {
       size_t need = 0;
@@ -113,13 +114,15 @@
     YMK_CHECK(finalized, "model not finalized");
     YMK_CHECK(n > 0 && h % 32 == 0 && w % 32 == 0 && h >= 32 && w >= 32, "dbnet reserve: sizes must be multiples of 32");
     sync_workspace_mode();
+    ConvSplitScope split_scope(conv_split(), split_ctx.get(), SPLIT_MODEL_DEFAULT);
     size_t need = 0;
     for (int turn = 0; turn < 2; ++turn) {
+      fuse_ = decide_fusion(n, turn ? w : h, turn ? h : w);
       arena.dry_run = true;
       arena.reset();
       run(nullptr, n, turn ? w : h, turn ? h : w, nullptr, s);
       arena.dry_run = false;
-      need = std::max(need, arena.plan_commit(shape_key(n, turn ? w : h, turn ? h : w), true));
+      need = std::max(need, arena.plan_commit(shape_key(n, turn ? w : h, turn ? h : w, fuse_), true));
       arena.reset();
     }
     if (need > arena.capacity() || arena.resize_pending()) {
@@ -130,7 +133,42 @@
   }
 
  private:
-  static uint64_t shape_key(int n, int h, int w) { return ((uint64_t)n << 40) | ((uint64_t)h << 20) | (uint64_t)w; }
+  static uint64_t shape_key(int n, int h, int w, int fuse) {
+    return ((uint64_t)fuse << 60) | ((uint64_t)n << 40) | ((uint64_t)h << 20) | (uint64_t)w;
+  }
+
+  enum : int { FUSE_P2 = 1, FUSE_P1 = 2, FUSE_TO1 = 4 };
+  int decide_fusion(int n, int h, int w) const {
+    int f = dbnet_fuse_to1() ? FUSE_TO1 : 0;
+    if (dbnet_fuse_up2()) {
+      const ConvArgs a;
+      for (int L = 1; L >= 0; --L) {
+        const int fh = h >> (L + 2), fw = w >> (L + 2), c = in_proj_[L].cout;
+        const Tensor in{nullptr, n, fh, fw, in_proj_[L].cin, in_proj_[L].cin}, top{nullptr, n, fh / 2, fw / 2, c, c};
+        if (conv_res_up2_ok(in, in_proj_[L], a, top)) f |= L == 1 ? FUSE_P2 : FUSE_P1;
+      }
+    }
+    return f;
+  }
+
+  Tensor lateral(hipStream_t s, const Tensor& feat, const ConvW& w, const Tensor& top, bool fused) {
+    if (fused) {
+      Tensor out = arena.tensor(feat.n, feat.h, feat.w, w.cout);
+      out.amax = arena.amax_next();
+      if (arena.dry_run) return out;
+      ConvArgs a;
+      a.res = &top;
+      a.res_up2 = true;
+      conv2d(s, feat, w, a, out);
+      return out;
+    }
+    Tensor up = arena.tensor(feat.n, feat.h, feat.w, top.c);
+    if (!arena.dry_run && dbnet_fuse_up2()) note_res_up2_fallback();
+    if (!arena.dry_run) upsample_bilinear(s, top, up, nullptr);
+    Tensor out = conv(s, feat, w, 1, 0, 1, ACT_NONE, &up);
+    arena.release(up);
+    return out;
+  }
 
   Tensor conv(hipStream_t s, const Tensor& in, const ConvW& w, int stride, int pad, int dil, int act,
               const Tensor* res = nullptr, const Tensor* into = nullptr, unsigned* rec = nullptr, bool out_planes = false) {
@@ -206,15 +244,9 @@
       arena.release(up);
     }
     arena.release(feat[2]);
-    Tensor up3 = arena.tensor(n, feat[1].h, feat[1].w, p3.c);
-    if (!dry) upsample_bilinear(s, p3, up3, nullptr);
-    Tensor p2 = conv(s, feat[1], in_proj_[1], 1, 0, 1, ACT_NONE, &up3);
-    arena.release(up3);
+    Tensor p2 = lateral(s, feat[1], in_proj_[1], p3, (fuse_ & FUSE_P2) != 0);
     arena.release(feat[1]);
-    Tensor up2 = arena.tensor(n, feat[0].h, feat[0].w, p2.c);
-    if (!dry) upsample_bilinear(s, p2, up2, nullptr);
-    Tensor p1 = conv(s, feat[0], in_proj_[0], 1, 0, 1, ACT_NONE, &up2);
-    arena.release(up2);
+    Tensor p1 = lateral(s, feat[0], in_proj_[0], p2, (fuse_ & FUSE_P1) != 0);
     arena.release(feat[0]);
 
     const int fh = p1.h, fw = p1.w;
@@ -256,14 +288,27 @@
     arena.release(cmean);
     Tensor b0 = conv(s, fused, bin_conv_, 1, 1, 1, ACT_RELU);
     arena.release(fused);
+    if (!dry) YMK_CHECK(4 * fh == h && 4 * fw == w, "binarize output shape");
+    if (fuse_ & FUSE_TO1) {
+      if (!dry) {
+        ConvArgs a;
+        a.act = ACT_RELU;
+        a.epi = EPI_DECONV2X2_TO1;
+        a.to1_w = deconv2_w_;
+        a.to1_b = deconv2_b_;
+        const Tensor pr{prob, n, h, w, 1, 1};
+        conv2d(s, b0, deconv1_, a, pr);
+      }
+      return;
+    }
     Tensor b1 = arena.tensor(n, 2 * fh, 2 * fw, 64);
     if (!dry) {
       ConvArgs a;
       a.act = ACT_RELU;
       a.epi = EPI_DECONV2X2;
       conv2d(s, b0, deconv1_, a, b1);
-      YMK_CHECK(4 * fh == h && 4 * fw == w, "binarize output shape");
       deconv2x2_to1_sigmoid(s, b1, deconv2_w_, deconv2_b_, prob);
+      note_deconv_to1_unfused();
     }
   }
 
@@ -277,6 +322,7 @@
   float* deconv2_w_ = nullptr;
   float deconv2_b_ = 0.f;
   uint64_t shape_key_ = 0;
+  int fuse_ = 0;
 };
 
 }
diff --git a/yomitoku_amd/csrc/ymk_elem.hip b/yomitoku_amd/csrc/ymk_elem.hip
--- a/yomitoku_amd/csrc/ymk_elem.hip
+++ b/yomitoku_amd/csrc/ymk_elem.hip
@@ -104,24 +104,16 @@
     pix /= OW;
     const int oh = (int)(pix % OH);
     const int n = (int)(pix / OH);
-    float fy = ((float)oh + 0.5f) * sh - 0.5f;
-    float fx = ((float)ow + 0.5f) * sw - 0.5f;
-    fy = fy < 0.f ? 0.f : fy;
-    fx = fx < 0.f ? 0.f : fx;
-    const int y0 = (int)fy, x0 = (int)fx;
-    const int y1 = y0 + (y0 < H - 1 ? 1 : 0), x1 = x0 + (x0 < W - 1 ? 1 : 0);
-    const float ly = fy - (float)y0, lx = fx - (float)x0;
-    const float hy = 1.f - ly, hx = 1.f - lx;
+    int y0, y1, x0, x1;
+    float ly, lx;
+    bilinear_src(oh, sh, H, y0, y1, ly);
+    bilinear_src(ow, sw, W, x0, x1, lx);
     const float* b = in + (size_t)n * H * W * in_ld + c4 * 4;
     const float4 v00 = *reinterpret_cast<const float4*>(b + ((size_t)y0 * W + x0) * in_ld);
     const float4 v01 = *reinterpret_cast<const float4*>(b + ((size_t)y0 * W + x1) * in_ld);
     const float4 v10 = *reinterpret_cast<const float4*>(b + ((size_t)y1 * W + x0) * in_ld);
     const float4 v11 = *reinterpret_cast<const float4*>(b + ((size_t)y1 * W + x1) * in_ld);
-    float4 r;
-    r.x = hy * (hx * v00.x + lx * v01.x) + ly * (hx * v10.x + lx * v11.x);
-    r.y = hy * (hx * v00.y + lx * v01.y) + ly * (hx * v10.y + lx * v11.y);
-    r.z = hy * (hx * v00.z + lx * v01.z) + ly * (hx * v10.z + lx * v11.z);
-    r.w = hy * (hx * v00.w + lx * v01.w) + ly * (hx * v10.w + lx * v11.w);
+    float4 r = bilinear_blend4(ly, lx, v00, v01, v10, v11);
     const size_t opix = (size_t)(n * OH + oh) * OW + ow;
     if (add) {
       const float4 t = *reinterpret_cast<const float4*>(add + opix * add_ld + c4 * 4);
```

Result: no change. 130.2, median of 6 (+2.5%).
